# CMU-Quake/hercules

Measured on AMD Instinct MI355X. Metric: element-updates/sec (whole node) + achieved HBM GB/s, 64M-elem box, higher is better.
Workload: dtype f64

## Files before the change

### hercules_amd/capi.py

```python
import ctypes
import os

import numpy as np

_HERE = os.path.dirname(os.path.abspath(__file__))
_LIBPATH = os.environ.get("HQ_SOLVER_LIB") or os.path.join(_HERE, "csrc", "libhq_solver.so")

HQ_VARIANT_AUTO, HQ_VARIANT_SCATTER, HQ_VARIANT_PATCH = 0, 1, 2
IPC_BLOB_BYTES = 4096

EXPORTS = ["hq_device_count", "hq_last_error", "hq_create", "hq_destroy", "hq_get_info", "hq_get_info_sized", "hq_abi_version", "hq_comm_init_ipc_n",
           "hq_options_init", "hq_create_opts", "hq_get_options", "hq_real_bytes",
           "hq_comm_unique_id", "hq_comm_init", "hq_comm_selftest", "hq_group_link", "hq_group_run", "hq_set_source", "hq_run", "hq_sync", "hq_gather", "hq_gather3",
           "hq_download", "hq_upload", "hq_phase_force", "hq_phase_update", "hq_download_force",
           "hq_run_timed", "hq_dominant_kernel", "hq_plan_check", "hq_stencil_plan_check", "hq_check_finite",
           "hq_stencil_coefficients", "hq_brick_plan_check", "hq_brick_plan_check_n", "hq_comm_init_host",
           "hq_comm_ipc_export", "hq_comm_init_ipc", "hq_comm_init_loopback"]


class HqError(RuntimeError):
    pass


HOST_EXCHANGE_FN = ctypes.CFUNCTYPE(ctypes.c_int, ctypes.c_void_p, ctypes.c_int32, ctypes.POINTER(ctypes.c_int32),
                                    ctypes.POINTER(ctypes.c_int64), ctypes.POINTER(ctypes.c_void_p), ctypes.c_int32,
                                    ctypes.POINTER(ctypes.c_int32), ctypes.POINTER(ctypes.c_int64),
                                    ctypes.POINTER(ctypes.c_void_p), ctypes.c_int32)


class _Messenger(ctypes.Structure):
    _fields_ = [("procid", ctypes.c_int32), ("nodecount", ctypes.c_int32),
                ("mapping", ctypes.c_void_p)]


class _Schedule(ctypes.Structure):
    _fields_ = [("c_count", ctypes.c_int32), ("first_c", ctypes.POINTER(_Messenger)),
                ("s_count", ctypes.c_int32), ("first_s", ctypes.POINTER(_Messenger))]


class _Desc(ctypes.Structure):
    _fields_ = [("lenum", ctypes.c_int32), ("nharbored", ctypes.c_int32), ("ldnnum", ctypes.c_int32),
                ("lnid", ctypes.c_void_p), ("node_xyz", ctypes.c_void_p),
                ("dn_ldnid", ctypes.c_void_p), ("dn_ptr", ctypes.c_void_p), ("dn_lanid", ctypes.c_void_p),
                ("eTable", ctypes.c_void_p), ("nTable", ctypes.c_void_p),
                ("tm1", ctypes.c_void_p), ("tm2", ctypes.c_void_p),
                ("an_sched", _Schedule), ("dn_sched", _Schedule),
                ("deltaT", ctypes.c_double), ("rank", ctypes.c_int32), ("nranks", ctypes.c_int32),
                ("variant", ctypes.c_int32), ("reserved", ctypes.c_int32), ("node_gnid", ctypes.c_void_p),
                ("edata", ctypes.c_void_p), ("mat_bbase", ctypes.c_double), ("mat_threshold_damping", ctypes.c_double),
                ("mat_threshold_vpvs", ctypes.c_double)]


class _Info(ctypes.Structure):
    _fields_ = [("variant", ctypes.c_int32), ("npatches", ctypes.c_int32),
                ("patch_pairs", ctypes.c_int64), ("device_bytes", ctypes.c_int64),
                ("step", ctypes.c_int32), ("nranks", ctypes.c_int32),
                ("lattice_patches", ctypes.c_int32), ("stencil_patches", ctypes.c_int32),
                ("ragged_patches", ctypes.c_int32), ("brick_units", ctypes.c_int32),
                ("brick_nodes", ctypes.c_int64), ("brick_units_pernode", ctypes.c_int32),
                ("brick_units_het", ctypes.c_int32), ("pcie_h2d_bytes", ctypes.c_int64),
                ("pcie_d2h_bytes", ctypes.c_int64), ("transport", ctypes.c_int32), ("ipc_arena_coarse", ctypes.c_int32),
                ("ipc_arena_kind", ctypes.c_int32), ("debug_halo", ctypes.c_int32),
                ("brick_units_packed", ctypes.c_int32), ("brick_units_ragged", ctypes.c_int32),
                ("brick_stream", ctypes.c_int32), ("brick_units_ragged_het", ctypes.c_int32), ("timed_steps", ctypes.c_int64),
                ("t_step_us", ctypes.c_double), ("t_shell_us", ctypes.c_double), ("t_interior_us", ctypes.c_double),
                ("t_chain_us", ctypes.c_double), ("t_chain_exposed_us", ctypes.c_double)]


OPTION_FIELDS = ["no_bricks", "brick_cz", "brick_minz", "brick_minnodes", "brick_no_het", "brick_no_ntsame", "brick_by_component",
                 "brick_stream", "brick_no_faces", "brick_half_tiles", "brick_no_pack", "patch_pipe", "patch_threads", "patch_pmax", "patch_pmerge", "patch_psplit", "patch_nlmax",
                 "patch_vmax", "patch_ragged", "patch_no_lattice", "patch_no_stencil", "patch_no_uniform", "patch_no_iso",
                 "patch_no_ntsame", "patch_no_dedup", "patch_wform", "patch_merge_rounds", "overlap", "no_overlap", "reserve_cus",
                 "cu_mask", "no_fused_share", "group_copies", "debug_halo", "ipc_arena"]


class Options(ctypes.Structure):
    _fields_ = ([("size", ctypes.c_uint64)] + [(n, ctypes.c_int32) for n in OPTION_FIELDS] +
                [("ipc_timeout_ms", ctypes.c_double), ("loopback_delay_us", ctypes.c_double),
                 ("verbose", ctypes.c_int32), ("quiet", ctypes.c_int32),
                 ("brick_ragged", ctypes.c_int32), ("brick_ragged_minfill", ctypes.c_int32),
                 ("allow_env", ctypes.c_int32), ("brick_ragged_het", ctypes.c_int32), ("reserved0", ctypes.c_int32),
                 ("phase_timing", ctypes.c_int32)])

    def __init__(self, **kw):
        super().__init__()
        load_library().hq_options_init(ctypes.byref(self), ctypes.c_uint64(ctypes.sizeof(self)))
        for k, v in kw.items():
            if k not in dict(self._fields_):
                raise TypeError("hq_options has no field %r" % k)
            setattr(self, k, v)

    def as_dict(self):
        return {k: getattr(self, k) for k, _ in self._fields_ if k != "size"}


_lib = None
_lib_f32 = None
_LIBPATH_F32 = os.environ.get("HQ_SOLVER_LIB_F32") or os.path.join(_HERE, "csrc", "libhq_solver_f32.so")


def load_library(path=None, precision="f64"):
    global _lib, _lib_f32
    if precision == "f32" and path is None:
        if _lib_f32 is None:
            _lib_f32 = load_library(_LIBPATH_F32)
            if _lib_f32.hq_real_bytes() != 4:
                raise HqError("%s was not built with -DHQ_SINGLE_PRECISION_SOLVER" % _LIBPATH_F32)
        return _lib_f32
    if _lib is not None and path is None:
        return _lib
    p = path or _LIBPATH
    if not os.path.exists(p):
        raise HqError("native library %s is missing: run `python -m hercules_amd.build` "
                      "(there is no Python/CPU fallback)" % p)
    probe = ctypes.CDLL(p, mode=ctypes.RTLD_LOCAL)
    lib = probe if probe.hq_real_bytes() == 4 else ctypes.CDLL(p, mode=ctypes.RTLD_GLOBAL)
    lib.hq_last_error.restype = ctypes.c_char_p
    lib.hq_dominant_kernel.restype = ctypes.c_char_p
    lib.hq_dominant_kernel.argtypes = [ctypes.c_void_p]
    for name in EXPORTS:
        getattr(lib, name)
    if path is None:
        _lib = lib
    return lib


def device_count():
    return int(load_library().hq_device_count())


def _check(rc, lib=None):
    if rc != 0:
        raise HqError("hq error %d: %s" % (rc, (lib or load_library()).hq_last_error().decode()))


def _ptr(a):
    return None if a is None else a.ctypes.data_as(ctypes.c_void_p)


def _schedule(sched, keep):
    out = _Schedule()
    if not sched:
        return out
    for key, cnt, first in (("c", "c_count", "first_c"), ("s", "s_count", "first_s")):
        items = sched.get(key, [])
        arr = (_Messenger * max(len(items), 1))()
        for i, (procid, mapping) in enumerate(items):
            m = np.ascontiguousarray(mapping, np.int32)
            keep.append(m)
            arr[i].procid = int(procid)
            arr[i].nodecount = len(m)
            arr[i].mapping = m.ctypes.data
        keep.append(arr)
        setattr(out, cnt, len(items))
        setattr(out, first, ctypes.cast(arr, ctypes.POINTER(_Messenger)))
    return out


class Solver:

    def __init__(self, lnid, etable, ntable, dt, tm1=None, tm2=None, node_xyz=None,
                 dangling=None, an_sched=None, dn_sched=None, rank=0, nranks=1,
                 variant=HQ_VARIANT_AUTO, device=0, options=None, edata=None, material=None, precision="f64"):
        lib = load_library(precision=precision)
        self.real = np.float32 if precision == "f32" else np.float64
        if lib.hq_real_bytes() != np.dtype(self.real).itemsize:
            raise HqError("library and precision %r disagree about sizeof(hq_real)" % precision)
        if isinstance(options, dict):
            options = Options(**options)
        keep = []
        lnid = np.ascontiguousarray(lnid, np.int32)
        etable = np.ascontiguousarray(etable, np.float64)
        ntable = np.ascontiguousarray(ntable, self.real)
        d = _Desc()
        d.lenum, d.nharbored = lnid.shape[0], ntable.shape[0]
        d.lnid, d.eTable, d.nTable = _ptr(lnid), _ptr(etable), _ptr(ntable)
        keep += [lnid, etable, ntable]
        if node_xyz is not None:
            node_xyz = np.ascontiguousarray(node_xyz, np.int32)
            keep.append(node_xyz)
            d.node_xyz = _ptr(node_xyz)
        for name, a in (("tm1", tm1), ("tm2", tm2)):
            if a is not None:
                a = np.ascontiguousarray(a, self.real)
                keep.append(a)
                setattr(d, name, _ptr(a))
        if dangling is not None:
            ids, ptr, anchors = [np.ascontiguousarray(x, np.int32) for x in dangling]
            keep += [ids, ptr, anchors]
            d.ldnnum = len(ids)
            d.dn_ldnid, d.dn_ptr, d.dn_lanid = _ptr(ids), _ptr(ptr), _ptr(anchors)
        if edata is not None:
            edata = np.ascontiguousarray(edata, np.float32)
            assert edata.shape == (lnid.shape[0], 4) and material is not None
            keep.append(edata)
            d.edata = _ptr(edata)
            d.mat_bbase, d.mat_threshold_damping, d.mat_threshold_vpvs = [float(v) for v in material]
        d.an_sched = _schedule(an_sched, keep)
        d.dn_sched = _schedule(dn_sched, keep)
        d.deltaT, d.rank, d.nranks, d.variant = dt, rank, nranks, variant
        self._h = ctypes.c_void_p()
        self.N, self.E = d.nharbored, d.lenum
        self._lib = lib
        if options is None:
            _check(lib.hq_create(ctypes.byref(d), ctypes.c_int(device), ctypes.byref(self._h)), lib)
        else:
            _check(lib.hq_create_opts(ctypes.byref(d), ctypes.c_int(device), ctypes.byref(options), ctypes.byref(self._h)), lib)

    def close(self):
        if getattr(self, "_h", None) and self._h.value:
            self._lib.hq_destroy(self._h)
            self._h = ctypes.c_void_p()

    __del__ = close

    def info(self):
        i = _Info()
        _check(self._lib.hq_get_info_sized(self._h, ctypes.byref(i), ctypes.c_uint64(ctypes.sizeof(i))), self._lib)
        return {k: getattr(i, k) for k, _ in _Info._fields_}

    def options(self):
        o = Options()
        _check(self._lib.hq_get_options(self._h, ctypes.byref(o), ctypes.c_uint64(ctypes.sizeof(o))), self._lib)
        return o.as_dict()

    def set_source(self, loaded_lnid, forces, step0=0):
        ids = np.ascontiguousarray(loaded_lnid, np.int32)
        F = np.ascontiguousarray(forces, np.float64)
        nsteps = F.shape[0] if len(ids) else 0
        _check(self._lib.hq_set_source(self._h, ctypes.c_int32(len(ids)), _ptr(ids),
                                       ctypes.c_int32(step0), ctypes.c_int32(nsteps), _ptr(F)))

    def comm_init(self, id128):
        buf = (ctypes.c_char * 128).from_buffer_copy(bytes(id128))
        _check(self._lib.hq_comm_init(self._h, buf), self._lib)

    def comm_init_host(self, exchange):
        import numpy as np

        def view(ptr, n):
            return np.ctypeslib.as_array(ctypes.cast(ctypes.c_void_p(ptr), ctypes.POINTER(ctypes.c_double)), shape=(int(n),))

        def trampoline(user, nrecv, rpeer, rcount, rbuf, nsend, speer, scount, sbuf, tag):
            try:
                exchange([(rpeer[i], view(rbuf[i], rcount[i])) for i in range(nrecv)],
                         [(speer[i], view(sbuf[i], scount[i])) for i in range(nsend)], tag)
                return 0
            except Exception:
                import traceback
                traceback.print_exc()
                return 1
        self._host_exchange = HOST_EXCHANGE_FN(trampoline)
        _check(self._lib.hq_comm_init_host(self._h, self._host_exchange, None), self._lib)

    def comm_ipc_export(self):
        buf = (ctypes.c_char * IPC_BLOB_BYTES)()
        _check(self._lib.hq_comm_ipc_export(self._h, buf), self._lib)
        return bytes(buf)

    def comm_init_ipc(self, blobs):
        raw = blobs if isinstance(blobs, (bytes, bytearray)) else b"".join(blobs)
        if len(raw) % IPC_BLOB_BYTES:
            raise HqError("comm_init_ipc: %d bytes is not a whole number of %d-byte blobs" % (len(raw), IPC_BLOB_BYTES))
        buf = (ctypes.c_char * len(raw)).from_buffer_copy(bytes(raw))
        _check(self._lib.hq_comm_init_ipc_n(self._h, buf, ctypes.c_int32(len(raw) // IPC_BLOB_BYTES)), self._lib)

    def comm_init_loopback(self):
        _check(self._lib.hq_comm_init_loopback(self._h), self._lib)

    def comm_selftest(self, count=1024):
        _check(self._lib.hq_comm_selftest(self._h, ctypes.c_int32(count)), self._lib)

    def run(self, nsteps):
        _check(self._lib.hq_run(self._h, ctypes.c_int32(nsteps)), self._lib)

    def sync(self):
        _check(self._lib.hq_sync(self._h), self._lib)

    def check_finite(self):
        n = ctypes.c_int64()
        _check(self._lib.hq_check_finite(self._h, ctypes.byref(n)), self._lib)
        return int(n.value)

    def run_timed(self, nsteps):
        tot, ker = ctypes.c_double(), ctypes.c_double()
        _check(self._lib.hq_run_timed(self._h, ctypes.c_int32(nsteps), ctypes.byref(tot), ctypes.byref(ker)), self._lib)
        return tot.value, ker.value

    def dominant_kernel(self):
        return self._lib.hq_dominant_kernel(self._h).decode()

    def download(self, want_tm2=True):
        tm1 = np.empty((self.N, 3), self.real)
        tm2 = np.empty((self.N, 3), self.real) if want_tm2 else None
        _check(self._lib.hq_download(self._h, _ptr(tm1), _ptr(tm2)), self._lib)
        return tm1, tm2

    def upload(self, tm1, tm2, step):
        a = np.ascontiguousarray(tm1, self.real)
        b = np.ascontiguousarray(tm2, self.real)
        _check(self._lib.hq_upload(self._h, _ptr(a), _ptr(b), ctypes.c_int32(step)), self._lib)

    def gather(self, lnid):
        ids = np.ascontiguousarray(np.asarray(lnid).reshape(-1), np.int32)
        o1 = np.empty((len(ids), 3), self.real)
        o2 = np.empty((len(ids), 3), self.real)
        _check(self._lib.hq_gather(self._h, ctypes.c_int32(len(ids)), _ptr(ids), _ptr(o1), _ptr(o2)), self._lib)
        return o1, o2

    def gather3(self, lnid):
        ids = np.ascontiguousarray(np.asarray(lnid).reshape(-1), np.int32)
        o = [np.empty((len(ids), 3), self.real) for _ in range(3)]
        _check(self._lib.hq_gather3(self._h, ctypes.c_int32(len(ids)), _ptr(ids), _ptr(o[0]), _ptr(o[1]), _ptr(o[2])), self._lib)
        return tuple(o)

    def phase_force(self):
        _check(self._lib.hq_phase_force(self._h), self._lib)

    def phase_update(self):
        _check(self._lib.hq_phase_update(self._h), self._lib)

    def download_force(self):
        f = np.empty((self.N, 3))
        _check(self._lib.hq_download_force(self._h, _ptr(f)), self._lib)
        return f


PLAN_REPORT = ("patches", "lattice_patches", "pairs", "distinct_row_blocks", "gather_passes", "gather_instructions",
               "lattice_gather_passes", "faults")


def plan_check(desc):
    rep = (ctypes.c_int64 * 8)()
    _check(load_library().hq_plan_check(ctypes.byref(desc), rep))
    return dict(zip(PLAN_REPORT, [int(v) for v in rep]))


STENCIL_PLAN_REPORT = ("patches", "tables", "full_lattices", "boundary_nodes", "corners_checked", "faults")


def stencil_plan_check(desc):
    rep = (ctypes.c_int64 * 6)()
    _check(load_library().hq_stencil_plan_check(ctypes.byref(desc), rep))
    return dict(zip(STENCIL_PLAN_REPORT, [int(v) for v in rep]))


BRICK_PLAN_REPORT = ("brick_nodes", "columns", "units", "units_one_nt_row", "het_units", "neighbours_checked",
                     "patch_nodes", "faults", "ragged_units", "ragged_nodes", "ragged_het_units", "ragged_het_nodes")


def brick_plan_check(desc):
    rep = (ctypes.c_int64 * len(BRICK_PLAN_REPORT))()
    _check(load_library().hq_brick_plan_check_n(ctypes.byref(desc), rep, ctypes.c_int32(len(BRICK_PLAN_REPORT))))
    return dict(zip(BRICK_PLAN_REPORT, [int(v) for v in rep]))


def comm_unique_id():
    buf = (ctypes.c_char * 128)()
    _check(load_library().hq_comm_unique_id(buf))
    return bytes(buf)


def group_link(solvers):
    arr = (ctypes.c_void_p * len(solvers))(*[s._h for s in solvers])
    lib = solvers[0]._lib
    _check(lib.hq_group_link(arr, ctypes.c_int32(len(solvers))), lib)


def group_run(solvers, nsteps):
    arr = (ctypes.c_void_p * len(solvers))(*[s._h for s in solvers])
    lib = solvers[0]._lib
    _check(lib.hq_group_run(arr, ctypes.c_int32(len(solvers)), ctypes.c_int32(nsteps)), lib)
    for s in solvers:
        s.sync()
```

### hercules_amd/csrc/hq_brick.h

```cpp
#ifndef HQ_BRICK_H
#define HQ_BRICK_H

#include <chrono>
#include <map>

#include "hq_patch.h"

#define HQ_BK_TX 64
#ifndef HQ_BK_TY
#define HQ_BK_TY 8
#endif
#define HQ_BK_THREADS (HQ_BK_TX * HQ_BK_TY)
#define HQ_BK_PY (HQ_BK_TX + 2)
#define HQ_BK_PLANE ((HQ_BK_TX + 2) * (HQ_BK_TY + 2))
#ifndef HQ_BK_ATTR
#define HQ_BK_ATTR
#endif
#define HQ_BK_NTSAME 1
#define HQ_BK_HET 2
#define HQ_BK_TOPFACE 8
#define HQ_BK_BOTFACE 16
#define HQ_BK_RAGGED 32
#define HQ_BK_PACKED 4
#ifndef HQ_BH_WAVES
#define HQ_BH_WAVES 8
#endif
#define HQ_BH_THREADS (64 * HQ_BH_WAVES)
#define HQ_BH_NRT (64 + 2 * (HQ_BH_WAVES - 1))
#define HQ_BH_TX 62
#define HQ_BH_TY (HQ_BH_WAVES - 1)
#define HQ_BH_PY 65
#define HQ_BH_CS HQ_BH_THREADS
#define HQ_BH_ROWS (65 * (HQ_BH_WAVES + 1))

struct hq_brick_unit {
    int64_t base;
    int64_t tab;
    int32_t nx, ny, np, flags;
    double  c1, c2, beta;
    double  m0, m2, m1;
    double  ft[7], fb[7];
    int64_t coef;
};

struct hq_brick_cfg {
    int cz = 32;
    int minz = 4;
    int minnodes = 512;
    int ragged = 1;
    int minfill = 128;
    int ragged_het = 1;
};

static hq_brick_cfg hq_brick_cfg_of(const hq_options& o)
{
    hq_brick_cfg c;
    c.cz = std::max(2, hq_value_or(o.brick_cz, c.cz));
    c.minz = std::max(1, hq_value_or(o.brick_minz, c.minz));
    c.minnodes = std::max(1, hq_value_or(o.brick_minnodes, c.minnodes));
    c.ragged = hq_value_or(o.brick_ragged, c.ragged) != 0;
    c.minfill = std::min(HQ_BK_THREADS, std::max(1, hq_value_or(o.brick_ragged_minfill, c.minfill)));
    c.ragged_het = hq_value_or(o.brick_ragged_het, c.ragged_het) != 0;
    return c;
}

struct hq_brick_host {
    int64_t nb = 0;
    std::vector<int32_t> perm;
    std::vector<hq_brick_unit> units;
    int32_t nsame = 0;
    int32_t nrag = 0;
    std::vector<int32_t> tab;
    std::vector<double> coef;
    std::vector<float> coef32;
    std::vector<double> nt2;
    int32_t nhet = 0;
    int32_t npacked = 0;
    int32_t nrhet = 0, nrpacked = 0;
    int32_t ncolumns = 0, nlevels = 0;
};

struct hq_brick_plan {
    int64_t nb = 0;
    int32_t nunits = 0, nsame = 0, nrag = 0, nhet = 0, npacked = 0, nrhet = 0, nrpacked = 0;
    hq_brick_unit* d_units = nullptr;
    int32_t* d_tab = nullptr;
    double* d_coef = nullptr;
    float* d_coef32 = nullptr;
    double* d_nt2 = nullptr;
    hq_mat_const mat = { 0, 0, 0, 0, 0, 0 };
    int32_t* d_src_ptr = nullptr;
    int32_t* d_src_ent = nullptr;
    std::vector<int64_t> h_base;
    std::vector<int32_t> h_slot;
    std::vector<int64_t> h_size;
    std::vector<int64_t> h_first;
};

struct hq_mat_src {
    const float* edata = nullptr;
    double dt = 0, bbase = 0, thr_damp = 0, thr_vpvs = 0;
};

static int hq_brick_plan_host(const hq_options& o, int64_t E, int64_t N, const int32_t* lnid, const int32_t* xyz, const double* c1,
                              const double* c2, const double* beta, const double* ntab, const char* excl,
                              hq_brick_host* B, const hq_mat_src* MS = nullptr)
{
    *B = hq_brick_host();
    if (!xyz || E <= 0 || N <= 0) return 0;
    const hq_brick_cfg cfg = hq_brick_cfg_of(o);
    const bool verbose = o.verbose > 1;
    auto t_lap = std::chrono::steady_clock::now();
    auto lap = [&](const char* what) {
        if (!verbose) return;
        const auto now = std::chrono::steady_clock::now();
        fprintf(stderr, "  brick plan: %-36s %6.2f s\n", what, std::chrono::duration<double>(now - t_lap).count());
        t_lap = now;
    };
    const int TX = HQ_BK_TX, TY = HQ_BK_TY;
    const bool want_het = !hq_set(o.brick_no_het);
    const bool stencil_ok = hq_stencil().ok;

    std::vector<int32_t> hs((size_t)E);
    std::map<int32_t, int64_t> cnt;
    {
        bool bad_order = false;
#pragma omp parallel
        {
            std::map<int32_t, int64_t> mine;
#pragma omp for schedule(static) reduction(|| : bad_order)
            for (int64_t e = 0; e < E; e++) {
                const int32_t* id = lnid + 8 * e;
                const int64_t h = (int64_t)xyz[3 * (int64_t)id[1]] - xyz[3 * (int64_t)id[0]];
                if (h <= 0 || h > 0x7fffffff) { bad_order = true; hs[(size_t)e] = 0; continue; }
                hs[(size_t)e] = (int32_t)h;
                mine[(int32_t)h]++;
            }
#pragma omp critical
            for (auto& kv : mine) cnt[kv.first] += kv.second;
        }
        if (bad_order) return 0;
    }
    lap("edge lengths");

    const bool want_faces = stencil_ok && hq_stencil().face_ok && !hq_set(o.brick_no_faces) && !hq_set(o.brick_no_ntsame);
    std::vector<uint8_t> touch;
    if (want_faces) {
        touch.assign((size_t)N, 0);
#pragma omp parallel for schedule(static)
        for (int64_t i = 0; i < E * 8; i++) {
            uint8_t& t8 = touch[(size_t)lnid[i]];
#pragma omp atomic
            t8++;
        }
    }

    struct level_t {
        int32_t h;
        int64_t O[3];
        int64_t D[3];
        std::vector<int32_t> Ng;
        std::vector<int32_t> Eg;
    };
    struct column_t { int lvl; int32_t x0, y0, nx, ny, z0, nz, ti, tj; int64_t base; int het; int top, bot; int rag; };
    struct ragged_t { std::vector<uint8_t> own; std::vector<int32_t> pfx; double c[3], m[3]; };
    std::vector<level_t> levels;
    std::vector<column_t> cols;
    std::vector<ragged_t> rags;
    std::vector<int32_t> ntx_of_level;

    for (auto& kv : cnt) {
        const int32_t h = kv.first;
        if (kv.second < (int64_t)cfg.minnodes) continue;
        level_t L;
        L.h = h;
        int64_t mn[3] = { INT64_MAX, INT64_MAX, INT64_MAX }, mx[3] = { INT64_MIN, INT64_MIN, INT64_MIN };
        {
            int64_t mn0 = INT64_MAX, mn1 = INT64_MAX, mn2 = INT64_MAX, mx0 = INT64_MIN, mx1 = INT64_MIN, mx2 = INT64_MIN;
#pragma omp parallel for schedule(static) reduction(min : mn0, mn1, mn2) reduction(max : mx0, mx1, mx2)
            for (int64_t e = 0; e < E; e++) {
                if (hs[(size_t)e] != h) continue;
                const int32_t* p = xyz + 3 * (int64_t)lnid[8 * e];
                mn0 = std::min<int64_t>(mn0, p[0]); mn1 = std::min<int64_t>(mn1, p[1]); mn2 = std::min<int64_t>(mn2, p[2]);
                mx0 = std::max<int64_t>(mx0, p[0]); mx1 = std::max<int64_t>(mx1, p[1]); mx2 = std::max<int64_t>(mx2, p[2]);
            }
            mn[0] = mn0; mn[1] = mn1; mn[2] = mn2; mx[0] = mx0; mx[1] = mx1; mx[2] = mx2;
        }
        bool ok = true;
        for (int d = 0; d < 3; d++) {
            L.O[d] = mn[d];
            if ((mx[d] - mn[d]) % h) ok = false;
            L.D[d] = (mx[d] - mn[d]) / h + 1;
        }
        if (!ok) continue;
        const int64_t NX = L.D[0] + 1, NY = L.D[1] + 1, NZ = L.D[2] + 1;
        const double vol = (double)NX * (double)NY * (double)NZ;
        if (vol > 8.0 * (double)kv.second + 65536.0 || vol > 2.0e9) continue;
        std::vector<int32_t>& Eg = L.Eg;
        Eg.assign((size_t)(L.D[0] * L.D[1] * L.D[2]), -1);
        L.Ng.assign((size_t)(NX * NY * NZ), -1);
        for (int pass = 0; pass < 2 && ok; pass++) {
            bool bad = false;
#pragma omp parallel for schedule(static) reduction(|| : bad)
            for (int64_t e = 0; e < E; e++) {
                if (hs[(size_t)e] != h) continue;
                const int32_t* id = lnid + 8 * e;
                int64_t q[3];
                bool good = true;
                for (int d = 0; d < 3; d++) {
                    const int64_t v = (int64_t)xyz[3 * (int64_t)id[0] + d] - L.O[d];
                    if (v % h) good = false;
                    q[d] = v / h;
                }
                if (!good) { bad = true; continue; }
                int32_t& cell = Eg[(size_t)((q[2] * L.D[1] + q[1]) * L.D[0] + q[0])];
                if (pass == 0) cell = (int32_t)e; else if (cell != (int32_t)e) bad = true;
                for (int c = 0; c < 8; c++) {
                    const int64_t X = q[0] + (c & 1), Y = q[1] + ((c >> 1) & 1), Z = q[2] + ((c >> 2) & 1);
                    const int32_t* p = xyz + 3 * (int64_t)id[c];
                    if (p[0] != L.O[0] + X * h || p[1] != L.O[1] + Y * h || p[2] != L.O[2] + Z * h) { bad = true; break; }
                    int32_t& g = L.Ng[(size_t)((Z * NY + Y) * NX + X)];
                    if (pass == 0) g = id[c]; else if (g != id[c]) bad = true;
                }
            }
            if (bad) ok = false;
        }
        if (!ok) continue;
        lap("level grids");
        std::vector<char> S((size_t)(NX * NY * NZ), 0);
        int64_t sx0 = INT64_MAX, sx1 = -1, sy0 = INT64_MAX, sy1 = -1;
        int64_t nsimple = 0;
#pragma omp parallel for schedule(static) reduction(min : sx0, sy0) reduction(max : sx1, sy1) reduction(+ : nsimple)
        for (int64_t Z = 1; Z < L.D[2]; Z++)
            for (int64_t Y = 1; Y < L.D[1]; Y++)
                for (int64_t X = 1; X < L.D[0]; X++) {
                    const int32_t n = L.Ng[(size_t)((Z * NY + Y) * NX + X)];
                    if (n < 0 || (excl && excl[n])) continue;
                    const double* q = ntab + 7 * (int64_t)n;
                    if (!((q[1] == q[2]) && (q[1] == q[3]) && (q[4] == q[5]) && (q[4] == q[6]))) continue;
                    int32_t e0 = -1;
                    bool s = true, uni = true;
                    for (int o = 0; o < 8 && s; o++) {
                        const int64_t cx = X - (o & 1), cy = Y - ((o >> 1) & 1), cz = Z - ((o >> 2) & 1);
                        const int32_t e = Eg[(size_t)((cz * L.D[1] + cy) * L.D[0] + cx)];
                        if (e < 0) { s = false; break; }
                        if (e0 < 0) e0 = e;
                        else uni = uni && c1[e] == c1[e0] && c2[e] == c2[e0] && beta[e] == beta[e0];
                    }
                    if (!s) continue;
                    if (!stencil_ok) uni = false;
// ... 252 lines not shown
    lap("numbering");
    B->nb = nb;
    B->ncolumns = (int32_t)cols.size();
    B->nlevels = (int32_t)levels.size();

    struct unit_t { int col; int32_t za, np; int64_t key; };
    std::vector<unit_t> us;
    int cz = cfg.cz;
    if (!hq_given(o.brick_cz)) {
        for (cz = 32; cz > 8; cz /= 2) {
            int64_t n = 0;
            for (auto& c : cols) n += (c.nz + cz - 1) / cz;
            if (n >= 512) break;
        }
    }
    for (size_t ci = 0; ci < cols.size(); ci++) {
        const column_t& c = cols[ci];
        const int32_t nch = (c.nz + cz - 1) / cz;
        const int32_t G = std::max(1, 64 / std::max(1, ntx_of_level[(size_t)c.lvl]));
        for (int32_t k = 0; k < nch; k++) {
            const int32_t za = (int32_t)((int64_t)c.nz * k / nch), zb = (int32_t)((int64_t)c.nz * (k + 1) / nch);
            const int64_t key = ((int64_t)c.lvl << 56) | ((int64_t)(c.tj / G) << 42) | ((int64_t)((c.z0 + za) / cz) << 28) |
                                ((int64_t)(c.tj % G) << 20) | (int64_t)c.ti;
            us.push_back({ (int)ci, c.z0 + za, zb - za, key });
        }
    }
    std::stable_sort(us.begin(), us.end(), [](const unit_t& a, const unit_t& b) { return a.key < b.key; });
    B->units.resize(us.size());
    std::vector<int64_t> toff(us.size() + 1, 0);
    for (size_t u = 0; u < us.size(); u++) {
        const column_t& c = cols[(size_t)us[u].col];
        const int64_t nr = 2 * (c.nx + 2) + 2 * c.ny;
        toff[u + 1] = toff[u] + ((int64_t)(us[u].np + 2) * nr + (c.rag ? us[u].np + 2 : 2) * (int64_t)c.nx * c.ny + 3) / 4 * 4;
    }
    B->tab.assign((size_t)toff[us.size()] + 64, 0);
    std::vector<int64_t> coff(us.size() + 1, 0);
    for (size_t u = 0; u < us.size(); u++)
        coff[u + 1] = coff[u] + (cols[(size_t)us[u].col].het ? (int64_t)(us[u].np + 1) * HQ_BH_THREADS * 3 : 0);
    B->coef.assign((size_t)coff[us.size()] + 8, 0.0);
    const bool try_pack = MS && MS->edata && MS->dt > 0 && !hq_set(o.brick_no_pack);
    if (try_pack) { B->coef32.assign((size_t)coff[us.size()] + 8, 0.0f); B->nt2.assign(2 * (size_t)N, 0.0); }
    int fault = 0;
    auto set_fault = [&]() {
#pragma omp atomic write
        fault = 1;
    };
    std::vector<char> same(us.size(), 0);
#pragma omp parallel for schedule(dynamic, 16)
    for (int64_t u = 0; u < (int64_t)us.size(); u++) {
        const column_t& c = cols[(size_t)us[(size_t)u].col];
        const level_t& L = levels[(size_t)c.lvl];
        const int64_t NX = L.D[0] + 1, NY = L.D[1] + 1;
        const int32_t za = us[(size_t)u].za, np = us[(size_t)u].np, nx = c.nx, ny = c.ny, nr = 2 * (nx + 2) + 2 * ny;
        auto dev = [&](int64_t X, int64_t Y, int64_t Z) -> int32_t {
            if (X < 0 || Y < 0 || Z < 0 || X > L.D[0] || Y > L.D[1] || Z > L.D[2]) { set_fault(); return 0; }
            const int32_t n = L.Ng[(size_t)((Z * NY + Y) * NX + X)];
            if (n < 0) { set_fault(); return 0; }
            return B->perm[(size_t)n];
        };
        int32_t* t = B->tab.data() + toff[(size_t)u];
        hq_brick_unit& U = B->units[(size_t)u];
        if (c.rag) {
            const ragged_t& R = rags[(size_t)c.rag - 1];
            auto any = [&](int64_t X, int64_t Y, int64_t Z) -> int32_t {
                if (X < 0 || Y < 0 || Z < 0 || X > L.D[0] || Y > L.D[1] || Z > L.D[2]) return -1;
                const int32_t n = L.Ng[(size_t)((Z * NY + Y) * NX + X)];
                return n < 0 ? -1 : B->perm[(size_t)n];
            };
            auto owns = [&](int32_t i, int32_t j, int32_t k) -> bool {
                return i >= 0 && i < nx && j >= 0 && j < ny && k >= 1 && k <= np && R.own[(size_t)((((int64_t)za - 1 + k - c.z0) * ny + j) * nx + i)];
            };
            auto wanted = [&](int32_t i, int32_t j, int32_t k) -> bool {
                for (int32_t dk = -1; dk <= 1; dk++)
                    for (int32_t dj = -1; dj <= 1; dj++)
                        for (int32_t di = -1; di <= 1; di++)
                            if (owns(i + di, j + dj, k + dk)) return true;
                return false;
            };
            for (int32_t k = 0; k < np + 2; k++) {
                const int64_t Z = (int64_t)za - 1 + k;
                int32_t* r = t + (int64_t)k * nr;
                for (int32_t i = 0; i < nx + 2; i++) {
                    r[i] = wanted(i - 1, -1, k) ? any(c.x0 - 1 + i, c.y0 - 1, Z) : -1;
                    r[nx + 2 + i] = wanted(i - 1, ny, k) ? any(c.x0 - 1 + i, c.y0 + ny, Z) : -1;
                }
                for (int32_t j = 0; j < ny; j++) {
                    r[2 * (nx + 2) + j] = wanted(-1, j, k) ? any(c.x0 - 1, c.y0 + j, Z) : -1;
                    r[2 * (nx + 2) + ny + j] = wanted(nx, j, k) ? any(c.x0 + nx, c.y0 + j, Z) : -1;
                }
                int32_t* pl = t + (int64_t)(np + 2) * nr + (int64_t)k * nx * ny;
                for (int32_t j = 0; j < ny; j++)
                    for (int32_t i = 0; i < nx; i++) {
                        const bool own = owns(i, j, k);
                        const int32_t q = own || wanted(i, j, k) ? any(c.x0 + i, c.y0 + j, Z) : -1;
                        if (own && q < 0) set_fault();
                        pl[j * nx + i] = own ? q : (q < 0 ? -1 : -q - 2);
                    }
            }
            U.base = c.base + R.pfx[(size_t)(za - c.z0)];
            U.tab = toff[(size_t)u];
            U.nx = nx; U.ny = ny; U.np = np; U.flags = HQ_BK_NTSAME | HQ_BK_RAGGED;
            memset(U.ft, 0, sizeof U.ft); memset(U.fb, 0, sizeof U.fb);
            U.coef = 0;
            if (!c.het) {
                U.c1 = R.c[0]; U.c2 = R.c[1]; U.beta = R.c[2];
                U.m0 = R.m[0]; U.m2 = R.m[1]; U.m1 = R.m[2];
                same[(size_t)u] = 4;
                continue;
            }
            U.flags = HQ_BK_RAGGED;
            U.c1 = U.c2 = U.beta = 0.0; U.m0 = 1.0; U.m2 = U.m1 = 0.0;
        }
        if (!c.rag) {
        for (int32_t k = 0; k < np + 2; k++) {
            const int64_t Z = (int64_t)za - 1 + k;
            int32_t* r = t + (int64_t)k * nr;
            for (int32_t i = 0; i < nx + 2; i++) { r[i] = dev(c.x0 - 1 + i, c.y0 - 1, Z); r[nx + 2 + i] = dev(c.x0 - 1 + i, c.y0 + ny, Z); }
            for (int32_t j = 0; j < ny; j++) { r[2 * (nx + 2) + j] = dev(c.x0 - 1, c.y0 + j, Z); r[2 * (nx + 2) + ny + j] = dev(c.x0 + nx, c.y0 + j, Z); }
        }
        int32_t* cap = t + (int64_t)(np + 2) * nr;
        for (int32_t j = 0; j < ny; j++)
            for (int32_t i = 0; i < nx; i++) {
                cap[j * nx + i] = dev(c.x0 + i, c.y0 + j, (int64_t)za - 1);
                cap[nx * ny + j * nx + i] = dev(c.x0 + i, c.y0 + j, (int64_t)za + np);
            }
        U.base = c.base + (int64_t)(za - c.z0 + c.top) * nx * ny;
        U.tab = toff[(size_t)u];
        U.nx = nx; U.ny = ny; U.np = np; U.flags = 0;
        memset(U.ft, 0, sizeof U.ft); memset(U.fb, 0, sizeof U.fb);
        if (c.top && za == c.z0) {
            U.flags |= HQ_BK_TOPFACE;
            memcpy(U.ft, ntab + 7 * (int64_t)L.Ng[(size_t)((((int64_t)za - 1) * NY + c.y0) * NX + c.x0)], sizeof U.ft);
        }
        if (c.bot && za + np == c.z0 + c.nz) {
            U.flags |= HQ_BK_BOTFACE;
            memcpy(U.fb, ntab + 7 * (int64_t)L.Ng[(size_t)((((int64_t)za + np) * NY + c.y0) * NX + c.x0)], sizeof U.fb);
        }
        const int32_t n0 = L.Ng[(size_t)(((int64_t)za * NY + c.y0) * NX + c.x0)];
        {
            const int32_t e0 = L.Eg[(size_t)((((int64_t)za - 1) * L.D[1] + (c.y0 - 1)) * L.D[0] + (c.x0 - 1))];
            if (e0 < 0) { set_fault(); continue; }
            U.c1 = c1[e0]; U.c2 = c2[e0]; U.beta = beta[e0];
        }
        bool sm = true;
        const double* q0 = ntab + 7 * (int64_t)n0;
        for (int32_t z = 0; z < np && sm; z++)
            for (int32_t y = 0; y < ny && sm; y++)
                for (int32_t x = 0; x < nx; x++) {
                    const int32_t n = L.Ng[(size_t)((((int64_t)za + z) * NY + (c.y0 + y)) * NX + (c.x0 + x))];
                    const double* q = ntab + 7 * (int64_t)n;
                    if (q[0] != q0[0] || q[1] != q0[1] || q[4] != q0[4]) { sm = false; break; }
                }
        if (sm && !c.het && !hq_set(o.brick_no_ntsame)) { U.flags |= HQ_BK_NTSAME; same[(size_t)u] = 1; }
        U.m0 = q0[0]; U.m2 = q0[1]; U.m1 = q0[4];
        U.coef = 0;
        }
        if (c.het) {
            U.flags |= HQ_BK_HET;
            same[(size_t)u] = c.rag ? 5 : 2;
            U.coef = coff[(size_t)u];
            double* cf = B->coef.data() + coff[(size_t)u];
            for (int32_t l = 0; l <= np; l++)
                for (int32_t j = 0; j < HQ_BH_WAVES; j++)
                    for (int32_t i = 0; i < 64; i++) {
                        const int64_t cx = (int64_t)c.x0 - 1 + i, cy = (int64_t)c.y0 - 1 + j, cz = (int64_t)za - 1 + l;
                        double* o = cf + (int64_t)l * (3 * HQ_BH_THREADS) + (j * 64 + i);
                        int32_t e = -1;
                        if (cx >= 0 && cy >= 0 && cz >= 0 && cx < L.D[0] && cy < L.D[1] && cz < L.D[2])
                            e = L.Eg[(size_t)((cz * L.D[1] + cy) * L.D[0] + cx)];
                        if (e >= 0) { o[0] = c1[e]; o[HQ_BH_CS] = c2[e]; o[2 * HQ_BH_CS] = beta[e]; }
                        else if (!c.rag && i <= nx && j <= ny) set_fault();
                    }
            if (try_pack) {
                bool ok = true;
                int32_t e0 = L.Eg[(size_t)(((int64_t)za * L.D[1] + c.y0) * L.D[0] + c.x0)];
                if (c.rag) {
                    e0 = -1;
                    for (int32_t l = 0; l <= np && e0 < 0; l++)
                        for (int32_t j = 0; j < HQ_BH_WAVES && e0 < 0; j++)
                            for (int32_t i = 0; i < 64 && e0 < 0; i++) {
                                const int64_t cx = (int64_t)c.x0 - 1 + i, cy = (int64_t)c.y0 - 1 + j, cz = (int64_t)za - 1 + l;
                                if (cx >= 0 && cy >= 0 && cz >= 0 && cx < L.D[0] && cy < L.D[1] && cz < L.D[2]) e0 = L.Eg[(size_t)((cz * L.D[1] + cy) * L.D[0] + cx)];
                            }
                }
                const float hf = e0 >= 0 ? MS->edata[4 * (int64_t)e0] : 0.0f;
                hq_mat_const K = { (MS->dt * MS->dt) * (double)hf, (double)hf, MS->dt, MS->bbase, MS->thr_damp, MS->thr_vpvs };
                float* cq = B->coef32.data() + coff[(size_t)u];
                for (int32_t l = 0; l <= np && ok; l++)
                    for (int32_t j = 0; j < HQ_BH_WAVES && ok; j++)
                        for (int32_t i = 0; i < 64; i++) {
                            const int64_t cx = (int64_t)c.x0 - 1 + i, cy = (int64_t)c.y0 - 1 + j, cz = (int64_t)za - 1 + l;
                            int32_t e = -1;
                            if (cx >= 0 && cy >= 0 && cz >= 0 && cx < L.D[0] && cy < L.D[1] && cz < L.D[2])
                                e = L.Eg[(size_t)((cz * L.D[1] + cy) * L.D[0] + cx)];
                            float* o = cq + (int64_t)l * (3 * HQ_BH_THREADS) + (j * 64 + i);
                            o[0] = o[HQ_BH_CS] = o[2 * HQ_BH_CS] = 0.0f;
                            if (e < 0) continue;
                            const float* ed = MS->edata + 4 * (int64_t)e;
                            if (ed[0] != hf || !(ed[3] > 0.0f)) { ok = false; break; }
                            bool hit = false;
                            for (int fixed = 0; fixed < 2 && !hit; fixed++) {
                                double k1, k2, kb;
                                hq_material_coef(fixed ? -ed[3] : ed[3], ed[2], ed[1], K, &k1, &k2, &kb);
                                if (k1 == c1[e] && k2 == c2[e] && kb == beta[e]) { o[0] = fixed ? -ed[3] : ed[3]; o[HQ_BH_CS] = ed[2]; o[2 * HQ_BH_CS] = ed[1]; hit = true; }
                            }
                            if (!hit) { ok = false; break; }
                        }
                const int32_t* own_ids = c.rag ? t + (int64_t)(np + 2) * nr + (int64_t)nx * ny : nullptr;
                for (int32_t z = 0; z < np && ok; z++)
                    for (int32_t y = 0; y < ny && ok; y++)
                        for (int32_t x = 0; x < nx; x++) {
                            if (own_ids && own_ids[((int64_t)z * ny + y) * nx + x] < 0) continue;
                            const int32_t n = L.Ng[(size_t)((((int64_t)za + z) * NY + (c.y0 + y)) * NX + (c.x0 + x))];
                            const double* q = ntab + 7 * (int64_t)n;
                            const double sdiff = q[0] - q[4];
                            if (q[0] - sdiff != q[4] || fabs((2.0 * q[0] - sdiff) - q[1]) > 1e-15 * fabs(q[1])) { ok = false; break; }
                            double* o2 = B->nt2.data() + 2 * (own_ids ? (int64_t)own_ids[((int64_t)z * ny + y) * nx + x] : U.base + ((int64_t)z * ny + y) * nx + x);
                            o2[0] = q[0]; o2[1] = sdiff;
                        }
                if (ok) { U.flags |= HQ_BK_PACKED; same[(size_t)u] = c.rag ? 6 : 3; U.c1 = K.A; U.c2 = K.h; }
            }
        }
    }
    lap("unit tables");
    if (fault) { g_patch_err = "brick plan: a neighbour of a simple node is missing"; return -1; }
    {
        std::vector<hq_brick_unit> a, r, b, h, hp, rh, rhp;
        for (size_t u = 0; u < us.size(); u++)
            (same[u] == 1 ? a : (same[u] == 4 ? r : (same[u] == 2 ? h : (same[u] == 3 ? hp : (same[u] == 5 ? rh : (same[u] == 6 ? rhp : b)))))).push_back(B->units[u]);
        B->nsame = (int32_t)(a.size() + r.size());
        B->nrag = (int32_t)r.size();
        B->nhet = (int32_t)(h.size() + hp.size());
        B->npacked = (int32_t)hp.size();
        B->nrhet = (int32_t)(rh.size() + rhp.size());
        B->nrpacked = (int32_t)rhp.size();
        a.insert(a.end(), r.begin(), r.end());
        a.insert(a.end(), b.begin(), b.end());
        a.insert(a.end(), h.begin(), h.end());
        a.insert(a.end(), hp.begin(), hp.end());
        a.insert(a.end(), rh.begin(), rh.end());
        a.insert(a.end(), rhp.begin(), rhp.end());
        B->units.swap(a);
        if (B->npacked + B->nrpacked == 0) { std::vector<float>().swap(B->coef32); std::vector<double>().swap(B->nt2); }
        if (verbose) fprintf(stderr, "  brick plan: %d units: %d with one n_t row of which %d ragged, %d per-element coefficients of which %d packed, %d ragged per-element of which %d packed\n",
                             (int)B->units.size(), B->nsame, B->nrag, B->nhet, B->npacked, B->nrhet, B->nrpacked);
        if (verbose && B->nrag) {
            int64_t pos = 0, own = 0, other = 0;
            for (const hq_brick_unit& U : B->units) {
                if (!(U.flags & HQ_BK_RAGGED)) continue;
                const int32_t* pl = B->tab.data() + U.tab + (int64_t)(U.np + 2) * (2 * (U.nx + 2) + 2 * U.ny);
                for (int64_t i = 0; i < (int64_t)U.nx * U.ny * (U.np + 2); i++) { pos++; own += pl[i] >= 0; other += pl[i] <= -2; }
            }
            fprintf(stderr, "  brick plan: ragged units: %lld positions, %lld owned, %lld loaded for their neighbours' sake\n", (long long)pos, (long long)own, (long long)other);
        }
    }
    return 0;
}


static __device__ __forceinline__ double hq_uniform(double v)
{
    const int lo = __builtin_amdgcn_readfirstlane(__double2loint(v)), hi = __builtin_amdgcn_readfirstlane(__double2hiint(v));
    return __hiloint2double(hi, lo);
}

template <bool PERNODE, bool BYCOMP, bool RAGGED = false>
__global__ void HQ_BK_ATTR __launch_bounds__(HQ_BK_THREADS, 4)
hq_k_brick(int32_t count, int32_t per_xcd, const hq_brick_unit* __restrict__ units, const int32_t* __restrict__ tab,
           const hq_real* __restrict__ u1g, const hq_real* __restrict__ u2g, hq_real* __restrict__ ung,
           const double* __restrict__ nt3, const int32_t* __restrict__ src_ptr, const int32_t* __restrict__ src_ent,
           const double* __restrict__ F, double dt2, hq_stencil_coef sc)
{
    __shared__ __align__(16) double s_w[2 * 3 * HQ_BK_PLANE];
    const int slot = (int)(blockIdx.x & 7) * per_xcd + (int)(blockIdx.x >> 3);
    if (slot >= count) return;
    const hq_brick_unit U = units[slot];
    const int nx = U.nx, ny = U.ny, np = U.np, nxy = nx * ny, nr = 2 * (nx + 2) + 2 * ny;
    const int t = threadIdx.x, lx = t & (HQ_BK_TX - 1), ly = t >> 6;
    const bool active = lx < nx && ly < ny;
    const int sidx = active ? ly * nx + lx : 0;
    const int myrow = (ly + 1) * HQ_BK_PY + lx + 1;
    const bool ring = t < nr;
    int rrow;
    {
        int rx, ry;
        if (t < nx + 2) { rx = t - 1; ry = -1; }
        else if (t < 2 * (nx + 2)) { rx = t - (nx + 2) - 1; ry = ny; }
        else if (t < 2 * (nx + 2) + ny) { rx = -1; ry = t - 2 * (nx + 2); }
        else { rx = nx; ry = t - 2 * (nx + 2) - ny; }
        rrow = (ry + 1) * HQ_BK_PY + rx + 1;
    }
    const int32_t* __restrict__ utab = tab + U.tab;
    const int rofs = ring ? t : 0;
    const int32_t* __restrict__ cap = utab + (int64_t)(np + 2) * nr;
    int32_t vOut = -1, vMid = RAGGED ? cap[sidx] : 0, vCur = RAGGED ? cap[nxy + sidx] : 0, vNext = 0;
    const int32_t id_lo = RAGGED ? (vMid >= 0 ? vMid : -vMid - 2) : cap[sidx];
    const double beta = U.beta;
    double P[6], Q[2];
#pragma unroll
    for (int i = 0; i < 6; i++) P[i] = hq_uniform(U.c1 * sc.p1[i] + U.c2 * sc.p2[i]);
#pragma unroll
    for (int i = 0; i < 2; i++) Q[i] = hq_uniform(U.c1 * sc.q1[i] + U.c2 * sc.q2[i]);
    const bool has_src = F && src_ptr[slot + 1] > src_ptr[slot];

    hq_real x1[3] = { 0, 0, 0 }, x2[3] = { 0, 0, 0 }, y1[3] = { 0, 0, 0 }, y2[3] = { 0, 0, 0 };
    double mn[3] = { U.m0, U.m2, U.m1 };
    double m0A = hq_uniform(1.0 / U.m0), m0B = m0A;
    double fA[3] = { 0.0, 0.0, 0.0 }, fB[3] = { 0.0, 0.0, 0.0 };
    int32_t rid = utab[rofs];

#define HQ_BK_LOAD(node_)                                                                             \
    {                                                                                                 \
        const int64_t a_ = (node_);                                                                   \
        if (active && (!RAGGED || a_ >= 0)) {                                                         \
            _Pragma("unroll") for (int d = 0; d < 3; d++) { x1[d] = u1g[3 * a_ + d]; x2[d] = u2g[3 * a_ + d]; } \
            if (PERNODE) { _Pragma("unroll") for (int d = 0; d < 3; d++) mn[d] = nt3[3 * a_ + d]; }    \
        }                                                                                             \
        if (ring && (!RAGGED || rid >= 0)) {                                                          \
            const int64_t b_ = (int64_t)rid;                                                          \
            _Pragma("unroll") for (int d = 0; d < 3; d++) { y1[d] = u1g[3 * b_ + d]; y2[d] = u2g[3 * b_ + d]; } \
        }                                                                                             \
    }
#define HQ_BK_PUT(s_, acc_, M2_, M1_)                                                                 \
    {                                                                                                 \
        hq_lds_double* img_ = (hq_lds_double*)s_w + 3 * HQ_BK_PLANE * (s_);                            \
        if (active) {                                                                                 \
            _Pragma("unroll") for (int d = 0; d < 3; d++) {                                           \
                const double a1_ = x1[d], a2_ = x2[d];                                                \
                img_[3 * myrow + d] = a1_ + beta * (a1_ - a2_);                                       \
                acc_[d] += (M2_) * a1_ - (M1_) * a2_;                                                 \
            }                                                                                         \
        }                                                                                             \
        if (ring) { _Pragma("unroll") for (int d = 0; d < 3; d++) { const double b1_ = y1[d], b2_ = y2[d]; img_[3 * rrow + d] = b1_ + beta * (b1_ - b2_); } } \
    }

    const bool topf = !PERNODE && !RAGGED && (U.flags & HQ_BK_TOPFACE) != 0, botf = !PERNODE && !RAGGED && (U.flags & HQ_BK_BOTFACE) != 0;
    const double rho = hq_uniform((U.c1 - U.c2) / (U.c1 + U.c2));

    HQ_BK_LOAD((int64_t)id_lo)
    rid = utab[nr + rofs];
    if (topf) HQ_BK_PUT(0, fB, U.ft[1 + d], U.ft[4 + d])
    else { double dummy[3] = { 0.0, 0.0, 0.0 }; HQ_BK_PUT(0, dummy, mn[1], mn[2]) }
    for (int k = 0; k <= np + 1; k++) {
        if (k <= np) {
            if (RAGGED) {
                HQ_BK_LOAD((int64_t)(vCur >= 0 ? vCur : -vCur - 2))
                if (k < np) vNext = cap[(k + 2) * nxy + sidx];
            } else HQ_BK_LOAD(k == np ? (int64_t)cap[nxy + sidx] : U.base + (int64_t)k * nxy + sidx)
            if (k < np) rid = utab[(k + 2) * nr + rofs];
        }
        __syncthreads();
        const hq_lds_double* __restrict__ q = (const hq_lds_double*)s_w + 3 * (HQ_BK_PLANE * (k & 1) + myrow);
        double m[3], g[3], Uo[3];
        if (BYCOMP) {
            double A_x, A_y;
            {
                const double C = q[2], XM = q[2 - 3], XP = q[2 + 3], YM = q[2 - 3 * HQ_BK_PY], YP = q[2 + 3 * HQ_BK_PY];
                const double MM = q[2 - 3 * HQ_BK_PY - 3], PM = q[2 - 3 * HQ_BK_PY + 3], MP = q[2 + 3 * HQ_BK_PY - 3], PP = q[2 + 3 * HQ_BK_PY + 3];
                const double sxy = (XM + XP) + (YM + YP), dg = (MM + PP) + (PM + MP);
                m[2] = fma(P[0], C, fma(P[2], sxy, P[4] * dg));
                g[2] = fma(P[1], C, fma(P[3], sxy, P[5] * dg));
                Uo[0] = fma(Q[0], XP - XM, Q[1] * ((PP - MP) + (PM - MM)));
                Uo[1] = fma(Q[0], YP - YM, Q[1] * ((PP - PM) + (MP - MM)));
            }
            __builtin_amdgcn_sched_barrier(0);
            {
                const double C = q[0], XM = q[0 - 3], XP = q[0 + 3], YM = q[0 - 3 * HQ_BK_PY], YP = q[0 + 3 * HQ_BK_PY];
                const double MM = q[0 - 3 * HQ_BK_PY - 3], PM = q[0 - 3 * HQ_BK_PY + 3], MP = q[0 + 3 * HQ_BK_PY - 3], PP = q[0 + 3 * HQ_BK_PY + 3];
                const double sx = XM + XP, sy = YM + YP, dg = (MM + PP) + (PM + MP);
                A_x = (PP + MM) - (PM + MP);
                m[0] = fma(P[0], C, fma(P[1], sx, fma(P[2], sy, P[3] * dg)));
                g[0] = fma(P[2], C, fma(P[3], sx, fma(P[4], sy, P[5] * dg)));
                Uo[2] = fma(Q[0], XP - XM, Q[1] * ((PP - MP) + (PM - MM)));
            }
            __builtin_amdgcn_sched_barrier(0);
            {
                const double C = q[1], XM = q[1 - 3], XP = q[1 + 3], YM = q[1 - 3 * HQ_BK_PY], YP = q[1 + 3 * HQ_BK_PY];
                const double MM = q[1 - 3 * HQ_BK_PY - 3], PM = q[1 - 3 * HQ_BK_PY + 3], MP = q[1 + 3 * HQ_BK_PY - 3], PP = q[1 + 3 * HQ_BK_PY + 3];
                const double sx = XM + XP, sy = YM + YP, dg = (MM + PP) + (PM + MP);
                A_y = (PP + MM) - (PM + MP);
                m[1] = fma(P[0], C, fma(P[1], sy, fma(P[2], sx, fma(P[3], dg, Q[0] * A_x))));
                g[1] = fma(P[2], C, fma(P[3], sy, fma(P[4], sx, fma(P[5], dg, Q[1] * A_x))));
                Uo[2] += fma(Q[0], YP - YM, Q[1] * ((PP - PM) + (MP - MM)));
            }
            m[0] = fma(Q[0], A_y, m[0]);
            g[0] = fma(Q[1], A_y, g[0]);
        } else {
            double C[3], XM[3], XP[3], YM[3], YP[3], MM[3], PM[3], MP[3], PP[3];
#pragma unroll
            for (int d = 0; d < 3; d++) {
                C[d] = q[d]; XM[d] = q[d - 3]; XP[d] = q[d + 3]; YM[d] = q[d - 3 * HQ_BK_PY]; YP[d] = q[d + 3 * HQ_BK_PY];
                MM[d] = q[d - 3 * HQ_BK_PY - 3]; PM[d] = q[d - 3 * HQ_BK_PY + 3];
                MP[d] = q[d + 3 * HQ_BK_PY - 3]; PP[d] = q[d + 3 * HQ_BK_PY + 3];
            }
            double sx[3], sy[3], dg[3];
#pragma unroll
            for (int d = 0; d < 3; d++) { sx[d] = XM[d] + XP[d]; sy[d] = YM[d] + YP[d]; dg[d] = (MM[d] + PP[d]) + (PM[d] + MP[d]); }
            const double A_x = (PP[0] + MM[0]) - (PM[0] + MP[0]), A_y = (PP[1] + MM[1]) - (PM[1] + MP[1]);
            const double Bx0_z = XP[2] - XM[2], Bx0_x = XP[0] - XM[0], By0_z = YP[2] - YM[2], By0_y = YP[1] - YM[1];
            const double Bx1_z = (PP[2] - MP[2]) + (PM[2] - MM[2]), Bx1_x = (PP[0] - MP[0]) + (PM[0] - MM[0]);
            const double By1_z = (PP[2] - PM[2]) + (MP[2] - MM[2]), By1_y = (PP[1] - PM[1]) + (MP[1] - MM[1]);
            const double sxy_z = sx[2] + sy[2];
            m[0] = fma(P[0], C[0], fma(P[1], sx[0], fma(P[2], sy[0], fma(P[3], dg[0], Q[0] * A_y))));
            m[1] = fma(P[0], C[1], fma(P[1], sy[1], fma(P[2], sx[1], fma(P[3], dg[1], Q[0] * A_x))));
            m[2] = fma(P[0], C[2], fma(P[2], sxy_z, P[4] * dg[2]));
            g[0] = fma(P[2], C[0], fma(P[3], sx[0], fma(P[4], sy[0], fma(P[5], dg[0], Q[1] * A_y))));
            g[1] = fma(P[2], C[1], fma(P[3], sy[1], fma(P[4], sx[1], fma(P[5], dg[1], Q[1] * A_x))));
            g[2] = fma(P[1], C[2], fma(P[3], sxy_z, P[5] * dg[2]));
            Uo[0] = fma(Q[0], Bx0_z, Q[1] * Bx1_z);
            Uo[1] = fma(Q[0], By0_z, Q[1] * By1_z);
            Uo[2] = fma(Q[0], Bx0_x, fma(Q[1], Bx1_x, fma(Q[0], By0_y, Q[1] * By1_y)));
        }
        if (k == 0 && topf) {
            m[0] = fma(rho, Uo[0], 0.5 * m[0]); m[1] = fma(rho, Uo[1], 0.5 * m[1]); m[2] = fma(-rho, Uo[2], 0.5 * m[2]);
        }
        if (k == np + 1 && botf && active) {
            double f[3];
            f[0] = fB[0] + fma(-rho, Uo[0], 0.5 * m[0]); f[1] = fB[1] + fma(-rho, Uo[1], 0.5 * m[1]); f[2] = fB[2] + fma(rho, Uo[2], 0.5 * m[2]);
            const int local = np * nxy + sidx;
            if (has_src) {
                for (int i = src_ptr[slot]; i < src_ptr[slot + 1]; i++)
                    if (src_ent[2 * i] == local) {
                        const int li = src_ent[2 * i + 1];
                        for (int d = 0; d < 3; d++) f[d] += F[3 * li + d] * dt2;
                    }
            }
            hq_real* out = ung + 3 * (int64_t)cap[nxy + sidx];
            const double rm = 1.0 / U.fb[0];
#pragma unroll
            for (int d = 0; d < 3; d++) out[d] = f[d] * rm;
        }
        const bool outface = k == 1 && topf;
        if ((k >= 2 || outface) && active && (!RAGGED || vOut >= 0)) {
            double f[3];
#pragma unroll
            for (int d = 0; d < 3; d++) f[d] = fA[d] + (g[d] + Uo[d]);
            const int local = RAGGED ? (int)(vOut - U.base) : (k - 2) * nxy + sidx;
            if (has_src) {
                for (int i = src_ptr[slot]; i < src_ptr[slot + 1]; i++)
                    if (src_ent[2 * i] == local) {
                        const int li = src_ent[2 * i + 1];
                        for (int d = 0; d < 3; d++) f[d] += F[3 * li + d] * dt2;
                    }
            }
            hq_real* out = ung + 3 * (RAGGED ? (int64_t)vOut : (outface ? (int64_t)cap[sidx] : U.base + (int64_t)local));
            const double rm = outface ? 1.0 / U.ft[0] : m0A;
#pragma unroll
            for (int d = 0; d < 3; d++) out[d] = f[d] * rm;
        }
#pragma unroll
        for (int d = 0; d < 3; d++) { fA[d] = fB[d] + m[d]; fB[d] = g[d] - Uo[d]; }
        if (RAGGED) { vOut = vMid; vMid = vCur; vCur = vNext; }
        if (PERNODE) { m0A = m0B; m0B = 1.0 / mn[0]; }
        if (k < np || (k == np && !botf)) HQ_BK_PUT((k + 1) & 1, fB, mn[1], mn[2])
        else if (k == np) HQ_BK_PUT((k + 1) & 1, fB, U.fb[1 + d], U.fb[4 + d])
    }
#undef HQ_BK_LOAD
#undef HQ_BK_PUT
}


#define HQ_BH_LDS (8 * (2 * 2 * 3 * HQ_BH_ROWS + 6 * HQ_BH_THREADS))
#ifndef HQ_BH_ABL
#define HQ_BH_ABL 0
#endif

static __device__ __forceinline__ double hq_dpp_from_next_lane(double v)
{
    int lo = __double2loint(v), hi = __double2hiint(v);
    lo = __builtin_amdgcn_update_dpp(0, lo, 0x130, 0xf, 0xf, true);
    hi = __builtin_amdgcn_update_dpp(0, hi, 0x130, 0xf, 0xf, true);
    return __hiloint2double(hi, lo);
}

static __device__ __forceinline__ int64_t hq_rag_node(int32_t v) { return v >= 0 ? (int64_t)v : (v <= -2 ? (int64_t)(-v - 2) : (int64_t)0); }

template <bool PACKED, bool RAGGED = false>
__global__ void __launch_bounds__(HQ_BH_THREADS, HQ_BH_WAVES == 12 ? 3 : 4)
hq_k_brick_het(int32_t count, int32_t per_xcd, const hq_brick_unit* __restrict__ units, const int32_t* __restrict__ tab,
               const void* __restrict__ coef_any, const hq_real* __restrict__ u1g, const hq_real* __restrict__ u2g,
               hq_real* __restrict__ ung, const double* __restrict__ nt3, const int32_t* __restrict__ src_ptr,
               const int32_t* __restrict__ src_ent, const double* __restrict__ F, double dt2, hq_mat_const mat)
{
    extern __shared__ __align__(16) double s_het[];
    hq_lds_double* const img = (hq_lds_double*)s_het;
    hq_lds_double* const xch = img + 2 * 2 * 3 * HQ_BH_ROWS;
    const int slot = (int)(blockIdx.x & 7) * per_xcd + (int)(blockIdx.x >> 3);
    if (slot >= count) return;
    const hq_brick_unit U = units[slot];
    const int nx = U.nx, ny = U.ny, np = U.np, nxy = nx * ny, nr = 2 * (nx + 2) + 2 * ny;
    const int t = threadIdx.x, lx = t & 63, ly = t >> 6;
    const bool owner = lx < nx && ly < ny;
    const int sidx = owner ? ly * nx + lx : 0;
    const int myrow = (ly + 1) * HQ_BH_PY + lx + 1;
    const int row0 = ly * HQ_BH_PY + lx;
    const int rq = ly == HQ_BH_WAVES - 1 ? lx : (lx >= 62 ? 64 + 2 * ly + (lx - 62) : -1);
    const bool ringA = rq >= 0 && rq < nr, ringB = rq >= 0 && rq + HQ_BH_NRT < nr;
    auto ring_row = [&](int r) {
        int rx, ry;
        if (r < nx + 2) { rx = r - 1; ry = -1; }
        else if (r < 2 * (nx + 2)) { rx = r - (nx + 2) - 1; ry = ny; }
        else if (r < 2 * (nx + 2) + ny) { rx = -1; ry = r - 2 * (nx + 2); }
        else { rx = nx; ry = r - 2 * (nx + 2) - ny; }
        return (ry + 1) * HQ_BH_PY + rx + 1;
    };
    const int rrowA = ringA ? ring_row(rq) : 0, rrowB = ringB ? ring_row(rq + HQ_BH_NRT) : 0;
    const int32_t* __restrict__ rtabA = tab + U.tab + (ringA ? rq : 0);
    const int32_t* __restrict__ rtabB = tab + U.tab + (ringB ? rq + HQ_BH_NRT : 0);
    const int32_t* __restrict__ cap = tab + U.tab + (int64_t)(np + 2) * nr;
    const int64_t id_lo = RAGGED ? 0 : cap[sidx], id_hi = RAGGED ? 0 : cap[nxy + sidx];
    int32_t vload = RAGGED ? cap[sidx] : 0, vnext = RAGGED ? cap[nxy + sidx] : 0, idA = -1, idB = -1;
    const double* __restrict__ cf = (const double*)coef_any + (PACKED ? 0 : U.coef + t);
    const float* __restrict__ cf32 = (const float*)coef_any + (PACKED ? U.coef + t : 0);
    hq_mat_const K = mat;
    if (PACKED) { K.A = hq_uniform(U.c1); K.h = hq_uniform(U.c2); }
    const int third = (PACKED && owner) ? 1 : 2;
    const bool has_src = F && src_ptr[slot + 1] > src_ptr[slot];

    hq_real x1[3] = { 0, 0, 0 }, x2[3] = { 0, 0, 0 }, rb1[3] = { 0, 0, 0 }, rb2[3] = { 0, 0, 0 };
    constexpr bool SAME = sizeof(hq_real) == sizeof(double);
    double mn[3] = { 1.0, 0.0, 0.0 };
    double accA[3] = { 0.0, 0.0, 0.0 }, accB[3] = { 0.0, 0.0, 0.0 }, m0A = 1.0, m0B = 1.0;
    int32_t ridA = rtabA[0], ridB = rtabB[0];
    if (RAGGED) { ridA = ridA < 0 ? 0 : ridA; ridB = ridB < 0 ? 0 : ridB; }

#define HQ_BH_LOAD(node_)                                                                             \
    {                                                                                                 \
        const int64_t a_ = owner ? (int64_t)(node_) : (int64_t)ridA;                                  \
        const double* __restrict__ pb_ = (owner || sizeof(hq_real) != sizeof(double)) ? nt3 + (PACKED ? 2 : 3) * a_ : (const double*)(const void*)(u1g + 3 * (int64_t)ridB); \
        _Pragma("unroll") for (int d = 0; d < 3; d++) { x1[d] = u1g[3 * a_ + d]; x2[d] = u2g[3 * a_ + d]; } \
        if (SAME || owner) {                                                                          \
            if (HQ_BH_ABL != 4) { mn[0] = pb_[0]; mn[1] = pb_[1]; mn[2] = pb_[third]; }                \
        } else {                      \
            const hq_real* __restrict__ pu_ = u1g + 3 * (int64_t)ridB;                                \
            rb1[0] = pu_[0]; rb1[1] = pu_[1]; rb1[2] = pu_[2];                                         \
        }                                                                                             \
    }
#define HQ_BH_LOAD_B()                                                                                \
    {                                                                                                 \
        if (ringB && HQ_BH_ABL != 1) {                                                                \
            const int64_t b_ = (int64_t)ridB;                                                         \
            _Pragma("unroll") for (int d = 0; d < 3; d++) { if (SAME) accB[d] = u2g[3 * b_ + d]; else rb2[d] = u2g[3 * b_ + d]; } \
        }                                                                                             \
    }
#define HQ_BH_PUT(s_, acc_, m0_)                                                                      \
    {                                                                                                 \
        hq_lds_double* iu_ = img + (size_t)(s_) * (2 * 3 * HQ_BH_ROWS);                                \
        hq_lds_double* iv_ = iu_ + 3 * HQ_BH_ROWS;                                                    \
        if (owner) {                                                                                  \
            const double m2_ = PACKED ? 2.0 * mn[0] - mn[1] : mn[1], m1_ = PACKED ? mn[0] - mn[1] : mn[2]; \
            _Pragma("unroll") for (int d = 0; d < 3; d++) {                                           \
                const double a1_ = x1[d], a2_ = x2[d];                                                \
                iu_[3 * myrow + d] = a1_; iv_[3 * myrow + d] = a1_ - a2_;                             \
                acc_[d] = m2_ * a1_ - m1_ * a2_;                                                      \
            }                                                                                         \
            m0_ = 1.0 / mn[0];                                                                        \
            if (RAGGED) idB = vload;                                                                  \
        }                                                                                             \
        if (ringA) { _Pragma("unroll") for (int d = 0; d < 3; d++) { const double a1_ = x1[d], a2_ = x2[d]; iu_[3 * rrowA + d] = a1_; iv_[3 * rrowA + d] = a1_ - a2_; } } \
        if (ringB) { _Pragma("unroll") for (int d = 0; d < 3; d++) { const double b1_ = SAME ? mn[d] : (double)rb1[d], b2_ = SAME ? accB[d] : (double)rb2[d]; iu_[3 * rrowB + d] = b1_; iv_[3 * rrowB + d] = b1_ - b2_; } } \
    }

    double nc1 = 0.0, nc2 = 0.0, nbeta = 0.0, c1 = 0.0, c2 = 0.0, beta = 0.0;
    float nrho = 0.0f, nvs = 0.0f, nvp = 0.0f;
#define HQ_BH_REQUEST(p_)                                                                             \
    {                                                                                                 \
        const int pp_ = (p_);                                                                         \
        if (HQ_BH_ABL != 2 && !PACKED) { const double* q_ = cf + (int64_t)(pp_ - 1) * (3 * HQ_BH_THREADS); nc1 = q_[0]; nc2 = q_[HQ_BH_CS]; nbeta = q_[2 * HQ_BH_CS]; } \
        if (HQ_BH_ABL != 2 && PACKED) { const float* q_ = cf32 + (int64_t)(pp_ - 1) * (3 * HQ_BH_THREADS); nrho = q_[0]; nvs = q_[HQ_BH_CS]; nvp = q_[2 * HQ_BH_CS]; } \
        if (RAGGED) vload = vnext;                                                                    \
        HQ_BH_LOAD(RAGGED ? hq_rag_node(vload) : (pp_ == np + 1 ? id_hi : U.base + (int64_t)(pp_ - 1) * nxy + sidx)) \
        HQ_BH_LOAD_B()                                                                                \
        { const int64_t r_ = (int64_t)(pp_ < np + 1 ? pp_ + 1 : np + 1) * nr; ridA = rtabA[r_]; ridB = rtabB[r_]; } \
        if (RAGGED) vnext = cap[(int64_t)(pp_ < np + 1 ? pp_ + 1 : np + 1) * nxy + sidx];              \
    }
    if (HQ_BH_ABL == 2) { nc1 = dt2; nc2 = dt2; nbeta = dt2; }
    HQ_BH_LOAD(RAGGED ? hq_rag_node(vload) : id_lo)
    HQ_BH_LOAD_B()
    ridA = rtabA[nr]; ridB = rtabB[nr];
    if (RAGGED) { ridA = ridA < 0 ? 0 : ridA; ridB = ridB < 0 ? 0 : ridB; }
    for (int l = -2; l <= np; l++) {
        if (l >= 0) {
            double X[8], Y[8], Z[8];
#pragma unroll
            for (int m = 0; m < 8; m++) {
                const hq_lds_double* pu = img + (size_t)((l + (m >> 2)) & 1) * (2 * 3 * HQ_BH_ROWS) + 3 * (row0 + (m & 1) + ((m >> 1) & 1) * HQ_BH_PY);
                const hq_lds_double* pv = pu + 3 * HQ_BH_ROWS;
                X[m] = fma(beta, pv[0], pu[0]); Y[m] = fma(beta, pv[1], pu[1]); Z[m] = fma(beta, pv[2], pu[2]);
            }
            if (HQ_BH_ABL != 3) hq_element_force<true>(X, Y, Z, c1, c2);
            double G[2][2][3];
#pragma unroll
            for (int yb = 0; yb < 2; yb++)
#pragma unroll
                for (int zb = 0; zb < 2; zb++) {
                    const int m1 = 1 + 2 * yb + 4 * zb, m0 = 2 * yb + 4 * zb;
                    G[yb][zb][0] = X[m1] + hq_dpp_from_next_lane(X[m0]);
                    G[yb][zb][1] = Y[m1] + hq_dpp_from_next_lane(Y[m0]);
                    G[yb][zb][2] = Z[m1] + hq_dpp_from_next_lane(Z[m0]);
                }
#pragma unroll
            for (int zb = 0; zb < 2; zb++)
#pragma unroll
                for (int d = 0; d < 3; d++) xch[(3 * zb + d) * HQ_BH_THREADS + t] = G[0][zb][d];
            __syncthreads();
            if (owner) {
                double H0[3], H1[3];
#pragma unroll
                for (int d = 0; d < 3; d++) {
                    H0[d] = G[1][0][d] + xch[d * HQ_BH_THREADS + t + 64];
                    H1[d] = G[1][1][d] + xch[(3 + d) * HQ_BH_THREADS + t + 64];
                }
                if (l >= 1 && (!RAGGED || idA >= 0)) {
                    double f[3];
#pragma unroll
                    for (int d = 0; d < 3; d++) f[d] = accA[d] + (H0[d] - H1[d]);
                    const int local = RAGGED ? (int)((int64_t)idA - U.base) : (l - 1) * nxy + sidx;
                    if (has_src) {
                        for (int i = src_ptr[slot]; i < src_ptr[slot + 1]; i++)
                            if (src_ent[2 * i] == local) {
                                const int li = src_ent[2 * i + 1];
                                for (int d = 0; d < 3; d++) f[d] += F[3 * li + d] * dt2;
                            }
                    }
                    hq_real* out = ung + 3 * (U.base + (int64_t)local);
#pragma unroll
                    for (int d = 0; d < 3; d++) out[d] = f[d] * m0A;
                }
#pragma unroll
                for (int d = 0; d < 3; d++) accA[d] = accB[d] + (H0[d] + H1[d]);
                m0A = m0B;
                if (RAGGED) idA = idB;
            }
        }
        if (l < np) HQ_BH_PUT(l & 1, accB, m0B)
        if (PACKED) hq_material_coef(nrho, nvs, nvp, K, &c1, &c2, &beta);
        else { c1 = nc1; c2 = nc2; beta = nbeta; }
        asm volatile("" : "+v"(c1), "+v"(c2), "+v"(beta), "+v"(ridA), "+v"(ridB));
        if (RAGGED) { asm volatile("" : "+v"(vnext)); ridA = ridA < 0 ? 0 : ridA; ridB = ridB < 0 ? 0 : ridB; }
        if (l + 1 < np) HQ_BH_REQUEST(l + 3)
        __syncthreads();
    }
#undef HQ_BH_REQUEST
#undef HQ_BH_LOAD
#undef HQ_BH_LOAD_B
#undef HQ_BH_PUT
}


static void hq_brick_free(hq_brick_plan* P)
{
    void* ptrs[] = { P->d_units, P->d_tab, P->d_coef, P->d_coef32, P->d_nt2, P->d_src_ptr, P->d_src_ent };
    for (void* p : ptrs) if (p) hipFree(p);
    *P = hq_brick_plan();
}

static int hq_brick_upload(hq_brick_plan* P, const hq_brick_host& B, int64_t* bytes)
{
    P->nb = B.nb;
    P->nunits = (int32_t)B.units.size();
    P->nsame = B.nsame;
    P->nrag = B.nrag;
    P->nhet = B.nhet;
    P->npacked = B.npacked;
    P->nrhet = B.nrhet;
    P->nrpacked = B.nrpacked;
    if (P->nunits == 0) return 0;
    if (P->nhet + P->nrhet > 0) {
        if (P->nhet > P->npacked || P->nrhet > P->nrpacked) {
            if (hipMalloc((void**)&P->d_coef, 8 * B.coef.size()) != hipSuccess) { g_patch_err = "hipMalloc failed"; return -2; }
            *bytes += (int64_t)(8 * B.coef.size());
            if (hipMemcpy(P->d_coef, B.coef.data(), 8 * B.coef.size(), hipMemcpyHostToDevice) != hipSuccess) { g_patch_err = "brick coefficient upload failed"; return -3; }
        }
        if (P->npacked + P->nrpacked > 0) {
            if (hipMalloc((void**)&P->d_coef32, 4 * B.coef32.size()) != hipSuccess || hipMalloc((void**)&P->d_nt2, 8 * B.nt2.size()) != hipSuccess) { g_patch_err = "hipMalloc failed"; return -2; }
            *bytes += (int64_t)(4 * B.coef32.size() + 8 * B.nt2.size());
            if (hipMemcpy(P->d_coef32, B.coef32.data(), 4 * B.coef32.size(), hipMemcpyHostToDevice) != hipSuccess ||
                hipMemcpy(P->d_nt2, B.nt2.data(), 8 * B.nt2.size(), hipMemcpyHostToDevice) != hipSuccess) { g_patch_err = "brick coefficient upload failed"; return -3; }
        }
        static bool attr_set = false;
        if (!attr_set) {
            if (hipFuncSetAttribute((const void*)hq_k_brick_het<false>, hipFuncAttributeMaxDynamicSharedMemorySize, HQ_BH_LDS) != hipSuccess ||
                hipFuncSetAttribute((const void*)hq_k_brick_het<true>, hipFuncAttributeMaxDynamicSharedMemorySize, HQ_BH_LDS) != hipSuccess ||
                hipFuncSetAttribute((const void*)hq_k_brick_het<false, true>, hipFuncAttributeMaxDynamicSharedMemorySize, HQ_BH_LDS) != hipSuccess ||
                hipFuncSetAttribute((const void*)hq_k_brick_het<true, true>, hipFuncAttributeMaxDynamicSharedMemorySize, HQ_BH_LDS) != hipSuccess) { g_patch_err = "hq_k_brick_het: LDS attribute"; return -3; }
            attr_set = true;
        }
    }
    if (hipMalloc((void**)&P->d_units, sizeof(hq_brick_unit) * B.units.size()) != hipSuccess ||
        hipMalloc((void**)&P->d_tab, 4 * B.tab.size()) != hipSuccess) { g_patch_err = "hipMalloc failed"; return -2; }
    *bytes += (int64_t)(sizeof(hq_brick_unit) * B.units.size() + 4 * B.tab.size());
    if (hipMemcpy(P->d_units, B.units.data(), sizeof(hq_brick_unit) * B.units.size(), hipMemcpyHostToDevice) != hipSuccess ||
        hipMemcpy(P->d_tab, B.tab.data(), 4 * B.tab.size(), hipMemcpyHostToDevice) != hipSuccess) { g_patch_err = "brick table upload failed"; return -3; }
    std::vector<std::pair<int64_t, int32_t>> by_base;
    for (int32_t u = 0; u < P->nunits; u++) by_base.push_back({ B.units[(size_t)u].base, u });
    std::sort(by_base.begin(), by_base.end());
    for (auto& pr : by_base) {
        const hq_brick_unit& U = B.units[(size_t)pr.second];
        const int64_t nxy = (int64_t)U.nx * U.ny;
        const int top = (U.flags & HQ_BK_TOPFACE) != 0, bot = (U.flags & HQ_BK_BOTFACE) != 0;
        int64_t size = nxy * (U.np + top + bot);
        if (U.flags & HQ_BK_RAGGED) {
            const int32_t* pl = B.tab.data() + U.tab + (int64_t)(U.np + 2) * (2 * (U.nx + 2) + 2 * U.ny);
            size = 0;
            for (int64_t i = nxy; i < nxy * (U.np + 1); i++) size += pl[i] >= 0;
        }
        P->h_base.push_back(pr.first - top * nxy); P->h_slot.push_back(pr.second); P->h_size.push_back(size);
        P->h_first.push_back(pr.first);
    }
    return 0;
}

static int hq_brick_set_source(hq_brick_plan* P, int32_t nloaded, const int32_t* loaded, int64_t* bytes)
{
    if (P->d_src_ptr) { hipFree(P->d_src_ptr); P->d_src_ptr = nullptr; }
    if (P->d_src_ent) { hipFree(P->d_src_ent); P->d_src_ent = nullptr; }
    if (nloaded <= 0 || P->nunits == 0) return 0;
    std::vector<std::array<int32_t, 3>> rec;
    for (int32_t i = 0; i < nloaded; i++) {
        if (loaded[i] >= P->nb) continue;
        const size_t k = (size_t)(std::upper_bound(P->h_base.begin(), P->h_base.end(), (int64_t)loaded[i]) - P->h_base.begin()) - 1;
        rec.push_back({ P->h_slot[k], (int32_t)(loaded[i] - P->h_first[k]), i });
    }
    if (rec.empty()) return 0;
    std::sort(rec.begin(), rec.end());
    std::vector<int32_t> ptr((size_t)P->nunits + 1, 0), ent(rec.size() * 2);
    for (auto& r : rec) ptr[(size_t)r[0] + 1]++;
    for (int32_t u = 0; u < P->nunits; u++) ptr[(size_t)u + 1] += ptr[(size_t)u];
    for (size_t k = 0; k < rec.size(); k++) { ent[2 * k] = rec[k][1]; ent[2 * k + 1] = rec[k][2]; }
    if (hipMalloc((void**)&P->d_src_ptr, 4 * ptr.size()) != hipSuccess) { P->d_src_ptr = nullptr; return -2; }
    if (hipMalloc((void**)&P->d_src_ent, 4 * ent.size()) != hipSuccess) {
        hipFree(P->d_src_ptr); P->d_src_ptr = nullptr; P->d_src_ent = nullptr;
        return -2;
    }
    if (hipMemcpy(P->d_src_ptr, ptr.data(), 4 * ptr.size(), hipMemcpyHostToDevice) != hipSuccess ||
        hipMemcpy(P->d_src_ent, ent.data(), 4 * ent.size(), hipMemcpyHostToDevice) != hipSuccess) {
        hipFree(P->d_src_ptr); hipFree(P->d_src_ent); P->d_src_ptr = nullptr; P->d_src_ent = nullptr;
        return -3;
    }
    *bytes += (int64_t)(4 * ptr.size() + 4 * ent.size());
    return 0;
}

static void hq_brick_launch(const hq_brick_plan* P, const hq_real* u1, const hq_real* u2, hq_real* un, const double* nt3,
                            const double* F, double dt2, hipStream_t stream, bool light = false)
{
    const int32_t cnt[7] = { P->nsame - P->nrag, P->nunits - P->nsame - P->nhet - P->nrhet, P->nhet - P->npacked, P->npacked, P->nrag,
                             P->nrhet - P->nrpacked, P->nrpacked };
    int32_t first = 0;
    for (int k4 = 0; k4 < 7; k4++) {
        const int k = k4 == 0 ? 0 : (k4 == 1 ? 4 : (k4 < 5 ? k4 - 1 : k4));
        const int32_t count = cnt[k];
        if (count <= 0) continue;
        const int per_xcd = (count + 7) / 8;
        const int32_t* sp = P->d_src_ptr ? P->d_src_ptr + first : nullptr;
#define HQ_BK_ARGS count, per_xcd, P->d_units + first, P->d_tab, u1, u2, un, nt3, sp, P->d_src_ent, (sp ? F : nullptr), dt2, hq_stencil().c
#ifdef HQ_EXPERIMENT
        const unsigned xpad = getenv("HQ_X_BRICK_LDS_PAD") ? (unsigned)atoi(getenv("HQ_X_BRICK_LDS_PAD")) : 0u;
        if (xpad && k == 0) {
            static bool once = false;
            if (!once) {
                once = true;
                hipFuncSetAttribute((const void*)hq_k_brick<false, true>, hipFuncAttributeMaxDynamicSharedMemorySize, (int)xpad);
                hipFuncSetAttribute((const void*)hq_k_brick<false, false>, hipFuncAttributeMaxDynamicSharedMemorySize, (int)xpad);
            }
            if (light) hq_k_brick<false, true><<<per_xcd * 8, HQ_BK_THREADS, xpad, stream>>>(HQ_BK_ARGS);
            else hq_k_brick<false, false><<<per_xcd * 8, HQ_BK_THREADS, xpad, stream>>>(HQ_BK_ARGS);
        } else
#endif
        if (k == 0 && light) hq_k_brick<false, true><<<per_xcd * 8, HQ_BK_THREADS, 0, stream>>>(HQ_BK_ARGS);
        else if (k == 0) hq_k_brick<false, false><<<per_xcd * 8, HQ_BK_THREADS, 0, stream>>>(HQ_BK_ARGS);
        else if (k == 1 && light) hq_k_brick<true, true><<<per_xcd * 8, HQ_BK_THREADS, 0, stream>>>(HQ_BK_ARGS);
        else if (k == 1) hq_k_brick<true, false><<<per_xcd * 8, HQ_BK_THREADS, 0, stream>>>(HQ_BK_ARGS);
        else if (k == 4 && light) hq_k_brick<false, true, true><<<per_xcd * 8, HQ_BK_THREADS, 0, stream>>>(HQ_BK_ARGS);
        else if (k == 4) hq_k_brick<false, false, true><<<per_xcd * 8, HQ_BK_THREADS, 0, stream>>>(HQ_BK_ARGS);
        else if (k == 2) hq_k_brick_het<false><<<per_xcd * 8, HQ_BH_THREADS, HQ_BH_LDS, stream>>>(count, per_xcd, P->d_units + first, P->d_tab, P->d_coef, u1, u2, un, nt3, sp,
                                                                                               P->d_src_ent, (sp ? F : nullptr), dt2, P->mat);
        else if (k == 3) hq_k_brick_het<true><<<per_xcd * 8, HQ_BH_THREADS, HQ_BH_LDS, stream>>>(count, per_xcd, P->d_units + first, P->d_tab, P->d_coef32, u1, u2, un, P->d_nt2, sp,
                                                                                   P->d_src_ent, (sp ? F : nullptr), dt2, P->mat);
        else if (k == 5) hq_k_brick_het<false, true><<<per_xcd * 8, HQ_BH_THREADS, HQ_BH_LDS, stream>>>(count, per_xcd, P->d_units + first, P->d_tab, P->d_coef, u1, u2, un, nt3, sp,
                                                                                                     P->d_src_ent, (sp ? F : nullptr), dt2, P->mat);
        else hq_k_brick_het<true, true><<<per_xcd * 8, HQ_BH_THREADS, HQ_BH_LDS, stream>>>(count, per_xcd, P->d_units + first, P->d_tab, P->d_coef32, u1, u2, un, P->d_nt2, sp,
                                                                                          P->d_src_ent, (sp ? F : nullptr), dt2, P->mat);
#undef HQ_BK_ARGS
        first += count;
    }
}

#endif
```

### hercules_amd/csrc/hq_engine.hip

```cpp
#include <hip/hip_runtime.h>
#include <dlfcn.h>
#include <stdint.h>
#include <stdio.h>
#include <stdlib.h>
#include <string.h>
#include <unistd.h>

#include <algorithm>
#include <chrono>
#include <vector>

#define HQ_SOLVER_IMPLEMENTATION 1
#include "../../include/hq_solver.h"
#include "hq_kernels.h"
#include "hq_opts.h"
#include "hq_patch.h"
#include "hq_brick.h"


static thread_local char g_err[512] = "";

static int hq_fail(int code, const char* fmt, const char* a = "", const char* b = "")
{
    snprintf(g_err, sizeof g_err, fmt, a, b);
    return code;
}

#define HQ_HIP(call)                                                                  \
    do {                                                                              \
        hipError_t e_ = (call);                                                       \
        if (e_ != hipSuccess)                                                         \
            return hq_fail(HQ_ERR_DEVICE, "%s: %s", #call, hipGetErrorString(e_));    \
    } while (0)

extern "C" const char* hq_last_error(void) { return g_err; }


#include <rccl/rccl.h>
typedef ncclUniqueId hq_nccl_id;
typedef ncclComm_t hq_nccl_comm;
struct hq_rccl {
    void* handle;
    decltype(&ncclGetUniqueId) GetUniqueId;
    decltype(&ncclCommInitRank) CommInitRank;
    decltype(&ncclCommDestroy) CommDestroy;
    decltype(&ncclSend) Send;
    decltype(&ncclRecv) Recv;
    decltype(&ncclGroupStart) GroupStart;
    decltype(&ncclGroupEnd) GroupEnd;
    decltype(&ncclGetErrorString) GetErrorString;
};
static hq_rccl g_rccl = {};
static const ncclDataType_t HQ_NCCL_INT64 = ncclInt64, HQ_NCCL_DOUBLE = ncclFloat64;
static_assert(sizeof(hq_nccl_id) == 128, "hq_comm_unique_id hands out 128 bytes (include/hq_solver.h)");
static_assert(sizeof(double) == 8 && sizeof(int64_t) == 8, "halo records are ncclFloat64, check words ncclInt64");

static int hq_rccl_load(void)
{
    if (g_rccl.handle) return HQ_OK;
    void* h = dlopen("librccl.so.1", RTLD_NOW | RTLD_GLOBAL);
    if (!h) h = dlopen("librccl.so", RTLD_NOW | RTLD_GLOBAL);
    if (!h) return hq_fail(HQ_ERR_COMM, "cannot load librccl: %s", dlerror());
#define HQ_SYM(field, name)                                                     \
    *(void**)(&g_rccl.field) = dlsym(h, name);                                  \
    if (!g_rccl.field) return hq_fail(HQ_ERR_COMM, "librccl lacks %s", name);
    HQ_SYM(GetUniqueId, "ncclGetUniqueId")
    HQ_SYM(CommInitRank, "ncclCommInitRank")
    HQ_SYM(CommDestroy, "ncclCommDestroy")
    HQ_SYM(Send, "ncclSend")
    HQ_SYM(Recv, "ncclRecv")
    HQ_SYM(GroupStart, "ncclGroupStart")
    HQ_SYM(GroupEnd, "ncclGroupEnd")
    HQ_SYM(GetErrorString, "ncclGetErrorString")
#undef HQ_SYM
    g_rccl.handle = h;
    return HQ_OK;
}

#define HQ_NCCL(call)                                                                     \
    do {                                                                                  \
        ncclResult_t r_ = (call);                                                         \
        if (r_ != ncclSuccess) return hq_fail(HQ_ERR_COMM, "%s: %s", #call, g_rccl.GetErrorString(r_)); \
    } while (0)


struct hq_dev_messenger {
    int32_t procid, nodecount;
    int32_t offset;
};

struct hq_dev_schedule {
    std::vector<hq_dev_messenger> c, s;
    int32_t* d_cmap = nullptr;
    int32_t* d_smap = nullptr;
    int32_t* d_cmap_f = nullptr;
    int32_t* d_smap_f = nullptr;
    double*  d_c_out = nullptr;
    double*  d_c_in = nullptr;
    double*  d_s_out = nullptr;
    double*  d_s_in = nullptr;
    int32_t  ctotal = 0, stotal = 0;
    int64_t* d_c_out_id = nullptr;
    int64_t* d_c_in_id = nullptr;
    int64_t* d_s_out_id = nullptr;
    int64_t* d_s_in_id = nullptr;
    double** d_c_dst = nullptr;
    double** d_s_dst = nullptr;
    double*  h_c_out = nullptr;
    double*  h_c_in = nullptr;
    double*  h_s_out = nullptr;
    double*  h_s_in = nullptr;
    int64_t* h_c_out_id = nullptr;
    int64_t* h_c_in_id = nullptr;
    int64_t* h_s_out_id = nullptr;
    int64_t* h_s_in_id = nullptr;
};

struct hq_ctx {
    hq_options opts;
    int device = 0;
    hipStream_t stream = nullptr;
    int32_t E = 0, N = 0, ldnnum = 0;
    int32_t variant = HQ_VARIANT_SCATTER;
    int32_t step = 0;
    int32_t rank = 0, nranks = 1;
    double dt = 0, dt2 = 0;
    int64_t bytes = 0;
    int64_t h2d_bytes = 0, d2h_bytes = 0;
    int32_t* d_gather_ids = nullptr;
    hq_real* d_gather_out = nullptr;
    int32_t gather_cap = 0;

    int32_t Epad = 0;
    int32_t* d_lnid = nullptr;
    double* d_c1 = nullptr;
    double* d_c2 = nullptr;
    double* d_beta = nullptr;
    double* d_nt = nullptr;
    double* d_nt_rows = nullptr;
    hq_real* d_u[3] = { nullptr, nullptr, nullptr };
    int now = 0, prev = 1, spare = 2;
    double* d_force = nullptr;
    int32_t nloaded = 0, src_step0 = 0, src_nsteps = 0;
    int32_t* d_loaded = nullptr;
    double* d_F = nullptr;
    std::vector<int32_t> h_loaded;
    size_t F_capacity = 0;
    int32_t* d_dn_id = nullptr;
    int32_t* d_dn_ptr = nullptr;
    int32_t* d_dn_anchor = nullptr;
    hq_dev_schedule an, dn;
    hq_nccl_comm comm = nullptr;
    hq_host_exchange_fn host_xchg = nullptr;
    void* host_user = nullptr;
    std::vector<hq_ctx*>* group = nullptr;
    bool group_owner = false;
    bool share_packed = false;
    struct hq_ipc_state* ipc = nullptr;
    hipEvent_t ev_sent = nullptr;
    hipStream_t cstream = nullptr;
    hipEvent_t ev_bnd = nullptr, ev_shared = nullptr, ev_an_shared = nullptr, ev_assigned = nullptr;
    hipStream_t bstream = nullptr;
// ... 1123 lines not shown
    const size_t bytes = sizeof(hq_real) * 3 * (size_t)c->N;
    c->d2h_bytes += (int64_t)bytes;
    if (c->perm.empty()) {
        HQ_HIP(hipMemcpy(host, dev, bytes, hipMemcpyDeviceToHost));
        return HQ_OK;
    }
    std::vector<hq_real> tmp;
    try { tmp.resize(3 * (size_t)c->N); } catch (...) { return hq_fail(HQ_ERR_NOMEM, "out of host memory%s", ""); }
    HQ_HIP(hipMemcpy(tmp.data(), dev, bytes, hipMemcpyDeviceToHost));
    const int32_t* pm = c->perm.data();
#pragma omp parallel for schedule(static) if (c->N > 262144)
    for (int64_t n = 0; n < (int64_t)c->N; n++) {
        const int64_t q = pm[n];
        host[3 * n] = tmp[(size_t)(3 * q)]; host[3 * n + 1] = tmp[(size_t)(3 * q + 1)]; host[3 * n + 2] = tmp[(size_t)(3 * q + 2)];
    }
    return HQ_OK;
}

static int hq_create_impl(const hq_desc* d, int device, const hq_options& opts, hq_ctx** out);

static const double* hq_ntable64(const hq_desc* d, std::vector<double>& store)
{
    if (sizeof(hq_real) == sizeof(double)) return reinterpret_cast<const double*>(d->nTable);
    const size_t n = 7 * (size_t)d->nharbored;
    store.resize(n);
#pragma omp parallel for schedule(static)
    for (int64_t i = 0; i < (int64_t)n; i++) store[(size_t)i] = (double)d->nTable[i];
    return store.data();
}

extern "C" void hq_options_init(hq_options* o, uint64_t size)
{
    if (!o || size < sizeof(uint64_t)) return;
    hq_options full;
    hq_options_defaults(&full);
    memcpy(o, &full, (size_t)std::min<uint64_t>(size, sizeof(full)));
    o->size = std::min<uint64_t>(size, sizeof(full));
}

extern "C" int hq_create_opts(const hq_desc* d, int device, const hq_options* opts, hq_ctx** out)
{
    if (opts && opts->size < sizeof(uint64_t)) return hq_fail(HQ_ERR_ARG, "hq_options.size is not set (hq_options_init)%s", "");
    hq_options full;
    hq_options_resolve(&full, opts);
    return hq_create_impl(d, device, full, out);
}

extern "C" int hq_create(const hq_desc* d, int device, hq_ctx** out) { return hq_create_opts(d, device, nullptr, out); }

extern "C" int hq_get_options(hq_ctx* c, hq_options* out, uint64_t size)
{
    if (!c || !out || size < sizeof(uint64_t)) return hq_fail(HQ_ERR_ARG, "null argument%s", "");
    memcpy(out, &c->opts, (size_t)std::min<uint64_t>(size, sizeof(c->opts)));
    out->size = std::min<uint64_t>(size, sizeof(c->opts));
    return HQ_OK;
}

static int hq_create_impl(const hq_desc* d, int device, const hq_options& opts, hq_ctx** out)
{
    if (!d || !out) return hq_fail(HQ_ERR_ARG, "null argument%s", "");
    *out = nullptr;
    if (d->lenum < 0 || d->nharbored <= 0 || d->ldnnum < 0 || (d->lenum && !d->lnid) || !d->eTable ||
        !d->nTable)
        return hq_fail(HQ_ERR_ARG, "inconsistent mesh description%s", "");
    int ndev = 0;
    if (hipGetDeviceCount(&ndev) != hipSuccess || ndev <= 0)
        return hq_fail(HQ_ERR_NODEVICE, "no HIP device: this engine has no CPU path%s", "");
    if (device < 0 || device >= ndev) return hq_fail(HQ_ERR_ARG, "device index out of range%s", "");
    hipDeviceProp_t prop;
    HQ_HIP(hipGetDeviceProperties(&prop, device));
    if (strncmp(prop.gcnArchName, "gfx950", 6) != 0)
        return hq_fail(HQ_ERR_NODEVICE, "device is %s, kernels are built for gfx950 only", prop.gcnArchName);
    HQ_HIP(hipSetDevice(device));

    hq_ctx* c = new (std::nothrow) hq_ctx();
    if (!c) return hq_fail(HQ_ERR_NOMEM, "out of host memory%s", "");
    c->device = device;
    c->opts = opts;
    c->E = d->lenum; c->N = d->nharbored; c->ldnnum = d->ldnnum;
    c->dt = d->deltaT; c->dt2 = d->deltaT * d->deltaT;
    c->rank = d->rank; c->nranks = d->nranks > 0 ? d->nranks : 1;
    int rc = HQ_OK;
    auto bail = [&](int r) { hq_destroy(c); return r; };

    for (int64_t i = 0; i < (int64_t)c->E * 8; i++)
        if (d->lnid[i] < 0 || d->lnid[i] >= c->N) return bail(hq_fail(HQ_ERR_ARG, "lnid out of range%s", ""));

    if (hipStreamCreateWithFlags(&c->stream, hipStreamNonBlocking) != hipSuccess)
        return bail(hq_fail(HQ_ERR_DEVICE, "hipStreamCreate failed%s", ""));

    int variant = d->variant;
    if (variant == HQ_VARIANT_AUTO) variant = HQ_VARIANT_PATCH;
    if (c->ldnnum && (!d->dn_ldnid || !d->dn_ptr || !d->dn_lanid))
        return bail(hq_fail(HQ_ERR_ARG, "dangling-node tables missing%s", ""));
    for (int32_t k = 0; k < c->ldnnum; k++) {
        if (d->dn_ldnid[k] < 0 || d->dn_ldnid[k] >= c->N || d->dn_ptr[k + 1] <= d->dn_ptr[k])
            return bail(hq_fail(HQ_ERR_ARG, "bad dangling-node table%s", ""));
        for (int32_t a = d->dn_ptr[k]; a < d->dn_ptr[k + 1]; a++)
            if (d->dn_lanid[a] < 0 || d->dn_lanid[a] >= c->N) return bail(hq_fail(HQ_ERR_ARG, "bad anchor id%s", ""));
    }
    if (c->ldnnum) {
        std::vector<char> is_dn((size_t)c->N, 0);
        for (int32_t k = 0; k < c->ldnnum; k++) is_dn[d->dn_ldnid[k]] = 1;
        for (int32_t a = 0; a < d->dn_ptr[c->ldnnum]; a++)
            if (is_dn[d->dn_lanid[a]]) return bail(hq_fail(HQ_ERR_ARG, "an anchor is itself a hanging node%s", ""));
    }
    if (hipEventCreateWithFlags(&c->ev_sent, hipEventDisableTiming) != hipSuccess)
        return bail(hq_fail(HQ_ERR_DEVICE, "hipEventCreate failed%s", ""));
    if (variant != HQ_VARIANT_SCATTER && variant != HQ_VARIANT_PATCH)
        return bail(hq_fail(HQ_ERR_ARG, "unknown variant%s", ""));
    c->variant = variant;

    std::vector<double> c1(c->E), c2(c->E), beta(c->E);
    for (int64_t e = 0; e < c->E; e++) {
        const double* ep = d->eTable + 4 * e;
        c1[e] = ep[0]; c2[e] = ep[1];
        beta[e] = (ep[0] != 0.0) ? ep[2] / ep[0] : ((ep[1] != 0.0) ? ep[3] / ep[1] : 0.0);
        const double lhs = ep[2] * ep[1], rhs = ep[3] * ep[0];
        if (fabs(lhs - rhs) > 1e-12 * std::max(fabs(lhs), fabs(rhs)))
            return bail(hq_fail(HQ_ERR_ARG, "eTable is not Rayleigh-proportional (c3/c1 != c4/c2): not the table solver_init builds%s", ""));
    }


    if (variant == HQ_VARIANT_PATCH && !d->node_xyz) {
        static bool warned = false;
        if (!warned && !hq_set(opts.quiet)) {
            warned = true;
            fprintf(stderr, "hq_create: hq_desc.node_xyz is NULL -- no bricks, no lattice / stencil patches (fixed runs of the node "
                            "order, element-form kernels only): expect about a third of the throughput; pass node_t.x/y/z\n");
        }
    }
    const bool verbose = hq_set(opts.verbose);
    auto t_last = std::chrono::steady_clock::now();
    auto lap = [&](const char* what) {
        if (!verbose) return;
        const auto now = std::chrono::steady_clock::now();
        fprintf(stderr, "hq_create: %-34s %7.2f s\n", what, std::chrono::duration<double>(now - t_last).count());
        t_last = now;
    };
    hq_desc dd = *d;
    std::vector<int32_t> p_lnid, p_xyz, p_dn_id, p_dn_anchor;
    std::vector<double> p_nt, nt64;
    const double* ntab = hq_ntable64(d, nt64);
    std::vector<int64_t> p_gnid;
    std::vector<std::vector<int32_t>> p_maps;
    std::vector<hq_messenger> p_msg[4];
    hq_brick_host BH;
    const hq_real *h_tm1 = d->tm1, *h_tm2 = d->tm2;
    if (variant == HQ_VARIANT_PATCH && d->node_xyz && !hq_set(opts.no_bricks)) {
        std::vector<char> excl;
        if ((rc = hq_brick_excluded(d, excl)) != HQ_OK) return bail(rc);
        hq_mat_src ms;
        ms.edata = d->edata; ms.dt = d->deltaT; ms.bbase = d->mat_bbase; ms.thr_damp = d->mat_threshold_damping; ms.thr_vpvs = d->mat_threshold_vpvs;
        if (hq_brick_plan_host(opts, c->E, c->N, d->lnid, d->node_xyz, c1.data(), c2.data(), beta.data(), ntab, excl.data(), &BH, &ms) != 0)
            return bail(hq_fail(HQ_ERR_ARG, "brick plan: %s", hq_patch_error()));
        lap("brick plan");
    }
    if (BH.nb > 0) {
        const std::vector<int32_t>& pm = BH.perm;
        const int64_t N = c->N;
        p_lnid.resize((size_t)c->E * 8);
#pragma omp parallel for schedule(static)
        for (int64_t i = 0; i < (int64_t)c->E * 8; i++) p_lnid[(size_t)i] = pm[(size_t)d->lnid[i]];
        p_xyz.resize((size_t)N * 3);
        p_nt.resize((size_t)N * 7);
#pragma omp parallel for schedule(static)
        for (int64_t n = 0; n < N; n++) {
            const int64_t q = pm[(size_t)n];
            for (int k = 0; k < 3; k++) p_xyz[(size_t)(3 * q + k)] = d->node_xyz[3 * n + k];
            for (int k = 0; k < 7; k++) p_nt[(size_t)(7 * q + k)] = ntab[7 * n + k];
        }
        dd.lnid = p_lnid.data(); dd.node_xyz = p_xyz.data(); dd.nTable = nullptr; ntab = p_nt.data();
        std::vector<double>().swap(nt64);
        if (d->node_gnid) {
            p_gnid.resize((size_t)N);
            for (int64_t n = 0; n < N; n++) p_gnid[(size_t)pm[(size_t)n]] = d->node_gnid[n];
            dd.node_gnid = p_gnid.data();
        }
        if (c->ldnnum) {
            const int32_t na = d->dn_ptr[c->ldnnum];
            p_dn_id.resize((size_t)c->ldnnum); p_dn_anchor.resize((size_t)na);
            for (int32_t k = 0; k < c->ldnnum; k++) p_dn_id[(size_t)k] = pm[(size_t)d->dn_ldnid[k]];
            for (int32_t a = 0; a < na; a++) p_dn_anchor[(size_t)a] = pm[(size_t)d->dn_lanid[a]];
            dd.dn_ldnid = p_dn_id.data(); dd.dn_lanid = p_dn_anchor.data();
        }
        {
            const hq_schedule* in[2] = { &d->an_sched, &d->dn_sched };
            hq_schedule* out[2] = { &dd.an_sched, &dd.dn_sched };
            size_t nm = 0;
            for (int s2 = 0; s2 < 2; s2++) nm += (size_t)in[s2]->c_count + (size_t)in[s2]->s_count;
            p_maps.reserve(nm);
            for (int s2 = 0; s2 < 2; s2++)
                for (int side = 0; side < 2; side++) {
                    const int32_t cnt = side ? in[s2]->s_count : in[s2]->c_count;
                    const hq_messenger* list = side ? in[s2]->first_s : in[s2]->first_c;
                    std::vector<hq_messenger>& v = p_msg[2 * s2 + side];
                    for (int32_t i = 0; i < cnt; i++) {
                        p_maps.emplace_back((size_t)list[i].nodecount);
                        for (int32_t k = 0; k < list[i].nodecount; k++) p_maps.back()[(size_t)k] = pm[(size_t)list[i].mapping[k]];
                        v.push_back({ list[i].procid, list[i].nodecount, p_maps.back().data() });
                    }
                    if (side) out[s2]->first_s = v.data(); else out[s2]->first_c = v.data();
                }
        }
        dd.tm1 = dd.tm2 = nullptr;
        c->perm = BH.perm;
        d = &dd;
        lap("renumbering");
    }

    size_t n3 = (size_t)c->N * 3;
    int nbuf = (variant == HQ_VARIANT_PATCH) ? 3 : 2;
    for (int b = 0; b < nbuf; b++) {
        if ((rc = hq_dev_alloc(c, &c->d_u[b], n3)) != HQ_OK) return bail(rc);
        if (hipMemset(c->d_u[b], 0, sizeof(hq_real) * n3) != hipSuccess) return bail(hq_fail(HQ_ERR_DEVICE, "memset%s", ""));
    }
    {
        const int64_t nt_first = (variant == HQ_VARIANT_PATCH) ? BH.nb : 0;
        const size_t rows = (size_t)std::max<int64_t>(c->N - nt_first, 1);
        if ((rc = hq_dev_alloc(c, &c->d_nt_rows, rows * 7)) != HQ_OK) return bail(rc);
        if (c->N > nt_first &&
            hipMemcpy(c->d_nt_rows, ntab + 7 * nt_first, sizeof(double) * 7 * (size_t)(c->N - nt_first), hipMemcpyHostToDevice) != hipSuccess)
            return bail(hq_fail(HQ_ERR_DEVICE, "nTable upload failed%s", ""));
        c->d_nt = c->d_nt_rows - 7 * nt_first;
    }
    lap("state buffers, n_t rows");
    if (h_tm1 && (rc = hq_field_to_device(c, h_tm1, c->d_u[c->now])) != HQ_OK) return bail(rc);
    if (h_tm2 && (rc = hq_field_to_device(c, h_tm2, c->d_u[c->prev])) != HQ_OK) return bail(rc);
    lap("start fields");

    if (c->ldnnum) {
        int32_t na = d->dn_ptr[c->ldnnum];
        if ((rc = hq_dev_alloc(c, &c->d_dn_id, (size_t)c->ldnnum)) != HQ_OK) return bail(rc);
        if ((rc = hq_dev_alloc(c, &c->d_dn_ptr, (size_t)c->ldnnum + 1)) != HQ_OK) return bail(rc);
        if ((rc = hq_dev_alloc(c, &c->d_dn_anchor, (size_t)na)) != HQ_OK) return bail(rc);
        if (hipMemcpy(c->d_dn_id, d->dn_ldnid, sizeof(int32_t) * c->ldnnum, hipMemcpyHostToDevice) != hipSuccess ||
            hipMemcpy(c->d_dn_ptr, d->dn_ptr, sizeof(int32_t) * (c->ldnnum + 1), hipMemcpyHostToDevice) != hipSuccess ||
            hipMemcpy(c->d_dn_anchor, d->dn_lanid, sizeof(int32_t) * na, hipMemcpyHostToDevice) != hipSuccess)
            return bail(hq_fail(HQ_ERR_DEVICE, "dangling-node table upload failed%s", ""));
    }

    if ((rc = hq_dev_alloc(c, &c->d_halo_err, 4)) != HQ_OK) return bail(rc);
    if (hipMemset(c->d_halo_err, 0, 4 * sizeof(int32_t)) != hipSuccess) return bail(hq_fail(HQ_ERR_DEVICE, "memset%s", ""));
    if (hq_set(opts.debug_halo) && c->nranks > 1) {
        if (!d->node_gnid && !d->node_xyz)
            return bail(hq_fail(HQ_ERR_ARG, "HQ_DEBUG_HALO needs hq_desc.node_gnid or node_xyz%s", ""));
        std::vector<int64_t> key((size_t)c->N);
        for (int64_t n = 0; n < c->N; n++) {
            if (d->node_gnid) { key[(size_t)n] = d->node_gnid[n]; continue; }
            uint64_t h = 0x9E3779B97F4A7C15ull;
            for (int k = 0; k < 3; k++) {
                h ^= (uint64_t)(uint32_t)d->node_xyz[3 * n + k];
                h *= 0xBF58476D1CE4E5B9ull; h ^= h >> 29;
            }
            key[(size_t)n] = (int64_t)h;
        }
        if ((rc = hq_dev_alloc(c, &c->d_gkey, (size_t)c->N)) != HQ_OK) return bail(rc);
        if (hipMemcpy(c->d_gkey, key.data(), sizeof(int64_t) * (size_t)c->N, hipMemcpyHostToDevice) != hipSuccess)
            return bail(hq_fail(HQ_ERR_DEVICE, "node identity upload failed%s", ""));
        c->debug_halo = true;
    }

    if (variant == HQ_VARIANT_SCATTER) {
        if ((rc = hq_dev_alloc(c, &c->d_force, n3)) != HQ_OK) return bail(rc);
        if (hipMemset(c->d_force, 0, sizeof(double) * n3) != hipSuccess) return bail(hq_fail(HQ_ERR_DEVICE, "memset%s", ""));
        c->Epad = (c->E + 63) & ~63;
        std::vector<int32_t> soa((size_t)8 * c->Epad, 0);
        for (int64_t e = 0; e < c->E; e++)
            for (int n = 0; n < 8; n++) soa[(size_t)n * c->Epad + e] = d->lnid[8 * e + n];
        if ((rc = hq_dev_alloc(c, &c->d_lnid, soa.size())) != HQ_OK) return bail(rc);
        if ((rc = hq_dev_alloc(c, &c->d_c1, (size_t)c->E)) != HQ_OK) return bail(rc);
        if ((rc = hq_dev_alloc(c, &c->d_c2, (size_t)c->E)) != HQ_OK) return bail(rc);
        if ((rc = hq_dev_alloc(c, &c->d_beta, (size_t)c->E)) != HQ_OK) return bail(rc);
        if (hipMemcpy(c->d_lnid, soa.data(), sizeof(int32_t) * soa.size(), hipMemcpyHostToDevice) != hipSuccess ||
            hipMemcpy(c->d_c1, c1.data(), sizeof(double) * c->E, hipMemcpyHostToDevice) != hipSuccess ||
            hipMemcpy(c->d_c2, c2.data(), sizeof(double) * c->E, hipMemcpyHostToDevice) != hipSuccess ||
            hipMemcpy(c->d_beta, beta.data(), sizeof(double) * c->E, hipMemcpyHostToDevice) != hipSuccess)
            return bail(hq_fail(HQ_ERR_DEVICE, "element table upload failed%s", ""));
        if ((rc = hq_build_schedule(c, &d->an_sched, &c->an)) != HQ_OK) return bail(rc);
        if ((rc = hq_build_schedule(c, &d->dn_sched, &c->dn)) != HQ_OK) return bail(rc);
        if (c->ldnnum) {
            std::vector<int32_t> sd;
            for (int32_t k = 0; k < c->ldnnum; k++)
                for (int32_t a = d->dn_ptr[k]; a < d->dn_ptr[k + 1]; a++) {
                    sd.push_back(d->dn_ldnid[k]); sd.push_back(d->dn_lanid[a]); sd.push_back(d->dn_ptr[k + 1] - d->dn_ptr[k]);
                }
            if ((rc = hq_build_distribution(c, sd)) != HQ_OK) return bail(rc);
        }
    } else {
        int64_t pb = 0;
        std::vector<char> shared_dn((size_t)c->N, 0);
        for (int32_t i = 0; i < d->dn_sched.s_count; i++)
            for (int32_t k = 0; k < d->dn_sched.first_s[i].nodecount; k++) {
                int32_t n = d->dn_sched.first_s[i].mapping[k];
                if (n < 0 || n >= c->N) return bail(hq_fail(HQ_ERR_ARG, "messenger node id out of range%s", ""));
                shared_dn[n] = 1;
            }
        std::vector<int32_t> l_id, l_ptr(1, 0), l_anc;
        for (int32_t k = 0; k < c->ldnnum; k++) {
            if (shared_dn[d->dn_ldnid[k]]) continue;
            l_id.push_back(d->dn_ldnid[k]);
            for (int32_t a = d->dn_ptr[k]; a < d->dn_ptr[k + 1]; a++) l_anc.push_back(d->dn_lanid[a]);
            l_ptr.push_back((int32_t)l_anc.size());
        }
        hq_dangling dn;
        dn.n = (int32_t)l_id.size(); dn.id = l_id.data(); dn.ptr = l_ptr.data(); dn.anchor = l_anc.data();
        std::vector<char> seed0((size_t)c->N, 0);
// ... 120 lines not shown
    }
    report[0] = (int64_t)H.desc.size(); report[1] = nlat; report[2] = (int64_t)H.pelem.size();
    report[3] = H.ndistinct; report[4] = passes; report[5] = instr;
    report[6] = lpasses; report[7] = bad;
    if (bad) return hq_fail(HQ_ERR_STATE, "patch plan self-check failed%s", "");
    return HQ_OK;
}

extern "C" int hq_stencil_coefficients(double out[16])
{
    if (!out) return hq_fail(HQ_ERR_ARG, "null argument%s", "");
    const hq_stencil_tab& t = hq_stencil();
    for (int i = 0; i < 6; i++) { out[i] = t.c.p1[i]; out[6 + i] = t.c.p2[i]; }
    for (int i = 0; i < 2; i++) { out[12 + i] = t.c.q1[i]; out[14 + i] = t.c.q2[i]; }
    return t.ok ? HQ_OK : hq_fail(HQ_ERR_STATE, "the assembled stencil lacks the cube symmetry%s", "");
}

extern "C" int hq_stencil_plan_check(const hq_desc* d, int64_t report[6])
{
    hq_options opts;
    hq_options_resolve(&opts, nullptr);
    if (!d || !report || d->lenum < 0 || d->nharbored <= 0 || (d->lenum && !d->lnid) || !d->node_xyz)
        return hq_fail(HQ_ERR_ARG, "inconsistent mesh description (node_xyz is needed)%s", "");
    const int64_t E = d->lenum, N = d->nharbored;
    for (int64_t i = 0; i < E * 8; i++)
        if (d->lnid[i] < 0 || d->lnid[i] >= N) return hq_fail(HQ_ERR_ARG, "lnid out of range%s", "");
    std::vector<char> shared_dn((size_t)N, 0);
    for (int32_t i = 0; i < d->dn_sched.s_count; i++)
        for (int32_t k = 0; k < d->dn_sched.first_s[i].nodecount; k++) shared_dn[d->dn_sched.first_s[i].mapping[k]] = 1;
    std::vector<int32_t> l_id, l_ptr(1, 0), l_anc;
    for (int32_t k = 0; k < d->ldnnum; k++) {
        if (shared_dn[d->dn_ldnid[k]]) continue;
        l_id.push_back(d->dn_ldnid[k]);
        for (int32_t a = d->dn_ptr[k]; a < d->dn_ptr[k + 1]; a++) l_anc.push_back(d->dn_lanid[a]);
        l_ptr.push_back((int32_t)l_anc.size());
    }
    hq_dangling dn;
    dn.n = (int32_t)l_id.size(); dn.id = l_id.data(); dn.ptr = l_ptr.data(); dn.anchor = l_anc.data();
    bool want_lattice = false;
    const hq_patch_cfg cfg = hq_patch_cfg_of(opts, dn.n > 0, true, &want_lattice);
    hq_patch_host H;
    if (hq_patch_plan_host(opts, cfg, E, N, d->lnid, d->node_xyz, dn, want_lattice, &H) != 0)
        return hq_fail(HQ_ERR_ARG, "patch plan: %s", hq_patch_error());
    int64_t ntab = 0, nfull = 0, nbnd_tot = 0, ncorner = 0, bad = 0;
#pragma omp parallel for schedule(dynamic, 64) reduction(+ : ntab, nfull, nbnd_tot, ncorner, bad)
    for (int64_t p = 0; p < (int64_t)H.desc.size(); p++) {
        const hq_patch_desc& D = H.desc[(size_t)p];
        if (D.nacc != D.nown) continue;
        if (!H.ds_ptr.empty() && H.ds_ptr[(size_t)p + 1] > H.ds_ptr[(size_t)p]) continue;
        std::vector<int32_t> h(H.halo.begin() + D.halo_off, H.halo.begin() + D.halo_off + D.nhalo);
        std::vector<uint32_t> tab;
        int32_t nbnd = 0;
        if (!hq_ragged_match(D.base, D.nown, d->lnid, d->node_xyz, &H.pelem[(size_t)D.pair_off], D.npairs, h, tab, &nbnd)) continue;
        ntab++;
        nbnd_tot += nbnd;
        if (nbnd == 0 && D.nown == HQ_LAT_NOWN && D.nhalo == HQ_LAT_NHALO && D.npairs == HQ_LAT_NELEM) nfull++;
        const int32_t nloc = D.nown + D.nhalo;
        if ((int32_t)tab.size() < nloc + nbnd) { bad++; continue; }
        std::unordered_map<int32_t, int32_t> local_of;
        std::vector<char> used(HQ_ST_ROWS, 0);
        for (int32_t t = 0; t < nloc; t++) {
            local_of[t < D.nown ? D.base + t : h[(size_t)(t - D.nown)]] = t;
            const int r = HQ_RG_ROW(tab[(size_t)t]);
            if (r >= HQ_ST_ROWS || used[(size_t)r]) bad++; else used[(size_t)r] = 1;
        }
        std::vector<unsigned> want((size_t)D.nown, 0u);
        for (int32_t q = 0; q < D.npairs; q++) {
            const int32_t* id = d->lnid + 8 * (int64_t)H.pelem[(size_t)D.pair_off + q];
            auto it0 = local_of.find(id[0]);
            if (it0 == local_of.end()) { bad++; continue; }
            const int r0 = HQ_RG_ROW(tab[(size_t)it0->second]);
            for (int c = 0; c < 8; c++) {
                auto it = local_of.find(id[c]);
                if (it == local_of.end()) { bad++; continue; }
                const int r = HQ_RG_ROW(tab[(size_t)it->second]);
                if (r != r0 + HQ_ST_PX * (c & 1) + HQ_ST_PY * ((c >> 1) & 1) + HQ_ST_PZ * ((c >> 2) & 1)) bad++;
                if (it->second < D.nown) want[(size_t)it->second] |= 1u << c;
                ncorner++;
            }
        }
        int32_t nb = 0;
        for (int32_t t = 0; t < D.nown; t++) {
            const uint32_t w = tab[(size_t)t];
            if (HQ_RG_MASK(w) != want[(size_t)t]) bad++;
            if (want[(size_t)t] != 0xffu) {
                if (nb >= nbnd || HQ_RG_BIDX(w) != nb) bad++;
                else {
                    const uint32_t b = tab[(size_t)(nloc + nb)];
                    if (HQ_RG_ROW(b) != HQ_RG_ROW(w) || HQ_RG_MASK(b) != want[(size_t)t]) bad++;
                }
                nb++;
            }
        }
        if (nb != nbnd) bad++;
    }
    {
        const hq_stencil_tab& T = hq_stencil();
        if (!T.ok) bad++;
        uint64_t seed = 88172645463325252ull;
        auto rnd = [&]() { seed ^= seed << 13; seed ^= seed >> 7; seed ^= seed << 17; return (double)(seed >> 11) / 9007199254740992.0 - 0.5; };
        for (int trial = 0; trial < 64; trial++) {
            const double c1 = 1.0 + rnd(), c2 = 2.0 + rnd();
            const unsigned mask = (unsigned)(trial * 37 + 1) & 0xffu;
            double w[27][3];
            for (auto& r : w) for (double& v : r) v = rnd();
            double ref[3] = { 0, 0, 0 }, got[3] = { 0, 0, 0 };
            for (int o = 0; o < 8; o++) {
                if (!((mask >> o) & 1)) continue;
                double X[8], Y[8], Z[8];
                for (int m = 0; m < 8; m++) {
                    const int dx = (m & 1) - (o & 1), dy = ((m >> 1) & 1) - ((o >> 1) & 1), dz = ((m >> 2) & 1) - ((o >> 2) & 1);
                    const double* q = w[(dx + 1) + 3 * (dy + 1) + 9 * (dz + 1)];
                    X[m] = q[0]; Y[m] = q[1]; Z[m] = q[2];
                    for (int a = 0; a < 3; a++)
                        for (int b = 0; b < 3; b++) {
                            const int k = ((o * 8 + m) * 3 + a) * 3 + b;
                            got[a] += (c1 * T.E1[k] + c2 * T.E2[k]) * q[b];
                        }
                }
                hq_element_force(X, Y, Z, c1, c2);
                ref[0] += X[o]; ref[1] += Y[o]; ref[2] += Z[o];
            }
            for (int a = 0; a < 3; a++)
                if (fabs(got[a] - ref[a]) > 1e-12 * (fabs(ref[a]) + 1.0)) bad++;
        }
    }
    report[0] = (int64_t)H.desc.size(); report[1] = ntab; report[2] = nfull; report[3] = nbnd_tot; report[4] = ncorner;
    report[5] = bad;
    if (bad) return hq_fail(HQ_ERR_STATE, "stencil table self-check failed%s", "");
    return HQ_OK;
}

static int hq_brick_excluded(const hq_desc* d, std::vector<char>& excl)
{
    excl.assign((size_t)d->nharbored, 0);
    for (int32_t k = 0; k < d->ldnnum; k++) {
        excl[d->dn_ldnid[k]] = 1;
        for (int32_t a = d->dn_ptr[k]; a < d->dn_ptr[k + 1]; a++) excl[d->dn_lanid[a]] = 1;
    }
    for (const hq_schedule* sc : { &d->an_sched, &d->dn_sched })
        for (int side = 0; side < 2; side++) {
            const int32_t cnt = side ? sc->s_count : sc->c_count;
            const hq_messenger* list = side ? sc->first_s : sc->first_c;
            for (int32_t i = 0; i < cnt; i++)
                for (int32_t k = 0; k < list[i].nodecount; k++) {
                    const int32_t n = list[i].mapping ? list[i].mapping[k] : -1;
                    if (n < 0 || n >= d->nharbored) return hq_fail(HQ_ERR_ARG, "messenger node id out of range%s", "");
                    excl[n] = 1;
                }
        }
    return HQ_OK;
}

static thread_local int64_t g_brick_check_extra[4];

extern "C" int hq_brick_plan_check(const hq_desc* d, int64_t report[8])
{
    hq_options opts;
    hq_options_resolve(&opts, nullptr);
    if (!d || !report || d->lenum < 0 || d->nharbored <= 0 || (d->lenum && !d->lnid) || !d->node_xyz || !d->eTable || !d->nTable)
        return hq_fail(HQ_ERR_ARG, "inconsistent mesh description (node_xyz is needed)%s", "");
    const int64_t E = d->lenum, N = d->nharbored;
    for (int64_t i = 0; i < E * 8; i++)
        if (d->lnid[i] < 0 || d->lnid[i] >= N) return hq_fail(HQ_ERR_ARG, "lnid out of range%s", "");
    std::vector<double> c1((size_t)E), c2((size_t)E), beta((size_t)E);
    for (int64_t e = 0; e < E; e++) {
        const double* ep = d->eTable + 4 * e;
        c1[(size_t)e] = ep[0]; c2[(size_t)e] = ep[1];
        beta[(size_t)e] = (ep[0] != 0.0) ? ep[2] / ep[0] : ((ep[1] != 0.0) ? ep[3] / ep[1] : 0.0);
    }
    std::vector<char> excl;
    HQ_TRY(hq_brick_excluded(d, excl));
    hq_brick_host B;
    hq_mat_src ms;
    ms.edata = d->edata; ms.dt = d->deltaT; ms.bbase = d->mat_bbase; ms.thr_damp = d->mat_threshold_damping; ms.thr_vpvs = d->mat_threshold_vpvs;
    std::vector<double> nt64;
    const double* ntab = hq_ntable64(d, nt64);
    if (hq_brick_plan_host(opts, E, N, d->lnid, d->node_xyz, c1.data(), c2.data(), beta.data(), ntab, excl.data(), &B, &ms) != 0)
        return hq_fail(HQ_ERR_ARG, "brick plan: %s", hq_patch_error());
    int64_t bad = 0, nchecked = 0;
    for (int k = 0; k < 8; k++) report[k] = 0;
    report[6] = N;
    if (B.nb == 0) return HQ_OK;
    std::vector<int32_t> inv((size_t)N, -1);
    for (int64_t n = 0; n < N; n++) {
        const int32_t q = B.perm[(size_t)n];
        if (q < 0 || q >= N || inv[(size_t)q] != -1) { bad++; continue; }
        inv[(size_t)q] = (int32_t)n;
    }
    std::vector<int64_t> aptr((size_t)N + 1, 0);
    for (int64_t i = 0; i < E * 8; i++) aptr[(size_t)d->lnid[i] + 1]++;
    for (int64_t n = 0; n < N; n++) aptr[(size_t)n + 1] += aptr[(size_t)n];
    std::vector<int64_t> adj((size_t)(E * 8));
    {
        std::vector<int64_t> fill(aptr.begin(), aptr.end() - 1);
        for (int64_t i = 0; i < E * 8; i++) adj[(size_t)fill[(size_t)d->lnid[i]]++] = i;
    }
    std::vector<int32_t> covered((size_t)B.nb, 0);
    int64_t nsame = 0;
#pragma omp parallel for schedule(dynamic, 4) reduction(+ : bad, nchecked, nsame)
    for (int64_t u = 0; u < (int64_t)B.units.size(); u++) {
        const hq_brick_unit& U = B.units[(size_t)u];
        const int nx = U.nx, ny = U.ny, np = U.np, nr = 2 * (nx + 2) + 2 * ny;
        const bool het = (U.flags & HQ_BK_HET) != 0, rag = (U.flags & HQ_BK_RAGGED) != 0;
        if (nx < 1 || nx > (het ? HQ_BH_TX : HQ_BK_TX) || ny < 1 || ny > (het ? HQ_BH_TY : HQ_BK_TY) || np < 1 || U.base < 0 ||
            (!rag && U.base + (int64_t)nx * ny * np > B.nb)) { bad++; continue; }
        nsame += (U.flags & HQ_BK_NTSAME) != 0;
        if (((U.flags & HQ_BK_NTSAME) != 0) != (u < B.nsame)) bad++;
        const int64_t nu = (int64_t)B.units.size();
        if ((rag && !het) != (u >= B.nsame - B.nrag && u < B.nsame) || (rag && (U.flags & (HQ_BK_TOPFACE | HQ_BK_BOTFACE)))) { bad++; continue; }
        if ((rag && het) != (u >= nu - B.nrhet)) { bad++; continue; }
        if (het != (u >= nu - B.nhet - B.nrhet)) bad++;
        if (het && ((U.flags & HQ_BK_PACKED) != 0) != (rag ? u >= nu - B.nrpacked : (u >= nu - B.nrhet - B.npacked && u < nu - B.nrhet))) bad++;
        if (het && (U.coef < 0 || U.coef + (int64_t)(np + 1) * HQ_BH_THREADS * 3 > (int64_t)B.coef.size())) { bad++; continue; }
        const int32_t* ring = B.tab.data() + U.tab;
        const int32_t* cap = ring + (int64_t)(np + 2) * nr;
        auto at = [&](int x, int y, int k) -> int64_t {
            const bool in = x >= 0 && x < nx && y >= 0 && y < ny;
            if (in && rag) {
                const int32_t v = cap[(int64_t)(k + 1) * nx * ny + y * nx + x];
                return v >= 0 ? v : (v == -1 ? -1 : -(int64_t)v - 2);
            }
            if (in) {
                if (k >= 0 && k < np) return U.base + ((int64_t)k * ny + y) * nx + x;
                return cap[(k < 0 ? 0 : nx * ny) + y * nx + x];
            }
            const int32_t* r = ring + (int64_t)(k + 1) * nr;
            if (y == -1) return r[x + 1];
            if (y == ny) return r[nx + 2 + x + 1];
            if (x == -1) return r[2 * (nx + 2) + y];
            return r[2 * (nx + 2) + ny + y];
        };
        int64_t next = U.base;
        for (int k = 0; k < np; k++)
            for (int y = 0; y < ny; y++)
                for (int x = 0; x < nx; x++) {
                    int64_t q = U.base + ((int64_t)k * ny + y) * nx + x;
                    if (rag) {
                        const int32_t v = cap[(int64_t)(k + 1) * nx * ny + y * nx + x];
                        if (v < 0) continue;
                        if (v != next++ || v >= B.nb) { bad++; continue; }
                        q = v;
                    }
#pragma omp atomic
                    covered[(size_t)q]++;
                    const int32_t n = inv[(size_t)q];
                    if (n < 0) { bad++; continue; }
                    if (excl[(size_t)n]) bad++;
                    const double* t7 = ntab + 7 * (int64_t)n;
                    if (!((t7[1] == t7[2]) && (t7[1] == t7[3]) && (t7[4] == t7[5]) && (t7[4] == t7[6]))) bad++;
                    if ((U.flags & HQ_BK_NTSAME) && (t7[0] != U.m0 || t7[1] != U.m2 || t7[4] != U.m1)) bad++;
                    int64_t el[8];
                    for (int o = 0; o < 8; o++) el[o] = -1;
                    if (aptr[(size_t)n + 1] - aptr[(size_t)n] != 8) { bad++; continue; }
                    bool ok = true;
                    for (int64_t a = aptr[(size_t)n]; a < aptr[(size_t)n + 1]; a++) {
                        const int64_t e = adj[(size_t)a] >> 3;
                        const int o = (int)(adj[(size_t)a] & 7);
                        if (el[o] != -1) ok = false;
                        el[o] = e;
                        if (het) {
                            const int i = x - (o & 1) + 1, j = y - ((o >> 1) & 1) + 1, l = k - ((o >> 2) & 1) + 1;
                            const double* q = B.coef.data() + U.coef + (int64_t)l * (3 * HQ_BH_THREADS) + (j * 64 + i);
                            if (c1[(size_t)e] != q[0] || c2[(size_t)e] != q[HQ_BH_CS] || beta[(size_t)e] != q[2 * HQ_BH_CS]) ok = false;
                        } else if (c1[(size_t)e] != U.c1 || c2[(size_t)e] != U.c2 || beta[(size_t)e] != U.beta) ok = false;
                    }
                    if (!ok) { bad++; continue; }
                    for (int dz = -1; dz <= 1; dz++)
                        for (int dy = -1; dy <= 1; dy++)
                            for (int dx = -1; dx <= 1; dx++) {
                                if (!dx && !dy && !dz) continue;
                                const int o = (dx < 0 ? 1 : 0) | (dy < 0 ? 2 : 0) | (dz < 0 ? 4 : 0);
                                const int m = (dx > 0 ? 1 : 0) | (dy > 0 ? 2 : 0) | (dz > 0 ? 4 : 0);
                                const int32_t nb_abi = d->lnid[8 * el[o] + m];
                                if (at(x + dx, y + dy, k + dz) != (int64_t)B.perm[(size_t)nb_abi]) bad++;
                                nchecked++;
                            }
                }
    }
#pragma omp parallel for schedule(dynamic, 4) reduction(+ : bad, nchecked)
    for (int64_t u = 0; u < (int64_t)B.units.size(); u++) {
        const hq_brick_unit& U = B.units[(size_t)u];
        const int nx = U.nx, ny = U.ny, np = U.np, nr = 2 * (nx + 2) + 2 * ny;
        if (!(U.flags & (HQ_BK_TOPFACE | HQ_BK_BOTFACE))) continue;
        if ((U.flags & HQ_BK_HET) || !(U.flags & HQ_BK_NTSAME)) { bad++; continue; }
        const int32_t* ring = B.tab.data() + U.tab;
        const int32_t* cap = ring + (int64_t)(np + 2) * nr;
        auto at = [&](int x, int y, int k) -> int64_t {
            const bool in = x >= 0 && x < nx && y >= 0 && y < ny;
            if (in) {
                if (k >= 0 && k < np) return U.base + ((int64_t)k * ny + y) * nx + x;
                return cap[(k < 0 ? 0 : nx * ny) + y * nx + x];
            }
            const int32_t* r = ring + (int64_t)(k + 1) * nr;
            if (y == -1) return r[x + 1];
            if (y == ny) return r[nx + 2 + x + 1];
            if (x == -1) return r[2 * (nx + 2) + y];
            return r[2 * (nx + 2) + ny + y];
        };
        for (int side = 0; side < 2; side++) {
            if (!(U.flags & (side ? HQ_BK_BOTFACE : HQ_BK_TOPFACE))) continue;
            const double* row = side ? U.fb : U.ft;
            const int kf = side ? np : -1;
            for (int y = 0; y < ny; y++)
                for (int x = 0; x < nx; x++) {
                    const int64_t q = U.base + ((int64_t)(side ? np : -1) * ny + y) * nx + x;
                    if (q < 0 || q >= B.nb) { bad++; continue; }
#pragma omp atomic
                    covered[(size_t)q]++;
                    if (at(x, y, kf) != q) bad++;
                    const int32_t n = inv[(size_t)q];
                    if (n < 0) { bad++; continue; }
                    if (excl[(size_t)n]) bad++;
                    if (memcmp(ntab + 7 * (int64_t)n, row, 7 * sizeof(double)) != 0) bad++;
                    int64_t el[8];
                    for (int o = 0; o < 8; o++) el[o] = -1;
                    if (aptr[(size_t)n + 1] - aptr[(size_t)n] != 4) { bad++; continue; }
                    bool ok = true;
                    for (int64_t a = aptr[(size_t)n]; a < aptr[(size_t)n + 1]; a++) {
                        const int64_t e = adj[(size_t)a] >> 3;
                        const int o = (int)(adj[(size_t)a] & 7);
                        if (((o >> 2) & 1) != side || el[o] != -1) ok = false;
                        el[o] = e;
                        if (c1[(size_t)e] != U.c1 || c2[(size_t)e] != U.c2 || beta[(size_t)e] != U.beta) ok = false;
                    }
                    if (!ok) { bad++; continue; }
                    for (int dz = (side ? -1 : 0); dz <= (side ? 0 : 1); dz++)
                        for (int dy = -1; dy <= 1; dy++)
                            for (int dx = -1; dx <= 1; dx++) {
                                if (!dx && !dy && !dz) continue;
                                const int o = (dx < 0 ? 1 : 0) | (dy < 0 ? 2 : 0) | (side ? 4 : 0);
                                const int m = (dx > 0 ? 1 : 0) | (dy > 0 ? 2 : 0) | ((side ? dz == 0 : dz > 0) ? 4 : 0);
                                const int32_t nb_abi = d->lnid[8 * el[o] + m];
                                if (at(x + dx, y + dy, kf + dz) != (int64_t)B.perm[(size_t)nb_abi]) bad++;
                                nchecked++;
                            }
                }
        }
    }
    for (int64_t q = 0; q < B.nb; q++) if (covered[(size_t)q] != 1) bad++;
    {
        std::vector<int32_t> p_lnid((size_t)E * 8), p_xyz((size_t)N * 3);
        for (int64_t i = 0; i < E * 8; i++) p_lnid[(size_t)i] = B.perm[(size_t)d->lnid[i]];
        for (int64_t n = 0; n < N; n++)
            for (int k = 0; k < 3; k++) p_xyz[(size_t)(3 * (int64_t)B.perm[(size_t)n] + k)] = d->node_xyz[3 * n + k];
        std::vector<char> shared_dn((size_t)N, 0);
        for (int32_t i = 0; i < d->dn_sched.s_count; i++)
            for (int32_t k = 0; k < d->dn_sched.first_s[i].nodecount; k++) shared_dn[(size_t)d->dn_sched.first_s[i].mapping[k]] = 1;
        std::vector<int32_t> l_id, l_ptr(1, 0), l_anc;
        for (int32_t k = 0; k < d->ldnnum; k++) {
            if (shared_dn[(size_t)d->dn_ldnid[k]]) continue;
            l_id.push_back(B.perm[(size_t)d->dn_ldnid[k]]);
            for (int32_t a = d->dn_ptr[k]; a < d->dn_ptr[k + 1]; a++) l_anc.push_back(B.perm[(size_t)d->dn_lanid[a]]);
            l_ptr.push_back((int32_t)l_anc.size());
        }
        hq_dangling dn;
        dn.n = (int32_t)l_id.size(); dn.id = l_id.data(); dn.ptr = l_ptr.data(); dn.anchor = l_anc.data();
        bool want_lattice = false;
        const hq_patch_cfg cfg = hq_patch_cfg_of(opts, dn.n > 0, true, &want_lattice);
        hq_patch_host Ha, Hb;
        std::vector<int32_t> all((size_t)E);
        for (int64_t e = 0; e < E; e++) all[(size_t)e] = (int32_t)e;
        if (hq_patch_plan_host(opts, cfg, E, N, p_lnid.data(), p_xyz.data(), dn, false, &Ha, B.nb) != 0 ||
            hq_patch_plan_host(opts, cfg, E, N, p_lnid.data(), p_xyz.data(), dn, false, &Hb, B.nb, &all) != 0)
            return hq_fail(HQ_ERR_ARG, "patch plan: %s", hq_patch_error());
        if (Ha.pelem != Hb.pelem || Ha.halo != Hb.halo || Ha.pidx != Hb.pidx || Ha.desc.size() != Hb.desc.size() || Ha.ds_ent != Hb.ds_ent) bad++;
        for (size_t q = 0; q < Ha.desc.size() && q < Hb.desc.size(); q++)
            if (Ha.desc[q].base != Hb.desc[q].base || Ha.desc[q].nown != Hb.desc[q].nown || Ha.desc[q].npairs != Hb.desc[q].npairs ||
                Ha.desc[q].nhalo != Hb.desc[q].nhalo || Ha.desc[q].pair_off != Hb.desc[q].pair_off) bad++;
        std::vector<int32_t> patch_of((size_t)N, -1);
        for (size_t q = 0; q < Ha.desc.size(); q++)
            for (int32_t n = Ha.desc[q].base; n < Ha.desc[q].base + Ha.desc[q].nown; n++) patch_of[(size_t)n] = (int32_t)q;
        for (int64_t n = B.nb; n < N; n++) if (patch_of[(size_t)n] < 0) bad++;
        int64_t need = 0, have = 0;
        for (int64_t e = 0; e < E; e++) {
            int32_t seen[8]; int ns = 0;
            for (int c8 = 0; c8 < 8; c8++) {
                const int32_t q = patch_of[(size_t)p_lnid[(size_t)(8 * e + c8)]];
                bool dup = q < 0;
                for (int t = 0; t < ns; t++) dup |= seen[t] == q;
                if (!dup) seen[ns++] = q;
            }
            for (int t = 0; t < ns; t++) {
                need++;
                const hq_patch_desc& D = Ha.desc[(size_t)seen[t]];
                have += std::binary_search(Ha.pelem.begin() + D.pair_off, Ha.pelem.begin() + D.pair_off + D.npairs, (int32_t)e);
            }
        }
        if (have != need) bad++;
    }
    report[0] = B.nb; report[1] = B.ncolumns; report[2] = (int64_t)B.units.size(); report[3] = nsame;
    report[4] = B.nhet + B.nrhet; report[5] = nchecked; report[6] = N - B.nb; report[7] = bad;
    g_brick_check_extra[0] = B.nrag;
    g_brick_check_extra[1] = 0;
    g_brick_check_extra[2] = B.nrhet;
    g_brick_check_extra[3] = 0;
    for (const hq_brick_unit& U : B.units) {
        if (!(U.flags & HQ_BK_RAGGED)) continue;
        const int32_t* pl = B.tab.data() + U.tab + (int64_t)(U.np + 2) * (2 * (U.nx + 2) + 2 * U.ny);
        for (int64_t i = (int64_t)U.nx * U.ny; i < (int64_t)U.nx * U.ny * (U.np + 1); i++) g_brick_check_extra[(U.flags & HQ_BK_HET) ? 3 : 1] += pl[i] >= 0;
    }
    if (bad) return hq_fail(HQ_ERR_STATE, "brick plan self-check failed%s", "");
    return HQ_OK;
}

extern "C" int hq_brick_plan_check_n(const hq_desc* d, int64_t* report, int32_t n)
{
    int64_t r8[8] = { 0, 0, 0, 0, 0, 0, 0, 0 };
    if (!report || n < 8) return hq_fail(HQ_ERR_ARG, "hq_brick_plan_check_n: a report of at least 8 entries%s", "");
    for (int k = 0; k < 4; k++) g_brick_check_extra[k] = 0;
    const int rc = hq_brick_plan_check(d, r8);
    for (int k = 0; k < 8; k++) report[k] = r8[k];
    for (int k = 8; k < n; k++) report[k] = k < 12 ? g_brick_check_extra[k - 8] : 0;
    return rc;
}

extern "C" int hq_destroy(hq_ctx* c)
{
    if (!c) return HQ_OK;
    hipSetDevice(c->device);
    if (c->stream) hq_quiesce(c);
    if (c->comm && g_rccl.handle) g_rccl.CommDestroy(c->comm);
    if (c->ipc) {
        hq_ipc_state* I = c->ipc;
        for (int x = 0; x < 4; x++) {
            hq_dev_schedule* sc = x < 2 ? &c->an : &c->dn;
            if (x & 1) sc->d_c_in = nullptr; else sc->d_s_in = nullptr;
            if (I->d_dst[x]) hipFree(I->d_dst[x]);
            if (I->d_sig[x]) hipFree(I->d_sig[x]);
            if (I->d_dst_id[x]) hipFree(I->d_dst_id[x]);
        }
        for (void* p : I->opened) hipIpcCloseMemHandle(p);
        if (I->d_done) hipFree(I->d_done);
        if (I->arena) hipFree(I->arena);
        delete I;
        c->ipc = nullptr;
    }
    void* ptrs[] = { c->d_gather_ids, c->d_gather_out, c->d_lnid, c->d_c1, c->d_c2, c->d_beta, c->d_nt_rows, c->d_u[0], c->d_u[1], c->d_u[2],
                     c->d_force, c->d_loaded, c->d_F, c->d_dn_id, c->d_dn_ptr, c->d_dn_anchor,
                     c->an.d_cmap, c->an.d_smap, c->an.d_c_out, c->an.d_c_in, c->an.d_s_out, c->an.d_s_in,
                     c->dn.d_cmap, c->dn.d_smap, c->dn.d_c_out, c->dn.d_c_in, c->dn.d_s_out, c->dn.d_s_in,
                     c->d_iforce, c->d_oi_node, c->d_oi_slot, c->d_oi_ptr, c->d_oi_pos, c->d_oi_fc, c->d_sd_dst, c->d_sd_ptr, c->d_sd_src, c->d_sd_deps,
                     c->d_gkey, c->d_halo_err, c->an.d_c_out_id, c->an.d_c_in_id, c->an.d_s_out_id, c->an.d_s_in_id,
                     c->dn.d_c_out_id, c->dn.d_c_in_id, c->dn.d_s_out_id, c->dn.d_s_in_id };
    for (void* p : ptrs) if (p) hipFree(p);
    if (c->an.d_cmap_f && c->an.d_cmap_f != c->an.d_cmap) hipFree(c->an.d_cmap_f);
    if (c->an.d_smap_f && c->an.d_smap_f != c->an.d_smap) hipFree(c->an.d_smap_f);
    if (c->dn.d_cmap_f && c->dn.d_cmap_f != c->dn.d_cmap) hipFree(c->dn.d_cmap_f);
    if (c->dn.d_smap_f && c->dn.d_smap_f != c->dn.d_smap) hipFree(c->dn.d_smap_f);
    for (hq_dev_schedule* sc : { &c->an, &c->dn }) {
        for (double* hp : { sc->h_c_out, sc->h_c_in, sc->h_s_out, sc->h_s_in })
            if (hp) hipHostFree(hp);
        for (int64_t* hp : { sc->h_c_out_id, sc->h_c_in_id, sc->h_s_out_id, sc->h_s_in_id })
            if (hp) hipHostFree(hp);
        if (sc->d_c_dst) hipFree(sc->d_c_dst);
        if (sc->d_s_dst) hipFree(sc->d_s_dst);
    }
    if (c->ev_sent) hipEventDestroy(c->ev_sent);
    if (c->cstream) { hipStreamSynchronize(c->cstream); hipStreamDestroy(c->cstream); }
    if (c->bstream) { hipStreamSynchronize(c->bstream); hipStreamDestroy(c->bstream); }
    for (auto& sl : c->clock) for (hipEvent_t e : sl.e) if (e) hipEventDestroy(e);
    if (c->ev_patches) hipEventDestroy(c->ev_patches);
    if (c->ev_bricks) hipEventDestroy(c->ev_bricks);
    if (c->ev_bnd) hipEventDestroy(c->ev_bnd);
    if (c->ev_shared) hipEventDestroy(c->ev_shared);
    if (c->ev_an_shared) hipEventDestroy(c->ev_an_shared);
    if (c->ev_assigned) hipEventDestroy(c->ev_assigned);
    if (c->group) {
        std::vector<hq_ctx*>* g = c->group;
        bool any = false;
        for (auto& m : *g) { if (m == c) m = nullptr; any |= (m != nullptr); }
        if (!any) delete g;
    }
    hq_patch_free(&c->plan);
    hq_brick_free(&c->bricks);
    for (hipEvent_t e : c->ev) hipEventDestroy(e);
    for (int k = 0; k < 2; k++) if (c->ev_span[k]) hipEventDestroy(c->ev_span[k]);
    if (c->stream) hipStreamDestroy(c->stream);
    delete c;
    return HQ_OK;
}

extern "C" int hq_real_bytes(void) { return (int)sizeof(hq_real); }

extern "C" int hq_abi_version(void) { return HQ_ABI_VERSION; }

extern "C" int hq_get_info_sized(hq_ctx* c, hq_info* info, uint64_t size)
{
    if (!c || !info) return hq_fail(HQ_ERR_ARG, "null argument%s", "");
    hq_info v;
    memset(&v, 0, sizeof(v));
    v.variant = c->variant;
    v.npatches = c->plan.npatches;
    v.patch_pairs = c->plan.npairs;
    v.device_bytes = c->bytes;
    v.step = c->step;
    v.nranks = c->nranks;
    v.lattice_patches = c->plan.nlattice;
    v.stencil_patches = c->plan.nstencil;
    v.ragged_patches = c->plan.nragged;
    v.brick_units = c->bricks.nunits;
    v.brick_nodes = c->bricks.nb;
    v.brick_units_pernode = c->bricks.nunits - c->bricks.nsame - c->bricks.nhet - c->bricks.nrhet;
    v.brick_units_het = c->bricks.nhet + c->bricks.nrhet;
    v.brick_units_packed = c->bricks.npacked + c->bricks.nrpacked;
    v.brick_units_ragged = c->bricks.nrag;
    v.brick_units_ragged_het = c->bricks.nrhet;
    v.pcie_h2d_bytes = c->h2d_bytes;
    v.pcie_d2h_bytes = c->d2h_bytes;
    v.transport = c->comm ? 1 : (hq_ipc_ready(c) ? (c->ipc->loopback ? 5 : 2) : (c->host_xchg ? 3 : (c->group ? 4 : 0)));
    v.ipc_arena_coarse = (c->ipc && c->ipc->coarse) ? 1 : 0;
    v.ipc_arena_kind = c->ipc ? c->ipc->arena_kind : 0;
    v.debug_halo = c->debug_halo ? 1 : 0;
    v.brick_stream = c->bstream ? 1 : 0;
    hq_clock_harvest_all(c, false);
    v.timed_steps = c->clk_steps;
    if (c->clk_steps > 0) {
        const double n = (double)c->clk_steps;
        v.t_step_us = c->clk_us[0] / n; v.t_shell_us = c->clk_us[1] / n; v.t_interior_us = c->clk_us[2] / n;
        v.t_chain_us = c->clk_us[3] / n; v.t_chain_exposed_us = c->clk_us[4] / n;
    }
    memset(info, 0, (size_t)size);
    memcpy(info, &v, (size_t)std::min<uint64_t>(size, sizeof(v)));
    return HQ_OK;
}

extern "C" int hq_get_info(hq_ctx* c, hq_info* info) { return hq_get_info_sized(c, info, 56); }

static int hq_mask_compute_stream(hq_ctx* c)
{
    if (!c->overlap || c->reserve_cus <= 0 || c->stream_masked) return HQ_OK;
    if (!hq_set(c->opts.cu_mask)) return HQ_OK;
    hipDeviceProp_t prop;
    HQ_HIP(hipGetDeviceProperties(&prop, c->device));
    const int ncu = prop.multiProcessorCount;
    if (c->reserve_cus >= ncu) return HQ_OK;
    std::vector<uint32_t> mask((size_t)(ncu + 31) / 32, 0u);
    for (int i = 0; i < ncu; i++) mask[(size_t)i / 32] |= 1u << (i % 32);
    for (int k = 0; k < c->reserve_cus; k++) {
        const int i = (33 * k) % ncu;
        mask[(size_t)i / 32] &= ~(1u << (i % 32));
    }
    hipStream_t ns = nullptr;
    if (hipExtStreamCreateWithCUMask(&ns, (uint32_t)mask.size(), mask.data()) != hipSuccess) {
        (void)hipGetLastError();
        return HQ_OK;
    }
    HQ_HIP(hq_quiesce(c));
    hipStreamDestroy(c->stream);
    c->stream = ns;
    c->stream_masked = true;
    c->plan.grid_cus = std::max(8, (ncu - c->reserve_cus) & ~7);
    return HQ_OK;
}

extern "C" int hq_comm_unique_id(void* id128)
{
    if (!id128) return hq_fail(HQ_ERR_ARG, "null argument%s", "");
    HQ_TRY(hq_rccl_load());
    hq_nccl_id id;
    HQ_NCCL(g_rccl.GetUniqueId(&id));
    memcpy(id128, &id, sizeof id);
    return HQ_OK;
}

extern "C" int hq_comm_init(hq_ctx* c, const void* id128)
// ... 663 lines not shown
```

### hercules_amd/csrc/hq_opts.h

```cpp
#ifndef HQ_OPTS_H
#define HQ_OPTS_H

#include <cstddef>
#include <cstdlib>
#include <cstring>

struct hq_opt_entry { const char* env; size_t off; int kind; };

#define HQ_OPT_I(env_, field_) { env_, offsetof(hq_options, field_), 0 }
#define HQ_OPT_D(env_, field_) { env_, offsetof(hq_options, field_), 1 }
static const hq_opt_entry g_opt_table[] = {
    HQ_OPT_I("HQ_NO_BRICKS", no_bricks), HQ_OPT_I("HQ_BRICK_CZ", brick_cz), HQ_OPT_I("HQ_BRICK_MINZ", brick_minz),
    HQ_OPT_I("HQ_BRICK_MINNODES", brick_minnodes), HQ_OPT_I("HQ_BRICK_NO_HET", brick_no_het),
    HQ_OPT_I("HQ_BRICK_NO_NTSAME", brick_no_ntsame), HQ_OPT_I("HQ_BRICK_BY_COMPONENT", brick_by_component),
    HQ_OPT_I("HQ_BRICK_STREAM", brick_stream), HQ_OPT_I("HQ_BRICK_NO_FACES", brick_no_faces), HQ_OPT_I("HQ_BRICK_HALF_TILES", brick_half_tiles), HQ_OPT_I("HQ_BRICK_NO_PACK", brick_no_pack), HQ_OPT_I("HQ_PATCH_PIPE", patch_pipe), HQ_OPT_I("HQ_PATCH_THREADS", patch_threads),
    HQ_OPT_I("HQ_PATCH_PMAX", patch_pmax), HQ_OPT_I("HQ_PATCH_PMERGE", patch_pmerge), HQ_OPT_I("HQ_PATCH_PSPLIT", patch_psplit),
    HQ_OPT_I("HQ_PATCH_NLMAX", patch_nlmax), HQ_OPT_I("HQ_PATCH_VMAX", patch_vmax), HQ_OPT_I("HQ_PATCH_RAGGED", patch_ragged),
    HQ_OPT_I("HQ_PATCH_NO_LATTICE", patch_no_lattice), HQ_OPT_I("HQ_PATCH_NO_STENCIL", patch_no_stencil),
    HQ_OPT_I("HQ_PATCH_NO_UNIFORM", patch_no_uniform), HQ_OPT_I("HQ_PATCH_NO_ISO", patch_no_iso),
    HQ_OPT_I("HQ_PATCH_NO_NTSAME", patch_no_ntsame), HQ_OPT_I("HQ_PATCH_NO_DEDUP", patch_no_dedup),
    HQ_OPT_I("HQ_PATCH_WFORM", patch_wform), HQ_OPT_I("HQ_PATCH_MERGE_ROUNDS", patch_merge_rounds),
    HQ_OPT_I("HQ_OVERLAP", overlap), HQ_OPT_I("HQ_NO_OVERLAP", no_overlap), HQ_OPT_I("HQ_RESERVE_CUS", reserve_cus),
    HQ_OPT_I("HQ_CU_MASK", cu_mask), HQ_OPT_I("HQ_NO_FUSED_SHARE", no_fused_share), HQ_OPT_I("HQ_GROUP_COPIES", group_copies),
    HQ_OPT_I("HQ_DEBUG_HALO", debug_halo), HQ_OPT_I("HQ_IPC_ARENA", ipc_arena), HQ_OPT_D("HQ_IPC_TIMEOUT_MS", ipc_timeout_ms),
    HQ_OPT_D("HQ_LOOPBACK_DELAY_US", loopback_delay_us), HQ_OPT_I("HQ_PATCH_VERBOSE", verbose), HQ_OPT_I("HQ_QUIET", quiet),
    HQ_OPT_I("HQ_BRICK_RAGGED", brick_ragged), HQ_OPT_I("HQ_BRICK_RAGGED_MINFILL", brick_ragged_minfill),
    HQ_OPT_I("HQ_PHASE_TIMING", phase_timing), HQ_OPT_I("HQ_BRICK_RAGGED_HET", brick_ragged_het),
};
#undef HQ_OPT_I
#undef HQ_OPT_D

static void hq_options_defaults(hq_options* o)
{
    o->size = sizeof(hq_options);
    for (const hq_opt_entry& e : g_opt_table) {
        if (e.kind == 0) *(int32_t*)((char*)o + e.off) = -1;
        else *(double*)((char*)o + e.off) = -1.0;
    }
    o->allow_env = -1;
    o->reserved0 = -1;
}

static void hq_options_adopt(hq_options* dst, const hq_options* src)
{
    hq_options_defaults(dst);
    if (!src) return;
    const size_t n = (size_t)(src->size < sizeof(hq_options) ? src->size : sizeof(hq_options));
    if (n > sizeof(uint64_t)) memcpy((char*)dst + sizeof(uint64_t), (const char*)src + sizeof(uint64_t), n - sizeof(uint64_t));
    dst->size = sizeof(hq_options);
}

static int hq_opt_env_int(const char* env, const char* v)
{
    if (!strcmp(env, "HQ_IPC_ARENA")) return !strcmp(v, "fine") ? 0 : (!strcmp(v, "uncached") ? 1 : (!strcmp(v, "coarse") ? 2 : atoi(v)));
    if (!*v) return 1;
    return atoi(v);
}

static void hq_options_resolve(hq_options* out, const hq_options* caller)
{
    hq_options_adopt(out, caller);
    const char* master = getenv("HQ_ALLOW_ENV");
    const bool allow = out->allow_env >= 0 ? out->allow_env != 0 : (master && *master && strcmp(master, "0") != 0);
    out->allow_env = allow ? 1 : 0;
    if (!allow) return;
    for (const hq_opt_entry& e : g_opt_table) {
        const char* v = getenv(e.env);
        if (!v) continue;
        if (e.kind == 0) *(int32_t*)((char*)out + e.off) = hq_opt_env_int(e.env, v);
        else if (*v) *(double*)((char*)out + e.off) = atof(v);
    }
}

template <typename T> static inline bool hq_given(T f) { return f >= 0; }
template <typename T> static inline T hq_value_or(T f, T def) { return f >= 0 ? f : def; }
template <typename T> static inline bool hq_set(T f) { return f > 0; }

static inline const char* hq_opt_env_only(const hq_options& o, const char* env)
{
    return o.allow_env == 1 ? getenv(env) : nullptr;
}

#endif
```

### include/hq_solver.h

```cpp
#ifndef HQ_SOLVER_H
#define HQ_SOLVER_H

#include <stdint.h>

#ifdef __cplusplus
extern "C" {
#endif

#define HQ_API __attribute__((visibility("default")))

typedef struct hq_ctx hq_ctx;

typedef enum {
    HQ_OK            =  0,
    HQ_ERR_ARG       = -1,
    HQ_ERR_NOMEM     = -2,
    HQ_ERR_DEVICE    = -3,
    HQ_ERR_NODEVICE  = -4,
    HQ_ERR_COMM      = -5,
    HQ_ERR_STATE     = -6
} hq_status;

enum {
    HQ_VARIANT_AUTO    = 0,
    HQ_VARIANT_SCATTER = 1,
    HQ_VARIANT_PATCH   = 2
};

typedef struct {
    int32_t        procid;
    int32_t        nodecount;
    const int32_t* mapping;
} hq_messenger;

#ifdef HQ_SINGLE_PRECISION_SOLVER
typedef float hq_real;
#else
typedef double hq_real;
#endif

typedef struct {
    int32_t             c_count;
    const hq_messenger* first_c;
    int32_t             s_count;
    const hq_messenger* first_s;
} hq_schedule;

typedef struct {
    int32_t        lenum;
    int32_t        nharbored;
    int32_t        ldnnum;
    const int32_t* lnid;
    const int32_t* node_xyz;
    const int32_t* dn_ldnid;
    const int32_t* dn_ptr;
    const int32_t* dn_lanid;
    const double*  eTable;
    const hq_real* nTable;
    const hq_real* tm1;
    const hq_real* tm2;
    hq_schedule    an_sched;
    hq_schedule    dn_sched;
    double         deltaT;
    int32_t        rank, nranks;
    int32_t        variant;
    int32_t        reserved;
    const int64_t* node_gnid;
    const float*  edata;
    double mat_bbase;
    double mat_threshold_damping;
    double mat_threshold_vpvs;
} hq_desc;

typedef struct {
    int32_t variant;
    int32_t npatches;
    int64_t patch_pairs;
    int64_t device_bytes;
    int32_t step;
    int32_t nranks;
    int32_t lattice_patches;
    int32_t stencil_patches;
    int32_t ragged_patches;
    int32_t brick_units;
    int64_t brick_nodes;
    int32_t brick_units_pernode;
    int32_t brick_units_het;
    int64_t pcie_h2d_bytes;
    int64_t pcie_d2h_bytes;
    int32_t transport;
    int32_t ipc_arena_coarse;
    int32_t ipc_arena_kind;
    int32_t debug_halo;
    int32_t brick_units_packed;
    int32_t brick_units_ragged;
    int32_t brick_stream;
    int32_t brick_units_ragged_het;
    int64_t timed_steps;
    double  t_step_us;
    double  t_shell_us;
    double  t_interior_us;
    double  t_chain_us;
    double  t_chain_exposed_us;
} hq_info;

HQ_API int hq_device_count(void);

HQ_API const char* hq_last_error(void);

HQ_API int hq_create(const hq_desc* desc, int device, hq_ctx** out);

typedef struct {
    uint64_t size;
    int32_t no_bricks;
    int32_t brick_cz;
    int32_t brick_minz;
    int32_t brick_minnodes;
    int32_t brick_no_het;
    int32_t brick_no_ntsame;
    int32_t brick_by_component;
    int32_t brick_stream;
    int32_t brick_no_faces;
    int32_t brick_half_tiles;
    int32_t brick_no_pack;
    int32_t patch_pipe;
    int32_t patch_threads;
    int32_t patch_pmax;
    int32_t patch_pmerge;
    int32_t patch_psplit;
    int32_t patch_nlmax;
    int32_t patch_vmax;
    int32_t patch_ragged;
    int32_t patch_no_lattice;
    int32_t patch_no_stencil;
    int32_t patch_no_uniform;
    int32_t patch_no_iso;
    int32_t patch_no_ntsame;
    int32_t patch_no_dedup;
    int32_t patch_wform;
    int32_t patch_merge_rounds;
    int32_t overlap;
    int32_t no_overlap;
    int32_t reserve_cus;
    int32_t cu_mask;
    int32_t no_fused_share;
    int32_t group_copies;
    int32_t debug_halo;
    int32_t ipc_arena;
    double  ipc_timeout_ms;
    double  loopback_delay_us;
    int32_t verbose;
    int32_t quiet;
    int32_t brick_ragged;
    int32_t brick_ragged_minfill;
    int32_t allow_env;
    int32_t brick_ragged_het;
    int32_t reserved0;
    int32_t phase_timing;
} hq_options;

HQ_API void hq_options_init(hq_options* opts, uint64_t size);
HQ_API int  hq_create_opts(const hq_desc* desc, int device, const hq_options* opts, hq_ctx** out);
HQ_API int  hq_get_options(hq_ctx* ctx, hq_options* out, uint64_t size);

HQ_API int hq_destroy(hq_ctx* ctx);

#define HQ_ABI_VERSION 6
HQ_API int hq_abi_version(void);
HQ_API int hq_real_bytes(void);
HQ_API int hq_get_info_sized(hq_ctx* ctx, hq_info* info, uint64_t size);
HQ_API int hq_get_info(hq_ctx* ctx, hq_info* info);
#ifndef HQ_SOLVER_IMPLEMENTATION
#define hq_get_info(ctx, info) hq_get_info_sized((ctx), (info), (uint64_t)sizeof(hq_info))
#endif

HQ_API int hq_comm_unique_id(void* id128);
HQ_API int hq_comm_init(hq_ctx* ctx, const void* id128);
HQ_API int hq_comm_selftest(hq_ctx* ctx, int32_t count);

typedef int (*hq_host_exchange_fn)(void* user, int32_t nrecv, const int32_t* recv_peer, const int64_t* recv_count,
                                   double* const* recv_buf, int32_t nsend, const int32_t* send_peer,
                                   const int64_t* send_count, const double* const* send_buf, int32_t tag);
HQ_API int hq_comm_init_host(hq_ctx* ctx, hq_host_exchange_fn fn, void* user);

#define HQ_IPC_BLOB_BYTES 4096
HQ_API int hq_comm_ipc_export(hq_ctx* ctx, void* blob);
HQ_API int hq_comm_init_ipc(hq_ctx* ctx, const void* all_blobs);
HQ_API int hq_comm_init_ipc_n(hq_ctx* ctx, const void* all_blobs, int32_t nblobs);
HQ_API int hq_comm_init_loopback(hq_ctx* ctx);

HQ_API int hq_group_link(hq_ctx** ctxs, int32_t n);
HQ_API int hq_group_run(hq_ctx** ctxs, int32_t n, int32_t nsteps);

HQ_API int hq_set_source(hq_ctx* ctx, int32_t nloaded, const int32_t* loaded_lnid,
                         int32_t step0, int32_t nsteps, const double* F);

HQ_API int hq_run(hq_ctx* ctx, int32_t nsteps);

HQ_API int hq_sync(hq_ctx* ctx);

HQ_API int hq_check_finite(hq_ctx* ctx, int64_t* nonfinite);

HQ_API int hq_gather(hq_ctx* ctx, int32_t n, const int32_t* lnid, hq_real* tm1_out, hq_real* tm2_out);
HQ_API int hq_gather3(hq_ctx* ctx, int32_t n, const int32_t* lnid, hq_real* tm1_out, hq_real* tm2_out,
                      hq_real* tm3_out);
HQ_API int hq_download(hq_ctx* ctx, hq_real* tm1, hq_real* tm2);
HQ_API int hq_upload(hq_ctx* ctx, const hq_real* tm1, const hq_real* tm2, int32_t step);

HQ_API int hq_phase_force(hq_ctx* ctx);
HQ_API int hq_phase_update(hq_ctx* ctx);
HQ_API int hq_download_force(hq_ctx* ctx, double* force);

HQ_API int hq_run_timed(hq_ctx* ctx, int32_t nsteps, double* total_ms, double* kernel_ms_avg);

HQ_API int hq_plan_check(const hq_desc* desc, int64_t report[8]);

HQ_API int hq_stencil_plan_check(const hq_desc* desc, int64_t report[6]);

HQ_API int hq_brick_plan_check(const hq_desc* desc, int64_t report[8]);
HQ_API int hq_brick_plan_check_n(const hq_desc* desc, int64_t* report, int32_t n);

HQ_API int hq_stencil_coefficients(double out[16]);

HQ_API const char* hq_dominant_kernel(hq_ctx* ctx);

#ifdef __cplusplus
}
#endif
#endif
```

Before: 63.34 billion.

## Chain consecutive brick units per column and compute arithmetic ring ids

Groups consecutive one-n_t-row brick units of the same column into chains that a single workgroup walks in sequence. Each next unit reuses the planes already held in LDS instead of reloading its top and bottom cap planes, and chains start at staggered offsets per XCD. Ring neighbour ids whose table rows form an arithmetic progression are now computed from a stride rather than loaded from the table, which cuts index traffic. The trade-offs are fewer, longer workgroups when chain length reduces parallelism, a more complex kernel control flow, and extra plan self-checks.

```diff
diff --git a/hercules_amd/capi.py b/hercules_amd/capi.py
--- a/hercules_amd/capi.py
+++ b/hercules_amd/capi.py
@@ -79,8 +79,8 @@
                 [("ipc_timeout_ms", ctypes.c_double), ("loopback_delay_us", ctypes.c_double),
                  ("verbose", ctypes.c_int32), ("quiet", ctypes.c_int32),
                  ("brick_ragged", ctypes.c_int32), ("brick_ragged_minfill", ctypes.c_int32),
-                 ("allow_env", ctypes.c_int32), ("brick_ragged_het", ctypes.c_int32), ("reserved0", ctypes.c_int32),
-                 ("phase_timing", ctypes.c_int32)])
+                 ("allow_env", ctypes.c_int32), ("brick_ragged_het", ctypes.c_int32), ("brick_chain", ctypes.c_int32),
+                 ("phase_timing", ctypes.c_int32), ("brick_ring_arith", ctypes.c_int32)])
 
     def __init__(self, **kw):
         super().__init__()
@@ -346,7 +346,8 @@
 
 
 BRICK_PLAN_REPORT = ("brick_nodes", "columns", "units", "units_one_nt_row", "het_units", "neighbours_checked",
-                     "patch_nodes", "faults", "ragged_units", "ragged_nodes", "ragged_het_units", "ragged_het_nodes")
+                     "patch_nodes", "faults", "ragged_units", "ragged_nodes", "ragged_het_units", "ragged_het_nodes",
+                     "chains", "chained_units", "chain_interior_caps", "ring_arith_units", "cap_planes_loaded")
 
 
 def brick_plan_check(desc):
diff --git a/hercules_amd/csrc/hq_brick.h b/hercules_amd/csrc/hq_brick.h
--- a/hercules_amd/csrc/hq_brick.h
+++ b/hercules_amd/csrc/hq_brick.h
@@ -21,6 +21,7 @@
 #define HQ_BK_TOPFACE 8
 #define HQ_BK_BOTFACE 16
 #define HQ_BK_RAGGED 32
+#define HQ_BK_RINGARITH 64
 #define HQ_BK_PACKED 4
 #ifndef HQ_BH_WAVES
 #define HQ_BH_WAVES 8
@@ -43,6 +44,17 @@
     int64_t coef;
 };
 
+struct hq_brick_chain { int32_t first, n, start, pad; };
+
+static __host__ __device__ __forceinline__ int hq_brick_chain_step(int n, int start, int i, bool* cont, bool* more)
+{
+    int j = start + i;
+    if (j >= n) j -= n;
+    *cont = i > 0 && j > 0;
+    *more = i + 1 < n && j + 1 < n;
+    return j;
+}
+
 struct hq_brick_cfg {
     int cz = 32;
     int minz = 4;
@@ -50,6 +62,8 @@
     int ragged = 1;
     int minfill = 128;
     int ragged_het = 1;
+    int chain = -1;
+    int ring_arith = 1;
 };
 
 static hq_brick_cfg hq_brick_cfg_of(const hq_options& o)
@@ -61,6 +75,8 @@
     c.ragged = hq_value_or(o.brick_ragged, c.ragged) != 0;
     c.minfill = std::min(HQ_BK_THREADS, std::max(1, hq_value_or(o.brick_ragged_minfill, c.minfill)));
     c.ragged_het = hq_value_or(o.brick_ragged_het, c.ragged_het) != 0;
+    c.chain = hq_given(o.brick_chain) ? o.brick_chain : -1;
+    c.ring_arith = hq_value_or(o.brick_ring_arith, c.ring_arith) != 0;
     return c;
 }
 
@@ -78,11 +94,16 @@
     int32_t npacked = 0;
     int32_t nrhet = 0, nrpacked = 0;
     int32_t ncolumns = 0, nlevels = 0;
+    std::vector<hq_brick_chain> chains;
+    int32_t nchained = 0;
+    int32_t narith = 0;
 };
 
 struct hq_brick_plan {
     int64_t nb = 0;
     int32_t nunits = 0, nsame = 0, nrag = 0, nhet = 0, npacked = 0, nrhet = 0, nrpacked = 0;
+    int32_t nchains = 0, nchained = 0;
+    hq_brick_chain* d_chains = nullptr;
     hq_brick_unit* d_units = nullptr;
     int32_t* d_tab = nullptr;
     double* d_coef = nullptr;
@@ -96,6 +117,16 @@
     std::vector<int64_t> h_size;
     std::vector<int64_t> h_first;
 };
+
+static bool hq_brick_ring_is_arith(const int32_t* t, int32_t np, int32_t nr)
+{
+    for (int32_t r = 0; r < nr; r++) {
+        const int64_t r0 = t[r], st = (int64_t)t[nr + r] - r0;
+        for (int32_t k = 2; k < np + 2; k++)
+            if ((int64_t)t[(int64_t)k * nr + r] != r0 + k * st) return false;
+    }
+    return true;
+}
 
 struct hq_mat_src {
     const float* edata = nullptr;
@@ -654,6 +685,7 @@
                     if (q[0] != q0[0] || q[1] != q0[1] || q[4] != q0[4]) { sm = false; break; }
                 }
         if (sm && !c.het && !hq_set(o.brick_no_ntsame)) { U.flags |= HQ_BK_NTSAME; same[(size_t)u] = 1; }
+        if ((U.flags & HQ_BK_NTSAME) && cfg.ring_arith && np >= 2 && hq_brick_ring_is_arith(t, np, nr)) U.flags |= HQ_BK_RINGARITH;
         U.m0 = q0[0]; U.m2 = q0[1]; U.m1 = q0[4];
         U.coef = 0;
         }
@@ -728,9 +760,68 @@
     if (fault) { g_patch_err = "brick plan: a neighbour of a simple node is missing"; return -1; }
     {
         std::vector<hq_brick_unit> a, r, b, h, hp, rh, rhp;
+        std::vector<hq_brick_unit> ch;
+        {
+            std::vector<std::vector<int32_t>> of_col(cols.size());
+            for (size_t u = 0; u < us.size(); u++) if (same[u] == 1) of_col[(size_t)us[u].col].push_back((int32_t)u);
+            int64_t nfree = 0;
+            for (size_t u = 0; u < us.size(); u++) nfree += same[u] != 1;
+            std::vector<int32_t> elig;
+            int32_t longest = 1;
+            for (size_t ci = 0; ci < cols.size(); ci++) {
+                std::vector<int32_t>& v = of_col[ci];
+                if (v.empty()) continue;
+                const int32_t nch = (cols[ci].nz + cz - 1) / cz;
+                bool ok = (int32_t)v.size() == nch;
+                std::sort(v.begin(), v.end(), [&](int32_t x, int32_t y) { return us[(size_t)x].za < us[(size_t)y].za; });
+                const hq_brick_unit& U0 = B->units[(size_t)v[0]];
+                for (size_t i = 0; i < v.size() && ok; i++) {
+                    const hq_brick_unit& U = B->units[(size_t)v[i]];
+                    ok = U.np >= 2 && U.c1 == U0.c1 && U.c2 == U0.c2 && U.beta == U0.beta && U.m0 == U0.m0 && U.m2 == U0.m2 && U.m1 == U0.m1 &&
+                         (i == 0 || (us[(size_t)v[i]].za == us[(size_t)v[i - 1]].za + us[(size_t)v[i - 1]].np &&
+                                     U.base == B->units[(size_t)v[i - 1]].base + (int64_t)U.nx * U.ny * B->units[(size_t)v[i - 1]].np));
+                }
+                if (!ok) { nfree += (int64_t)v.size(); v.clear(); continue; }
+                elig.push_back((int32_t)ci);
+                longest = std::max(longest, nch);
+            }
+            int32_t L = cfg.chain;
+            if (L < 0) {
+                for (L = longest; L > 1; L--) {
+                    int64_t n = nfree;
+                    for (int32_t ci : elig) n += ((int64_t)of_col[(size_t)ci].size() + L - 1) / L;
+                    if (n >= 512) break;
+                }
+            }
+            if (L > 1) {
+                struct chain_t { int64_t key; int32_t col, i0, n; };
+                std::vector<chain_t> cs;
+                for (int32_t ci : elig) {
+                    const std::vector<int32_t>& v = of_col[(size_t)ci];
+                    const int32_t nch = (int32_t)v.size(), parts = (nch + L - 1) / L;
+                    for (int32_t q = 0; q < parts; q++) {
+                        const int32_t i0 = (int32_t)((int64_t)nch * q / parts), i1 = (int32_t)((int64_t)nch * (q + 1) / parts);
+                        cs.push_back({ us[(size_t)v[(size_t)i0]].key, ci, i0, i1 - i0 });
+                    }
+                }
+                std::stable_sort(cs.begin(), cs.end(), [](const chain_t& x, const chain_t& y) { return x.key < y.key; });
+                const bool lockstep = hq_opt_env_only(o, "HQ_BRICK_CHAIN_LOCKSTEP") != nullptr;
+                const int32_t per_xcd = ((int32_t)cs.size() + 7) / 8;
+                for (size_t q = 0; q < cs.size(); q++) {
+                    const std::vector<int32_t>& v = of_col[(size_t)cs[q].col];
+                    hq_brick_chain C = { (int32_t)ch.size(), cs[q].n, lockstep ? 0 : (int32_t)(q / (size_t)std::max(1, per_xcd)) % cs[q].n, 0 };
+                    for (int32_t i = 0; i < cs[q].n; i++) { ch.push_back(B->units[(size_t)v[(size_t)(cs[q].i0 + i)]]); same[(size_t)v[(size_t)(cs[q].i0 + i)]] = 7; }
+                    B->chains.push_back(C);
+                }
+            }
+            B->nchained = (int32_t)ch.size();
+        }
         for (size_t u = 0; u < us.size(); u++)
+            if (same[u] == 7) continue; else
             (same[u] == 1 ? a : (same[u] == 4 ? r : (same[u] == 2 ? h : (same[u] == 3 ? hp : (same[u] == 5 ? rh : (same[u] == 6 ? rhp : b)))))).push_back(B->units[u]);
-        B->nsame = (int32_t)(a.size() + r.size());
+        B->nsame = (int32_t)(ch.size() + a.size() + r.size());
+        ch.insert(ch.end(), a.begin(), a.end());
+        a.swap(ch);
         B->nrag = (int32_t)r.size();
         B->nhet = (int32_t)(h.size() + hp.size());
         B->npacked = (int32_t)hp.size();
@@ -744,6 +835,8 @@
         a.insert(a.end(), rhp.begin(), rhp.end());
         B->units.swap(a);
         if (B->npacked + B->nrpacked == 0) { std::vector<float>().swap(B->coef32); std::vector<double>().swap(B->nt2); }
+        for (const hq_brick_unit& U : B->units) B->narith += (U.flags & HQ_BK_RINGARITH) != 0;
+        if (verbose) fprintf(stderr, "  brick plan: %d chains of %d units; %d units compute their ring ids\n", (int)B->chains.size(), B->nchained, B->narith);
         if (verbose) fprintf(stderr, "  brick plan: %d units: %d with one n_t row of which %d ragged, %d per-element coefficients of which %d packed, %d ragged per-element of which %d packed\n",
                              (int)B->units.size(), B->nsame, B->nrag, B->nhet, B->npacked, B->nrhet, B->nrpacked);
         if (verbose && B->nrag) {
@@ -766,18 +859,25 @@
     return __hiloint2double(hi, lo);
 }
 
-template <bool PERNODE, bool BYCOMP, bool RAGGED = false>
+#ifndef HQ_BK_ABL
+#define HQ_BK_ABL 0
+#endif
+
+template <bool PERNODE, bool BYCOMP, bool RAGGED = false, bool CHAIN = false>
 __global__ void HQ_BK_ATTR __launch_bounds__(HQ_BK_THREADS, 4)
 hq_k_brick(int32_t count, int32_t per_xcd, const hq_brick_unit* __restrict__ units, const int32_t* __restrict__ tab,
            const hq_real* __restrict__ u1g, const hq_real* __restrict__ u2g, hq_real* __restrict__ ung,
            const double* __restrict__ nt3, const int32_t* __restrict__ src_ptr, const int32_t* __restrict__ src_ent,
-           const double* __restrict__ F, double dt2, hq_stencil_coef sc)
+           const double* __restrict__ F, double dt2, hq_stencil_coef sc, const hq_brick_chain* __restrict__ chains)
 {
+    static_assert(!CHAIN || (!PERNODE && !RAGGED), "chains are units of full columns with one n_t row");
     __shared__ __align__(16) double s_w[2 * 3 * HQ_BK_PLANE];
-    const int slot = (int)(blockIdx.x & 7) * per_xcd + (int)(blockIdx.x >> 3);
-    if (slot >= count) return;
-    const hq_brick_unit U = units[slot];
-    const int nx = U.nx, ny = U.ny, np = U.np, nxy = nx * ny, nr = 2 * (nx + 2) + 2 * ny;
+    const int slot0 = (int)(blockIdx.x & 7) * per_xcd + (int)(blockIdx.x >> 3);
+    if (slot0 >= count) return;
+    int slot = slot0, cfirst = slot0, cn = 1, cstart = 0;
+    if (CHAIN) { const hq_brick_chain C = chains[slot0]; cfirst = C.first; cn = C.n; cstart = C.start; slot = cfirst + cstart; }
+    hq_brick_unit U = units[slot];
+    const int nx = U.nx, ny = U.ny, nxy = nx * ny, nr = 2 * (nx + 2) + 2 * ny;
     const int t = threadIdx.x, lx = t & (HQ_BK_TX - 1), ly = t >> 6;
     const bool active = lx < nx && ly < ny;
     const int sidx = active ? ly * nx + lx : 0;
@@ -792,24 +892,21 @@
         else { rx = nx; ry = t - 2 * (nx + 2) - ny; }
         rrow = (ry + 1) * HQ_BK_PY + rx + 1;
     }
-    const int32_t* __restrict__ utab = tab + U.tab;
     const int rofs = ring ? t : 0;
-    const int32_t* __restrict__ cap = utab + (int64_t)(np + 2) * nr;
-    int32_t vOut = -1, vMid = RAGGED ? cap[sidx] : 0, vCur = RAGGED ? cap[nxy + sidx] : 0, vNext = 0;
-    const int32_t id_lo = RAGGED ? (vMid >= 0 ? vMid : -vMid - 2) : cap[sidx];
+    int32_t vOut = -1, vMid = 0, vCur = 0, vNext = 0;
     const double beta = U.beta;
     double P[6], Q[2];
 #pragma unroll
     for (int i = 0; i < 6; i++) P[i] = hq_uniform(U.c1 * sc.p1[i] + U.c2 * sc.p2[i]);
 #pragma unroll
     for (int i = 0; i < 2; i++) Q[i] = hq_uniform(U.c1 * sc.q1[i] + U.c2 * sc.q2[i]);
-    const bool has_src = F && src_ptr[slot + 1] > src_ptr[slot];
 
     hq_real x1[3] = { 0, 0, 0 }, x2[3] = { 0, 0, 0 }, y1[3] = { 0, 0, 0 }, y2[3] = { 0, 0, 0 };
     double mn[3] = { U.m0, U.m2, U.m1 };
     double m0A = hq_uniform(1.0 / U.m0), m0B = m0A;
     double fA[3] = { 0.0, 0.0, 0.0 }, fB[3] = { 0.0, 0.0, 0.0 };
-    int32_t rid = utab[rofs];
+    int32_t rid = 0;
+    int32_t rstr = 0;
 
 #define HQ_BK_LOAD(node_)                                                                             \
     {                                                                                                 \
@@ -818,7 +915,7 @@
             _Pragma("unroll") for (int d = 0; d < 3; d++) { x1[d] = u1g[3 * a_ + d]; x2[d] = u2g[3 * a_ + d]; } \
             if (PERNODE) { _Pragma("unroll") for (int d = 0; d < 3; d++) mn[d] = nt3[3 * a_ + d]; }    \
         }                                                                                             \
-        if (ring && (!RAGGED || rid >= 0)) {                                                          \
+        if (ring && HQ_BK_ABL != 3 && (!RAGGED || rid >= 0)) {                                        \
             const int64_t b_ = (int64_t)rid;                                                          \
             _Pragma("unroll") for (int d = 0; d < 3; d++) { y1[d] = u1g[3 * b_ + d]; y2[d] = u2g[3 * b_ + d]; } \
         }                                                                                             \
@@ -836,23 +933,49 @@
         if (ring) { _Pragma("unroll") for (int d = 0; d < 3; d++) { const double b1_ = y1[d], b2_ = y2[d]; img_[3 * rrow + d] = b1_ + beta * (b1_ - b2_); } } \
     }
 
+    const double rho = hq_uniform((U.c1 - U.c2) / (U.c1 + U.c2));
+    bool cont = false, phas = false;
+    int par = 0, pslot = 0, pnp = 0;
+
+    for (int ci = 0; ci < (CHAIN ? cn : 1); ci++) {
+    bool more = false;
+    if (CHAIN) {
+        const int j = hq_brick_chain_step(cn, cstart, ci, &cont, &more);
+        if (ci > 0) {
+            slot = cfirst + j;
+            U = units[slot];
+            if (!cont) { __syncthreads(); par = 0; }
+        }
+    }
+    const int np = U.np;
+    const int pk = CHAIN ? par : 0;
+    const int32_t* __restrict__ utab = tab + U.tab;
+    const int32_t* __restrict__ cap = utab + (int64_t)(np + 2) * nr;
+    const bool has_src = F && src_ptr[slot + 1] > src_ptr[slot];
     const bool topf = !PERNODE && !RAGGED && (U.flags & HQ_BK_TOPFACE) != 0, botf = !PERNODE && !RAGGED && (U.flags & HQ_BK_BOTFACE) != 0;
-    const double rho = hq_uniform((U.c1 - U.c2) / (U.c1 + U.c2));
-
+    const bool arith = !PERNODE && !RAGGED && (U.flags & HQ_BK_RINGARITH) != 0;
+    if (arith) rstr = utab[nr + rofs] - utab[rofs];
+    if (!CHAIN || !cont) {
+    if (RAGGED) { vMid = cap[sidx]; vCur = cap[nxy + sidx]; }
+    const int32_t id_lo = RAGGED ? (vMid >= 0 ? vMid : -vMid - 2) : cap[sidx];
+    rid = utab[rofs];
+    if (CHAIN) { _Pragma("unroll") for (int d = 0; d < 3; d++) { fA[d] = 0.0; fB[d] = 0.0; } }
     HQ_BK_LOAD((int64_t)id_lo)
-    rid = utab[nr + rofs];
+    rid = arith ? rid + rstr : utab[nr + rofs];
     if (topf) HQ_BK_PUT(0, fB, U.ft[1 + d], U.ft[4 + d])
     else { double dummy[3] = { 0.0, 0.0, 0.0 }; HQ_BK_PUT(0, dummy, mn[1], mn[2]) }
-    for (int k = 0; k <= np + 1; k++) {
+    }
+    const int kend = CHAIN && more ? np - 1 : np + 1;
+    for (int k = 0; k <= kend; k++) {
         if (k <= np) {
             if (RAGGED) {
                 HQ_BK_LOAD((int64_t)(vCur >= 0 ? vCur : -vCur - 2))
                 if (k < np) vNext = cap[(k + 2) * nxy + sidx];
             } else HQ_BK_LOAD(k == np ? (int64_t)cap[nxy + sidx] : U.base + (int64_t)k * nxy + sidx)
-            if (k < np) rid = utab[(k + 2) * nr + rofs];
+            if (k < np) rid = arith ? rid + rstr : utab[(k + 2) * nr + rofs];
         }
         __syncthreads();
-        const hq_lds_double* __restrict__ q = (const hq_lds_double*)s_w + 3 * (HQ_BK_PLANE * (k & 1) + myrow);
+        const hq_lds_double* __restrict__ q = (const hq_lds_double*)s_w + 3 * (HQ_BK_PLANE * ((k + pk) & 1) + myrow);
         double m[3], g[3], Uo[3];
         if (BYCOMP) {
             double A_x, A_y;
@@ -933,14 +1056,16 @@
             for (int d = 0; d < 3; d++) out[d] = f[d] * rm;
         }
         const bool outface = k == 1 && topf;
-        if ((k >= 2 || outface) && active && (!RAGGED || vOut >= 0)) {
+        const bool inprev = CHAIN && cont && k < 2;
+        if ((k >= 2 || outface || inprev) && active && (!RAGGED || vOut >= 0)) {
             double f[3];
 #pragma unroll
             for (int d = 0; d < 3; d++) f[d] = fA[d] + (g[d] + Uo[d]);
             const int local = RAGGED ? (int)(vOut - U.base) : (k - 2) * nxy + sidx;
-            if (has_src) {
-                for (int i = src_ptr[slot]; i < src_ptr[slot + 1]; i++)
-                    if (src_ent[2 * i] == local) {
+            const int sslot = inprev ? pslot : slot, slocal = inprev ? local + pnp * nxy : local;
+            if (inprev ? phas : has_src) {
+                for (int i = src_ptr[sslot]; i < src_ptr[sslot + 1]; i++)
+                    if (src_ent[2 * i] == slocal) {
                         const int li = src_ent[2 * i + 1];
                         for (int d = 0; d < 3; d++) f[d] += F[3 * li + d] * dt2;
                     }
@@ -954,8 +1079,10 @@
         for (int d = 0; d < 3; d++) { fA[d] = fB[d] + m[d]; fB[d] = g[d] - Uo[d]; }
         if (RAGGED) { vOut = vMid; vMid = vCur; vCur = vNext; }
         if (PERNODE) { m0A = m0B; m0B = 1.0 / mn[0]; }
-        if (k < np || (k == np && !botf)) HQ_BK_PUT((k + 1) & 1, fB, mn[1], mn[2])
-        else if (k == np) HQ_BK_PUT((k + 1) & 1, fB, U.fb[1 + d], U.fb[4 + d])
+        if (k < np || (k == np && !botf)) HQ_BK_PUT((k + 1 + pk) & 1, fB, mn[1], mn[2])
+        else if (k == np) HQ_BK_PUT((k + 1 + pk) & 1, fB, U.fb[1 + d], U.fb[4 + d])
+    }
+    if (CHAIN && more) { par = (par + np) & 1; pslot = slot; pnp = np; phas = has_src; }
     }
 #undef HQ_BK_LOAD
 #undef HQ_BK_PUT
@@ -1152,7 +1279,7 @@
 
 static void hq_brick_free(hq_brick_plan* P)
 {
-    void* ptrs[] = { P->d_units, P->d_tab, P->d_coef, P->d_coef32, P->d_nt2, P->d_src_ptr, P->d_src_ent };
+    void* ptrs[] = { P->d_units, P->d_tab, P->d_coef, P->d_coef32, P->d_nt2, P->d_src_ptr, P->d_src_ent, P->d_chains };
     for (void* p : ptrs) if (p) hipFree(p);
     *P = hq_brick_plan();
 }
@@ -1167,7 +1294,14 @@
     P->npacked = B.npacked;
     P->nrhet = B.nrhet;
     P->nrpacked = B.nrpacked;
+    P->nchains = (int32_t)B.chains.size();
+    P->nchained = B.nchained;
     if (P->nunits == 0) return 0;
+    if (P->nchains > 0) {
+        if (hipMalloc((void**)&P->d_chains, sizeof(hq_brick_chain) * B.chains.size()) != hipSuccess) { g_patch_err = "hipMalloc failed"; return -2; }
+        *bytes += (int64_t)(sizeof(hq_brick_chain) * B.chains.size());
+        if (hipMemcpy(P->d_chains, B.chains.data(), sizeof(hq_brick_chain) * B.chains.size(), hipMemcpyHostToDevice) != hipSuccess) { g_patch_err = "brick table upload failed"; return -3; }
+    }
     if (P->nhet + P->nrhet > 0) {
         if (P->nhet > P->npacked || P->nrhet > P->nrpacked) {
             if (hipMalloc((void**)&P->d_coef, 8 * B.coef.size()) != hipSuccess) { g_patch_err = "hipMalloc failed"; return -2; }
@@ -1247,16 +1381,22 @@
 static void hq_brick_launch(const hq_brick_plan* P, const hq_real* u1, const hq_real* u2, hq_real* un, const double* nt3,
                             const double* F, double dt2, hipStream_t stream, bool light = false)
 {
-    const int32_t cnt[7] = { P->nsame - P->nrag, P->nunits - P->nsame - P->nhet - P->nrhet, P->nhet - P->npacked, P->npacked, P->nrag,
+    const int32_t* const sp0 = P->d_src_ptr;
+    if (P->nchains > 0) {
+        const int32_t count = P->nchains, per_xcd = (count + 7) / 8;
+        if (light) hq_k_brick<false, true, false, true><<<per_xcd * 8, HQ_BK_THREADS, 0, stream>>>(count, per_xcd, P->d_units, P->d_tab, u1, u2, un, nt3, sp0, P->d_src_ent, (sp0 ? F : nullptr), dt2, hq_stencil().c, P->d_chains);
+        else hq_k_brick<false, false, false, true><<<per_xcd * 8, HQ_BK_THREADS, 0, stream>>>(count, per_xcd, P->d_units, P->d_tab, u1, u2, un, nt3, sp0, P->d_src_ent, (sp0 ? F : nullptr), dt2, hq_stencil().c, P->d_chains);
+    }
+    const int32_t cnt[7] = { P->nsame - P->nrag - P->nchained, P->nunits - P->nsame - P->nhet - P->nrhet, P->nhet - P->npacked, P->npacked, P->nrag,
                              P->nrhet - P->nrpacked, P->nrpacked };
-    int32_t first = 0;
+    int32_t first = P->nchained;
     for (int k4 = 0; k4 < 7; k4++) {
         const int k = k4 == 0 ? 0 : (k4 == 1 ? 4 : (k4 < 5 ? k4 - 1 : k4));
         const int32_t count = cnt[k];
         if (count <= 0) continue;
         const int per_xcd = (count + 7) / 8;
         const int32_t* sp = P->d_src_ptr ? P->d_src_ptr + first : nullptr;
-#define HQ_BK_ARGS count, per_xcd, P->d_units + first, P->d_tab, u1, u2, un, nt3, sp, P->d_src_ent, (sp ? F : nullptr), dt2, hq_stencil().c
+#define HQ_BK_ARGS count, per_xcd, P->d_units + first, P->d_tab, u1, u2, un, nt3, sp, P->d_src_ent, (sp ? F : nullptr), dt2, hq_stencil().c, (const hq_brick_chain*)nullptr
 #ifdef HQ_EXPERIMENT
         const unsigned xpad = getenv("HQ_X_BRICK_LDS_PAD") ? (unsigned)atoi(getenv("HQ_X_BRICK_LDS_PAD")) : 0u;
         if (xpad && k == 0) {
diff --git a/hercules_amd/csrc/hq_engine.hip b/hercules_amd/csrc/hq_engine.hip
--- a/hercules_amd/csrc/hq_engine.hip
+++ b/hercules_amd/csrc/hq_engine.hip
@@ -8,6 +8,7 @@
 
 #include <algorithm>
 #include <chrono>
+#include <functional>
 #include <vector>
 
 #define HQ_SOLVER_IMPLEMENTATION 1
@@ -1437,7 +1438,9 @@
         if ((rc = hq_brick_excluded(d, excl)) != HQ_OK) return bail(rc);
         hq_mat_src ms;
         ms.edata = d->edata; ms.dt = d->deltaT; ms.bbase = d->mat_bbase; ms.thr_damp = d->mat_threshold_damping; ms.thr_vpvs = d->mat_threshold_vpvs;
-        if (hq_brick_plan_host(opts, c->E, c->N, d->lnid, d->node_xyz, c1.data(), c2.data(), beta.data(), ntab, excl.data(), &BH, &ms) != 0)
+        hq_options bopts = opts;
+        if (!hq_given(bopts.brick_chain) && c->nranks > 1) bopts.brick_chain = 0;
+        if (hq_brick_plan_host(bopts, c->E, c->N, d->lnid, d->node_xyz, c1.data(), c2.data(), beta.data(), ntab, excl.data(), &BH, &ms) != 0)
             return bail(hq_fail(HQ_ERR_ARG, "brick plan: %s", hq_patch_error()));
         lap("brick plan");
     }
@@ -1864,7 +1867,7 @@
     return HQ_OK;
 }
 
-static thread_local int64_t g_brick_check_extra[4];
+static thread_local int64_t g_brick_check_extra[9];
 
 extern "C" int hq_brick_plan_check(const hq_desc* d, int64_t report[8])
 {
@@ -1888,6 +1891,7 @@
     ms.edata = d->edata; ms.dt = d->deltaT; ms.bbase = d->mat_bbase; ms.thr_damp = d->mat_threshold_damping; ms.thr_vpvs = d->mat_threshold_vpvs;
     std::vector<double> nt64;
     const double* ntab = hq_ntable64(d, nt64);
+    if (!hq_given(opts.brick_chain) && d->nranks > 1) opts.brick_chain = 0;
     if (hq_brick_plan_host(opts, E, N, d->lnid, d->node_xyz, c1.data(), c2.data(), beta.data(), ntab, excl.data(), &B, &ms) != 0)
         return hq_fail(HQ_ERR_ARG, "brick plan: %s", hq_patch_error());
     int64_t bad = 0, nchecked = 0;
@@ -1910,6 +1914,55 @@
     }
     std::vector<int32_t> covered((size_t)B.nb, 0);
     int64_t nsame = 0;
+    const int64_t nunits_all = (int64_t)B.units.size();
+    std::vector<char> ucont((size_t)nunits_all, 0), umore((size_t)nunits_all, 0);
+    int64_t chain_interior_caps = 0, caps_loaded = 0;
+    {
+        std::vector<char> in_chain((size_t)nunits_all, 0);
+        for (const hq_brick_chain& C : B.chains) {
+            if (C.first < 0 || C.n < 1 || C.start < 0 || C.start >= C.n || (int64_t)C.first + C.n > B.nchained || B.nchained > B.nsame - B.nrag) { bad++; continue; }
+            for (int i = 0; i < C.n; i++) {
+                bool cont = false, more = false;
+                const int j = hq_brick_chain_step(C.n, C.start, i, &cont, &more);
+                const size_t u = (size_t)(C.first + j);
+                if (in_chain[u]) bad++;
+                in_chain[u] = 1;
+                ucont[u] = cont; umore[u] = more;
+                chain_interior_caps += (!cont && j > 0) + (!more && j + 1 < C.n);
+                const hq_brick_unit& U = B.units[u];
+                if (j > 0) {
+                    const hq_brick_unit& V = B.units[u - 1];
+                    if (U.nx != V.nx || U.ny != V.ny || U.base != V.base + (int64_t)V.nx * V.ny * V.np || U.c1 != V.c1 || U.c2 != V.c2 || U.beta != V.beta ||
+                        U.m0 != V.m0 || U.m2 != V.m2 || U.m1 != V.m1 || (U.flags & HQ_BK_TOPFACE) || (V.flags & HQ_BK_BOTFACE)) bad++;
+                }
+                if (U.np < 2 || (U.flags & (HQ_BK_HET | HQ_BK_RAGGED)) || !(U.flags & HQ_BK_NTSAME)) bad++;
+            }
+        }
+        for (int64_t u = 0; u < nunits_all; u++) {
+            if ((in_chain[(size_t)u] != 0) != (u < B.nchained)) bad++;
+            caps_loaded += !ucont[(size_t)u] + !umore[(size_t)u];
+            if ((B.units[(size_t)u].flags & HQ_BK_RINGARITH) && (B.units[(size_t)u].np < 2 || (B.units[(size_t)u].flags & (HQ_BK_HET | HQ_BK_RAGGED)) || !(B.units[(size_t)u].flags & HQ_BK_NTSAME))) bad++;
+        }
+    }
+    std::function<int64_t(int64_t, int, int)> ring_id = [&](int64_t u, int row, int pos) -> int64_t {
+        const hq_brick_unit& U = B.units[(size_t)u];
+        const int nr = 2 * (U.nx + 2) + 2 * U.ny;
+        const int32_t* t = B.tab.data() + U.tab;
+        const bool arith = (U.flags & HQ_BK_RINGARITH) != 0;
+        if (ucont[(size_t)u]) {
+            if (row <= 1) return ring_id(u - 1, B.units[(size_t)u - 1].np + row, pos);
+            return arith ? ring_id(u, 1, pos) + (int64_t)(row - 1) * ((int64_t)t[nr + pos] - t[pos]) : (int64_t)t[(int64_t)row * nr + pos];
+        }
+        return arith ? (int64_t)t[pos] + (int64_t)row * ((int64_t)t[nr + pos] - t[pos]) : (int64_t)t[(int64_t)row * nr + pos];
+    };
+    auto cap_id = [&](int64_t u, int side, int x, int y) -> int64_t {
+        const hq_brick_unit& U = B.units[(size_t)u];
+        const int64_t nxy = (int64_t)U.nx * U.ny;
+        if (!side && ucont[(size_t)u]) { const hq_brick_unit& V = B.units[(size_t)u - 1]; return V.base + (int64_t)(V.np - 1) * nxy + y * U.nx + x; }
+        if (side && umore[(size_t)u]) return B.units[(size_t)u + 1].base + y * U.nx + x;
+        const int32_t* cap = B.tab.data() + U.tab + (int64_t)(U.np + 2) * (2 * (U.nx + 2) + 2 * U.ny);
+        return cap[(side ? nxy : 0) + y * U.nx + x];
+    };
 #pragma omp parallel for schedule(dynamic, 4) reduction(+ : bad, nchecked, nsame)
     for (int64_t u = 0; u < (int64_t)B.units.size(); u++) {
         const hq_brick_unit& U = B.units[(size_t)u];
@@ -1935,13 +1988,19 @@
             }
             if (in) {
                 if (k >= 0 && k < np) return U.base + ((int64_t)k * ny + y) * nx + x;
-                return cap[(k < 0 ? 0 : nx * ny) + y * nx + x];
-            }
-            const int32_t* r = ring + (int64_t)(k + 1) * nr;
-            if (y == -1) return r[x + 1];
-            if (y == ny) return r[nx + 2 + x + 1];
-            if (x == -1) return r[2 * (nx + 2) + y];
-            return r[2 * (nx + 2) + ny + y];
+                return cap_id(u, k < 0 ? 0 : 1, x, y);
+            }
+            if (rag || het) {
+                const int32_t* r = ring + (int64_t)(k + 1) * nr;
+                if (y == -1) return r[x + 1];
+                if (y == ny) return r[nx + 2 + x + 1];
+                if (x == -1) return r[2 * (nx + 2) + y];
+                return r[2 * (nx + 2) + ny + y];
+            }
+            if (y == -1) return ring_id(u, k + 1, x + 1);
+            if (y == ny) return ring_id(u, k + 1, nx + 2 + x + 1);
+            if (x == -1) return ring_id(u, k + 1, 2 * (nx + 2) + y);
+            return ring_id(u, k + 1, 2 * (nx + 2) + ny + y);
         };
         int64_t next = U.base;
         for (int k = 0; k < np; k++)
@@ -2002,13 +2061,12 @@
             const bool in = x >= 0 && x < nx && y >= 0 && y < ny;
             if (in) {
                 if (k >= 0 && k < np) return U.base + ((int64_t)k * ny + y) * nx + x;
-                return cap[(k < 0 ? 0 : nx * ny) + y * nx + x];
-            }
-            const int32_t* r = ring + (int64_t)(k + 1) * nr;
-            if (y == -1) return r[x + 1];
-            if (y == ny) return r[nx + 2 + x + 1];
-            if (x == -1) return r[2 * (nx + 2) + y];
-            return r[2 * (nx + 2) + ny + y];
+                return cap_id(u, k < 0 ? 0 : 1, x, y);
+            }
+            if (y == -1) return ring_id(u, k + 1, x + 1);
+            if (y == ny) return ring_id(u, k + 1, nx + 2 + x + 1);
+            if (x == -1) return ring_id(u, k + 1, 2 * (nx + 2) + y);
+            return ring_id(u, k + 1, 2 * (nx + 2) + ny + y);
         };
         for (int side = 0; side < 2; side++) {
             if (!(U.flags & (side ? HQ_BK_BOTFACE : HQ_BK_TOPFACE))) continue;
@@ -2112,6 +2170,11 @@
         const int32_t* pl = B.tab.data() + U.tab + (int64_t)(U.np + 2) * (2 * (U.nx + 2) + 2 * U.ny);
         for (int64_t i = (int64_t)U.nx * U.ny; i < (int64_t)U.nx * U.ny * (U.np + 1); i++) g_brick_check_extra[(U.flags & HQ_BK_HET) ? 3 : 1] += pl[i] >= 0;
     }
+    g_brick_check_extra[4] = (int64_t)B.chains.size();
+    g_brick_check_extra[5] = B.nchained;
+    g_brick_check_extra[6] = chain_interior_caps;
+    g_brick_check_extra[7] = B.narith;
+    g_brick_check_extra[8] = caps_loaded;
     if (bad) return hq_fail(HQ_ERR_STATE, "brick plan self-check failed%s", "");
     return HQ_OK;
 }
@@ -2120,10 +2183,10 @@
 {
     int64_t r8[8] = { 0, 0, 0, 0, 0, 0, 0, 0 };
     if (!report || n < 8) return hq_fail(HQ_ERR_ARG, "hq_brick_plan_check_n: a report of at least 8 entries%s", "");
-    for (int k = 0; k < 4; k++) g_brick_check_extra[k] = 0;
+    for (int k = 0; k < 9; k++) g_brick_check_extra[k] = 0;
     const int rc = hq_brick_plan_check(d, r8);
     for (int k = 0; k < 8; k++) report[k] = r8[k];
-    for (int k = 8; k < n; k++) report[k] = k < 12 ? g_brick_check_extra[k - 8] : 0;
+    for (int k = 8; k < n; k++) report[k] = k < 17 ? g_brick_check_extra[k - 8] : 0;
     return rc;
 }
 
diff --git a/hercules_amd/csrc/hq_opts.h b/hercules_amd/csrc/hq_opts.h
--- a/hercules_amd/csrc/hq_opts.h
+++ b/hercules_amd/csrc/hq_opts.h
@@ -26,6 +26,7 @@
     HQ_OPT_D("HQ_LOOPBACK_DELAY_US", loopback_delay_us), HQ_OPT_I("HQ_PATCH_VERBOSE", verbose), HQ_OPT_I("HQ_QUIET", quiet),
     HQ_OPT_I("HQ_BRICK_RAGGED", brick_ragged), HQ_OPT_I("HQ_BRICK_RAGGED_MINFILL", brick_ragged_minfill),
     HQ_OPT_I("HQ_PHASE_TIMING", phase_timing), HQ_OPT_I("HQ_BRICK_RAGGED_HET", brick_ragged_het),
+    HQ_OPT_I("HQ_BRICK_CHAIN", brick_chain), HQ_OPT_I("HQ_BRICK_RING_ARITH", brick_ring_arith),
 };
 #undef HQ_OPT_I
 #undef HQ_OPT_D
@@ -38,7 +39,6 @@
         else *(double*)((char*)o + e.off) = -1.0;
     }
     o->allow_env = -1;
-    o->reserved0 = -1;
 }
 
 static void hq_options_adopt(hq_options* dst, const hq_options* src)
diff --git a/include/hq_solver.h b/include/hq_solver.h
--- a/include/hq_solver.h
+++ b/include/hq_solver.h
@@ -155,8 +155,9 @@
     int32_t brick_ragged_minfill;
     int32_t allow_env;
     int32_t brick_ragged_het;
-    int32_t reserved0;
+    int32_t brick_chain;
     int32_t phase_timing;
+    int32_t brick_ring_arith;
 } hq_options;
 
 HQ_API void hq_options_init(hq_options* opts, uint64_t size);
```

Measured after the change: 58.37 billion. -7.9%, worse.
